# sabarim/STEm-Seg

Measured on AMD Instinct MI355X. Metric: clips/sec (T=8, 480p) embed+cluster, higher is better.
Workload: dtype f16x3: fp32 emulated from 2 fp16 terms per operand (22-bit operand significands; fp32 has 24), power-of-two operand scaling, 3 fp16 MFMA products per fp32 product, fp32 accumulate; |activation| >= 2.6e5 -> non-finite, flagged on the device, clip re-run in bf16x6

## Files before the change

### include/stemseg_hip.h

```cpp
#ifndef STEMSEG_HIP_H
#define STEMSEG_HIP_H

#include <stddef.h>
#include <stdint.h>

#ifdef __cplusplus
extern "C" {
#endif

#define STEMSEG_HIP_ABI_VERSION 11

#define STEMSEG_OK              0
#define STEMSEG_E_INVALID      -1
#define STEMSEG_E_HIP          -2
#define STEMSEG_E_WORKSPACE    -3
#define STEMSEG_E_UNSUPPORTED  -4

#define STEMSEG_MAX_HEAD_OUT   10
#define STEMSEG_MAX_WIDE_HEAD_OUT 64
#define STEMSEG_MAX_INSTANCES  64
#define STEMSEG_MAX_EMB_DIMS    8
#define STEMSEG_MAX_SEMSEG_CLASSES 128

int         stemseg_hip_version(void);
const char* stemseg_hip_last_error(void);
int         stemseg_hip_device_count(void);

int stemseg_hip_profile_enable(int32_t on);
int stemseg_hip_profile_read(double* out_host, int32_t n_tags);

typedef struct StemsegVolume {
    float*  ptr;
    int64_t c_stride, t_stride, y_stride;
    int32_t C, T, H, W;
    int64_t limit;
} StemsegVolume;

int stemseg_hip_padded_geometry(int32_t C, int32_t T, int32_t H, int32_t W, int64_t out[5]);


int stemseg_hip_pack_conv_weight(const float* w, float* packed, int32_t Cout, int32_t Cin, int32_t taps, void* stream);

#define STEMSEG_TILE_CFG_DEEP 8
typedef struct StemsegConvEpilogue {
    int32_t      relu;
    const float* residual;
    int64_t      res_c_stride, res_t_stride, res_y_stride;
    int32_t      decode_H, decode_W;
    int32_t      precision;
    int32_t      frames, plan_frames;
    int64_t      plan_scratch_floats;
} StemsegConvEpilogue;
#define STEMSEG_PRECISION_F32    0
#define STEMSEG_PRECISION_BF16X6 2
#define STEMSEG_PRECISION_F16X3  3
int64_t stemseg_hip_packed_weight_bytes_prec(int32_t Cout, int32_t Cin, int32_t taps, int32_t precision);
int stemseg_hip_pack_conv_weight_prec(const float* w, void* packed, int32_t Cout, int32_t Cin, int32_t taps, int32_t precision, void* stream);
int stemseg_hip_conv3d(const StemsegVolume* in, const float* packed_w, const float* bias, const StemsegVolume* out,
                       int32_t kt, int32_t kh, int32_t kw, int32_t tile_cfg, float* splitk_scratch,
                       int64_t splitk_scratch_floats, const StemsegConvEpilogue* epilogue, void* stream);
int stemseg_hip_conv3d_zero_t_halo(const StemsegVolume* in, const float* packed_w, const float* bias, const StemsegVolume* out,
                                   int32_t kt, int32_t kh, int32_t kw, int32_t tile_cfg, float* splitk_scratch,
                                   int64_t splitk_scratch_floats, const StemsegConvEpilogue* epilogue, int32_t groups, float eps,
                                   float* stats, double* gn_scratch, void* stream);
int stemseg_hip_conv3d_zero_t_halo_clips(const StemsegVolume* in, const float* packed_w, const float* bias, const StemsegVolume* out,
                                         int32_t kt, int32_t kh, int32_t kw, int32_t tile_cfg, float* splitk_scratch,
                                         int64_t splitk_scratch_floats, const StemsegConvEpilogue* epilogue, int32_t groups, float eps,
                                         float* stats, double* gn_scratch, int32_t plan_clips, void* stream);

int stemseg_hip_conv3d_zero_t_halo_batch(const StemsegVolume* in, const float* packed_w, const float* bias, const StemsegVolume* out,
                                         int32_t kt, int32_t kh, int32_t kw, int32_t tile_cfg, const StemsegConvEpilogue* epilogue,
                                         int32_t n_clips, int64_t in_clip_stride, int64_t out_clip_stride, void* stream);

typedef struct StemsegConvPlanRecord {
    int32_t kt, kh, kw;
    int32_t ck, mt;
    int32_t rows, tw, nt;
    int32_t flat, pmax;
    int32_t gl, blk;
    int32_t threads;
    int32_t precision;
    int32_t ksplit, chunks_per_split, nchunks;
    int32_t grid[3];
    int32_t row0, row1;
    int32_t vec4, vec_epi;
    int32_t reduce;
    int32_t gn;
    int32_t zero_t_halo;
    int32_t nb;
    int32_t deep;
} StemsegConvPlanRecord;
#define STEMSEG_PLAN_GN          1
#define STEMSEG_PLAN_ZERO_T_HALO 2
int stemseg_hip_conv3d_plan(const StemsegVolume* in, const float* bias, const StemsegVolume* out, int32_t kt, int32_t kh, int32_t kw,
                            int32_t tile_cfg, const float* splitk_scratch, int64_t splitk_scratch_floats,
                            const StemsegConvEpilogue* epilogue, int32_t form, int32_t gn_groups, StemsegConvPlanRecord* records,
                            int32_t capacity, int32_t* count);
int stemseg_hip_conv3d_plan_clips(const StemsegVolume* in, const float* bias, const StemsegVolume* out, int32_t kt, int32_t kh, int32_t kw,
                                  int32_t tile_cfg, const float* splitk_scratch, int64_t splitk_scratch_floats,
                                  const StemsegConvEpilogue* epilogue, int32_t form, int32_t gn_groups, int32_t plan_clips,
                                  StemsegConvPlanRecord* records, int32_t capacity, int32_t* count);

int64_t stemseg_hip_packed_grouped_weight_bytes(int32_t Cout, int32_t Cin_g, int32_t groups, int32_t precision);
int stemseg_hip_pack_grouped_conv_weight(const float* w, void* packed, int32_t Cout, int32_t Cin_g, int32_t groups, int32_t precision, void* stream);
int stemseg_hip_conv2d_grouped(const StemsegVolume* in, const void* packed_w, const float* bias, const StemsegVolume* out, int32_t groups,
                               int32_t stride, int32_t relu, int32_t precision, int32_t plan_frames, void* stream);

int64_t stemseg_hip_conv3d_gn_scratch_doubles(int32_t Cout, int32_t groups);
int stemseg_hip_conv3d_gn(const StemsegVolume* in, const float* packed_w, const float* bias, const StemsegVolume* out,
                          int32_t kt, int32_t kh, int32_t kw, int32_t tile_cfg, float* splitk_scratch,
                          int64_t splitk_scratch_floats, int32_t precision, int32_t groups, float eps,
                          float* stats, double* gn_scratch, void* stream);

int stemseg_hip_groupnorm_stats(const float* x, int32_t C, int64_t S, int32_t groups, float eps,
                                float* stats, double* scratch, void* stream);

int stemseg_hip_gn_relu_pool(const float* x, int32_t C, int32_t T, int32_t H, int32_t W, int32_t groups,
                             const float* stats, const float* gamma, const float* beta, int32_t pool,
                             const StemsegVolume* out, void* stream);

int stemseg_hip_upsample_trilinear(const float* in, int32_t C, int32_t T, int32_t H, int32_t W,
                                   int32_t st, int32_t sy, int32_t sx, const StemsegVolume* out, void* stream);

int stemseg_hip_copy_to_volume(const float* in, int32_t layout, const StemsegVolume* out, void* stream);

int stemseg_hip_heads(const float* x, int32_t Cin, int32_t T, int32_t H, int32_t W,
                      const float* w, const float* bias, int32_t n_out, const int32_t* act_host,
                      const int32_t* grid_axis_host, const float* grid_t, const float* grid_y, const float* grid_x,
                      float* out, void* stream);

int stemseg_hip_nonfinite_flags(const float* x, int64_t n, int32_t* flags, int32_t n_flags, void* stream);

typedef struct StemsegDecoderDesc {
    int32_t struct_bytes;
    int32_t in_channels;
    int32_t inter[4];
    int32_t T, H4, W4;
    int32_t gn_groups;
    float   gn_eps;
    int32_t pool[3];
    int32_t t_scale[3];
    int32_t n_out;
    int32_t act[STEMSEG_MAX_EMB_DIMS * 2];
    int32_t grid_axis[STEMSEG_MAX_EMB_DIMS * 2];
    int32_t input_layout;
    int32_t concurrency;
    int32_t detached;
    int32_t precision;
    int32_t n_clips;
    int64_t feat_clip_stride[4];
    int64_t out_clip_stride;
    int32_t plan_clips;
    int32_t reserved;
} StemsegDecoderDesc;

typedef struct StemsegDecoderWeights {
    const float* conv_w[7];
    const float* conv_b[7];
    const float* gn_w[7];
    const float* gn_b[7];
    const float* fuse_w[3];
    const float* head_w;
    const float* head_b;
    const float* grid_t;
    const float* grid_y;
    const float* grid_x;
} StemsegDecoderWeights;

size_t stemseg_hip_decoder_workspace_bytes(const StemsegDecoderDesc* desc);
int stemseg_hip_decoder_init_workspace(const StemsegDecoderDesc* desc, void* workspace, size_t ws_bytes, void* stream);
int stemseg_hip_decoder_check_workspace(const StemsegDecoderDesc* desc, const void* workspace, size_t ws_bytes, int32_t* n_bad_host,
                                        int64_t* first_bad_host, void* stream);
int stemseg_hip_decoder_forward(const StemsegDecoderDesc* desc, const StemsegDecoderWeights* weights,
                                const float* const feats[4], float* out,
                                void* workspace, size_t ws_bytes, void* stream);

int stemseg_hip_decoder_join(int32_t concurrency, void* stream);

#define STEMSEG_MAX_ENCODER_BLOCKS 40

typedef struct StemsegEncoderDesc {
    int32_t struct_bytes;
    int32_t blocks[4];
    int32_t T, H, W;
    int32_t out_channels;
    int32_t precision;
    int32_t n_clips;
    int32_t clip_frames;
    int32_t clip_stride;
    int32_t plan_frames;
    int32_t fuse_tail;
    int32_t conv2_groups;
    int32_t width_per_group;
    int32_t stride_in_3x3;
} StemsegEncoderDesc;

typedef struct StemsegEncoderWeights {
    const float* stem_w;
    const float* stem_b;
    const float* stem_w_s2d;
    const float* conv1_w[STEMSEG_MAX_ENCODER_BLOCKS];   const float* conv1_b[STEMSEG_MAX_ENCODER_BLOCKS];
    const float* conv2_w[STEMSEG_MAX_ENCODER_BLOCKS];   const float* conv2_b[STEMSEG_MAX_ENCODER_BLOCKS];
    const float* conv3_w[STEMSEG_MAX_ENCODER_BLOCKS];   const float* conv3_b[STEMSEG_MAX_ENCODER_BLOCKS];
    const float* down_w[STEMSEG_MAX_ENCODER_BLOCKS];    const float* down_b[STEMSEG_MAX_ENCODER_BLOCKS];
    const float* fpn_inner_w[4]; const float* fpn_inner_b[4];
    const float* fpn_layer_w[4]; const float* fpn_layer_b[4];
} StemsegEncoderWeights;

size_t stemseg_hip_encoder_workspace_bytes(const StemsegEncoderDesc* desc);
int stemseg_hip_encoder_plan_offsets(const StemsegEncoderDesc* desc, int64_t* out25);
int stemseg_hip_encoder_stage_end_mask(const StemsegEncoderDesc* desc, int32_t* mask_out);

int stemseg_hip_stem_conv(const float* frames, const float* w_tap_major, const float* bias, float* out, int32_t T, int32_t H, int32_t W,
                          void* stream);
#define STEMSEG_STREAM_FORM_AUTO   0
#define STEMSEG_STREAM_FORM_SCALAR 1
#define STEMSEG_STREAM_FORM_VEC4   2
#define STEMSEG_UP2_FORM_SCALAR    1
#define STEMSEG_UP2_FORM_VEC4X2    2
#define STEMSEG_UP2_FORM_DENSE     3
int stemseg_hip_maxpool3x3s2(const float* in, int64_t planes, int32_t H, int32_t W, float* out, int32_t form, int32_t* form_used, void* stream);
int stemseg_hip_encoder_subsample2(const float* in, int64_t planes, int32_t H, int32_t W, float* out, int32_t form, int32_t* form_used,
                                   void* stream);
int stemseg_hip_upsample2x_add(const StemsegVolume* fine, const float* fine_dense, const StemsegVolume* coarse, int32_t form, int32_t* form_used,
                               void* stream);
int stemseg_hip_stem_s2d(const float* frames, int32_t T, int32_t H, int32_t W, const StemsegVolume* s2d, void* stream);
int stemseg_hip_encoder_stream_forms(const StemsegEncoderDesc* desc, int32_t out[7]);
int stemseg_hip_encoder_init_workspace(const StemsegEncoderDesc* desc, void* workspace, size_t ws_bytes, void* stream);
int stemseg_hip_encoder_check_workspace(const StemsegEncoderDesc* desc, const void* workspace, size_t ws_bytes, int32_t* n_bad_host,
                                        int64_t* first_bad_host, void* stream);
int stemseg_hip_encoder_forward(const StemsegEncoderDesc* desc, const StemsegEncoderWeights* weights, const float* frames,
                                const StemsegVolume* out, void* workspace, size_t ws_bytes, void* stream);
int stemseg_hip_encoder_stem_forward(const StemsegEncoderDesc* desc, const StemsegEncoderWeights* weights, const float* frames, float* stem_out,
                                     float* pooled, void* workspace, size_t ws_bytes, void* stream);


int stemseg_hip_seediness_accumulate(float* acc, const float* plane, int64_t n, int32_t first, void* stream);
int stemseg_hip_fg_mask(const float* acc, float count, float thr, uint8_t* mask, int64_t n, void* stream);
int stemseg_hip_fg_mask_frames(const float* acc, const float* counts, float thr, uint8_t* mask, int32_t F, int64_t HW,
                               void* stream);

int stemseg_hip_fg_gather(const float* emb, const float* bw, const float* seed, const uint8_t* fg,
                          int32_t E, int32_t Ev, int32_t T, int64_t HW,
                          float* emb_out, float* bw_out, float* seed_out, int32_t* voxel_index,
                          int64_t* frame_offsets, void* scratch, void* stream);

typedef struct StemsegClusterParams {
    float   primary_prob_thresh;
    float   secondary_prob_thresh;
    float   min_seediness_prob;
    int32_t max_instances;
    int32_t n_free_dims;
    float   free_dim_bandwidths[STEMSEG_MAX_EMB_DIMS];
} StemsegClusterParams;
// ... 319 lines not shown
```

### stem-seg_amd/csrc/conv_igemm.h

```cpp
#pragma once
#include "common.h"
#include "split_operand.h"
#include <algorithm>
#include <type_traits>

namespace stemseg {

typedef float f32x16 __attribute__((ext_vector_type(16)));

constexpr int MIN_WG4 = 4;

struct ConvKParams {
    const float* in;
    int64_t in_cs, in_ts, in_ys, in_limit;
    int in_H;
    const float* wpk;
    const float* bias;
    float* out;
    int64_t out_cs, out_ts, out_ys;
    int Cin, Cout, T, H, W;
    int tiles_x, tiles_y;
    int vec4;
    int chunks_per_split;
    int64_t out_split_stride;
    int relu;
    const float* res;
    int64_t res_cs, res_ts, res_ys;
    int dec_H, dec_W;
    int vec_epi;
    int t_fastest;
    int flat_t;
    int T_all;
    int n_co;
    double* gn_part;
    int gn_cpg, gn_cap, gn_slot0;
    int* gn_used_host;
    int nb;
    int zero_t_halo;
    int64_t in_bs, out_bs, gn_bs;
    unsigned int* out_p16;
};

template <int KT_, int KH_, int KW_, int CK_, int MI_, int NI_, int WM_, int WN_, int COLS_, bool PIPE_ = false, int BF_ = 0, bool DB_ = false,
          int PMAX_ = 0, bool GL_ = false, int BLK_ = 0>
struct ConvCfg {
    static constexpr bool PIPE = PIPE_, X6 = BF_ >= 2, F16 = BF_ == 3, DB = DB_, FLAT = PMAX_ > 0, GL = GL_;
    static_assert(BF_ == 0 || BF_ == 2 || BF_ == 3, "precision: 0 fp32-input MFMA, 2 bf16x6, 3 f16x3");
    static constexpr int NPX = BF_ == 2 ? 3 : 2;
    static constexpr int NPROD = BF_ == 2 ? 6 : 3;
    static constexpr int PMAX = PMAX_;
    static constexpr int KT = KT_, KH = KH_, KW = KW_, CK = CK_, MI = MI_, NI = NI_, WM = WM_, WN = WN_, COLS = COLS_;
    static constexpr int TAPS = KT * KH * KW;
    static constexpr int NTHREADS = 64 * WM * WN;
    static constexpr int MT = WM * MI * 32;
    static constexpr int NSEG = WN * NI;
    static constexpr bool BLK = BLK_ != 0;
    static constexpr bool DEEP = BLK_ < 0;
    static constexpr int TD = DEEP ? WN_ : 1;
    static constexpr int TPL = DEEP ? TD + 2 : KT_;
    static constexpr int NLIVE = (BLK && !DEEP) ? BLK_ * COLS_ : NSEG;
    static constexpr int ROWS = DEEP ? 4 * NI_ : (BLK ? 4 * BLK_ : NSEG / COLS);
    static constexpr int TW = BLK ? 8 * COLS_ : COLS_ * 32;
    static constexpr int RH = ROWS + KH - 1;
    static constexpr int XL = (TW + KW - 1 + 3) / 4;
    static constexpr int XP = DEEP ? 24 : (BLK ? ((4 * XL + 23) / 32) * 32 + 8 : 4 * XL);
    static constexpr int NT = NSEG * 32;
    static constexpr int FL = NT + 2 * PMAX + 8;
    static constexpr int IN_CH_STRIDE = FLAT ? KT * FL : KT * RH * XP;
    static constexpr int IN_PAIR_STRIDE = PMAX_ > 0 ? KT * (WN_ * NI_ * 32 + 2 * PMAX_ + 8) : TPL * RH * XP;
    static constexpr int IN_PLANE_STRIDE = (CK / 2) * IN_PAIR_STRIDE;
    static constexpr int IN_FLOATS = X6 ? NPX * IN_PLANE_STRIDE : CK * IN_CH_STRIDE;
    static constexpr SplitLayout SL = SplitLayout(TAPS, BF_, CK_);
    static_assert(BF_ < 2 || CK_ == split_chunk_channels(TAPS, BF_), "split-staged tiles walk the channel chunks the weights were packed in");
    static constexpr int TPG = SL.TPG, CPH = SL.CPH, NTG = SL.NTG;
    static constexpr int NCG = X6 ? SL.NCG : 1;
    static constexpr int G = NTG * NCG;
    static constexpr int NPL = SL.NPL;
    static constexpr int W_FLOATS = X6 ? NPL * G * 2 * MT * 4 : CK * TAPS * MT;
    static constexpr int GA = (G + 1) / 2;
    static constexpr int WMODE = (BF_ >= 2 && G <= 2) ? (BF_ == 3 ? 1 : ((WM * WN >= 8 || MI * NI < 8) ? 2 : 0)) : 0;
    static constexpr bool SP = WMODE == 1, LA = WMODE == 2;
    static constexpr int BUF_FLOATS = IN_FLOATS + W_FLOATS;
    static constexpr int LDS_FLOATS = BUF_FLOATS * (DB ? 2 : 1);
    static_assert(!X6 || CK % (2 * CPH) == 0, "split-staged: a chunk holds whole k-groups");
    static_assert(BLK || NSEG % COLS == 0, "segments must fill whole rows");
    static_assert(!BLK || (BF_ >= 2 && PMAX_ == 0 && NI_ == 2 && NLIVE <= NSEG && NLIVE > NSEG - NI_ && XP % 32 == (DEEP ? 24 : 8) && XP >= 4 * XL), "block tiles: split-staged, the last wave may lack its second block");
    static_assert(!DEEP || (BF_ == 3 && KT_ == 3 && WM_ == 1 && COLS_ == 1 && BLK_ == -1), "deep tile: f16x3, 3x3x3, one wave per output plane");
    static_assert(CK % 4 == 0 || (DB && GL_ && CK == 2 && !X6), "channel chunk is a multiple of the packed sub-chunk (4), or one channel pair (GL)");
    static_assert(LDS_FLOATS * 4 <= (X6 ? 160 : 80) * 1024, "two workgroups per CU (x6 eight-wave tiles: one)");
    static_assert(!X6 || (!DB && !GL && G >= 2 && CK % 2 == 0), "x6: 2-D / 3-D tiles, two weight phases");
    static_assert(!FLAT || (KH == 3 && KW == 3 && PMAX % 4 == 0), "flat tiles: 3x3 taps");
    static_assert(DB == GL_, "two LDS buffers are the direct-to-LDS form");
    static_assert(!GL || (DB && !X6), "direct-to-LDS staging is the double-buffered fp32 form");
    static constexpr int NWAVES = WM * WN;
    static constexpr int MIN_WG = X6 ? (MI * NI > 8 ? 1 : NWAVES >= 8 ? 2 : (LDS_FLOATS * 4 * 2 <= 160 * 1024 ? NWAVES / 2 : NWAVES / 4))
                                     : ((GL && LDS_FLOATS * 4 * 4 <= 140 * 1024 && MI * NI <= 4) ? MIN_WG4 : ((GL && LDS_FLOATS * 4 * 3 <= 160 * 1024) ? 3 : 2));
};

template <class C>
__global__ __launch_bounds__(C::NTHREADS, C::MIN_WG) void conv_igemm_kernel(const ConvKParams p) {
    __shared__ __attribute__((aligned(16))) float smem[C::LDS_FLOATS];
    float* const in_lds = smem;
    float* const w_lds = smem + C::IN_FLOATS;

    const int tid = threadIdx.x;
    const int lane = tid & 63;
    const int wave = __builtin_amdgcn_readfirstlane(tid >> 6);
    const int wm = wave / C::WN, wn = wave % C::WN;
    const int half = lane >> 5, l31 = lane & 31;

    int bx;
    {
        const int nwg = gridDim.x, xcd = blockIdx.x & 7, q = nwg >> 3, r = nwg & 7;
        bx = (xcd < r ? xcd * (q + 1) : r * (q + 1) + (xcd - r) * q) + (blockIdx.x >> 3);
    }
    const int co_tile = bx % p.n_co;
    bx /= p.n_co;
    int tx, ty, t;
    if constexpr (C::DEEP) {
        tx = bx % p.tiles_x;
        ty = bx / p.tiles_x;
        t = 0;
    } else if (C::KT > 1 && p.t_fastest) {
        t = bx % p.T;
        bx /= p.T;
        tx = bx % p.tiles_x;
        ty = bx / p.tiles_x;
    } else {
        tx = bx % p.tiles_x;
        bx /= p.tiles_x;
        ty = bx % p.tiles_y;
        t = bx / p.tiles_y;
    }
    const int x0 = C::FLAT ? 0 : tx * C::TW, y0 = C::FLAT ? 0 : ty * C::ROWS;
    constexpr bool TV = C::KT == 3 && C::X6 && !C::FLAT && (C::F16 || C::MI * C::NI < 8);
    int tvar = 0;
    if constexpr (TV) {
        if constexpr (C::DEEP) tvar = wn == 0 ? 1 : (wn == C::WN - 1 ? 2 : 0);
        else if (p.zero_t_halo && p.T > 1) tvar = t == 0 ? 1 : (t == p.T - 1 ? 2 : 0);
    }
    const int svar = C::DEEP ? 0 : tvar;
    const int t_out = C::DEEP ? wn : t;
    auto seg_row = [](const int sN, const int l) __attribute__((always_inline)) { return C::DEEP ? (sN % C::NI) * 4 + (l >> 3) : (C::BLK ? (sN / C::COLS) * 4 + (l >> 3) : sN / C::COLS); };
    auto seg_col = [](const int sN, const int l) __attribute__((always_inline)) { return C::DEEP ? (l & 7) : (C::BLK ? (sN % C::COLS) * 8 + (l & 7) : (sN % C::COLS) * 32 + l); };
    const bool ni1_live = !C::BLK || (wn * C::NI + 1 < C::NLIVE);
    const int pitch = (int)p.in_ys;
    const int F0 = pitch + tx * C::NT;
    const int co0 = co_tile * C::MT;

    f32x16 acc[C::MI][C::NI];
#pragma unroll
    for (int mi = 0; mi < C::MI; ++mi)
#pragma unroll
        for (int ni = 0; ni < C::NI; ++ni)
#pragma unroll
            for (int r = 0; r < 16; ++r) acc[mi][ni][r] = 0.f;

    const float* a_ptr = w_lds + half * C::MT + wm * (C::MI * 32) + l31;
    const float* b_ptr[C::NI];
#pragma unroll
    for (int ni = 0; ni < C::NI; ++ni) {
        const int s = wn * C::NI + ni;
        b_ptr[ni] = C::FLAT ? in_lds + half * C::IN_CH_STRIDE + s * 32 + l31 + 3
                            : in_lds + half * C::IN_CH_STRIDE + seg_row(s, l31) * C::XP + seg_col(s, l31);
    }

    const unsigned int* b_ptr6[C::NI];
#pragma unroll
    for (int ni = 0; ni < C::NI; ++ni) {
        const int s = wn * C::NI + ni;
        b_ptr6[ni] = C::FLAT ? reinterpret_cast<const unsigned int*>(in_lds) + half * (C::CPH / 2) * C::IN_PAIR_STRIDE + s * 32 + l31 + 3
                             : reinterpret_cast<const unsigned int*>(in_lds) + half * (C::CPH / 2) * C::IN_PAIR_STRIDE + seg_row(min(s, C::NLIVE - 1), l31) * C::XP + seg_col(min(s, C::NLIVE - 1), l31);
        if constexpr (C::DEEP) b_ptr6[ni] += wn * (C::RH * C::XP);
    }
    const float* in_tile = p.in + (int64_t)blockIdx.y * p.in_bs + (int64_t)t * p.in_ts + x0;
    const int64_t tile_base = (int64_t)t * p.in_ts + x0;

    constexpr int XQ = C::XP / 4;
    constexpr int NQ = C::FLAT ? C::IN_FLOATS / 4 : C::CK * C::KT * C::RH * XQ;
    constexpr int MQ = C::MT / 4;
    constexpr int NWQ = C::X6 ? C::NPL * C::G * 2 * C::MT : C::CK * C::TAPS * MQ;
    constexpr int IN_PT = (NQ + C::NTHREADS - 1) / C::NTHREADS, W_PT = (NWQ + C::NTHREADS - 1) / C::NTHREADS;
    auto fetch_in = [&](int c0, int q) -> float4 {
        if constexpr (C::FLAT) {
            constexpr int FQ = C::FL / 4;
            const int j4 = q % FQ, rr = q / FQ, dt = rr % C::KT, c = rr / C::KT;
            const int f = F0 - pitch - 4 + 4 * j4;
            const int64_t rel = (int64_t)(c0 + c) * p.in_cs + (int64_t)dt * p.in_ts + f;
            float4 v = make_float4(0.f, 0.f, 0.f, 0.f);
            if (c0 + c < p.Cin && f >= 0 && 4 * j4 < C::NT + 2 * pitch + 8 && tile_base + rel + 4 <= p.in_limit)
                v = *reinterpret_cast<const float4*>(in_tile + rel);
            return v;
        }
        const int xq = q % XQ;
        int rr = q / XQ;
        const int r = rr % C::RH;
        rr /= C::RH;
        const int dt = rr % C::KT;
        const int c = rr / C::KT;
        const int yy = min(y0 + r, p.in_H - 1);
        const int64_t rel = (int64_t)(c0 + c) * p.in_cs + (int64_t)dt * p.in_ts + (int64_t)yy * p.in_ys + xq * 4;
        float4 v = make_float4(0.f, 0.f, 0.f, 0.f);
        if (c0 + c < p.Cin && tile_base + rel + 4 <= p.in_limit) v = *reinterpret_cast<const float4*>(in_tile + rel);
        return v;
    };
    auto fetch_w = [&](int c0, int q) -> float4 {
        const int mq = q % MQ;
        if constexpr (C::CK == 2) {
            const int row2 = q / MQ, tap = row2 >> 1, e = row2 & 1;
            const float* wsrc2 = p.wpk + ((int64_t)(c0 / 4) * (C::TAPS * 4) + tap * 4 + ((c0 >> 1) & 1) * 2 + e) * p.Cout + co0;
            float4 v2 = make_float4(0.f, 0.f, 0.f, 0.f);
            if (c0 + e < p.Cin && co0 + mq * 4 < p.Cout) v2 = *reinterpret_cast<const float4*>(wsrc2 + mq * 4);
            return v2;
        }
        const int row = q / MQ;
        const int ch = c0 + (row / (C::TAPS * 4)) * 4 + (row & 3);
        const float* wsrc = p.wpk + (int64_t)(c0 / 4) * (C::TAPS * 4) * p.Cout + co0;
        float4 v = make_float4(0.f, 0.f, 0.f, 0.f);
        if (ch < p.Cin && co0 + mq * 4 < p.Cout) v = *reinterpret_cast<const float4*>(wsrc + (int64_t)row * p.Cout + mq * 4);
        return v;
    };
    auto addr_in = [&](int c0, int q) -> const float* {
        int64_t rel;
        if constexpr (C::FLAT) {
            constexpr int FQ = C::FL / 4;
            const int j4 = q % FQ, rr = q / FQ, dt = rr % C::KT, c = rr / C::KT;
            const int f = max(F0 - pitch - 4 + 4 * j4, 0);
            rel = (int64_t)(c0 + c) * p.in_cs + (int64_t)dt * p.in_ts + f;
        } else {
            const int xq = q % XQ;
            int rr = q / XQ;
            const int r = rr % C::RH;
            rr /= C::RH;
            const int dt = rr % C::KT;
            const int c = rr / C::KT;
            const int yy = min(y0 + r, p.in_H - 1);
            rel = (int64_t)(c0 + c) * p.in_cs + (int64_t)dt * p.in_ts + (int64_t)yy * p.in_ys + xq * 4;
        }
        const int64_t last = p.in_limit - 4 - tile_base;
        return in_tile + (rel < last ? rel : last);
    };
    auto addr_w = [&](int c0, int q) -> const float* {
        const int mq = q % MQ;
        if constexpr (C::CK == 2) {
            const int row2 = q / MQ, tap = row2 >> 1, e = row2 & 1;
            return p.wpk + ((int64_t)(c0 / 4) * (C::TAPS * 4) + tap * 4 + ((c0 >> 1) & 1) * 2 + e) * p.Cout + co0 + mq * 4;
        } else {
            const int row = q / MQ;
            return p.wpk + (int64_t)(c0 / 4) * (C::TAPS * 4) * p.Cout + co0 + (int64_t)row * p.Cout + mq * 4;
        }
    };
    auto glds_chunk = [&](int c0, const int off) {
        typedef const __attribute__((address_space(1))) void* gptr_t;
        typedef __attribute__((address_space(3))) void* lptr_t;
#pragma unroll
        for (int k = 0; k < IN_PT; ++k) {
            const int q = tid + k * C::NTHREADS;
            if (q < NQ) __builtin_amdgcn_global_load_lds((gptr_t)addr_in(c0, q), (lptr_t)(in_lds + off + (q - lane) * 4), 16, 0, 0);
        }
#pragma unroll
        for (int k = 0; k < W_PT; ++k) {
            const int q = tid + k * C::NTHREADS;
            if (q < NWQ) __builtin_amdgcn_global_load_lds((gptr_t)addr_w(c0, q), (lptr_t)(w_lds + off + (q - lane) * 4), 16, 0, 0);
        }
    };
    auto stage_direct = [&](int c0) {
        if (p.vec4) {
            for (int q = tid; q < NQ; q += C::NTHREADS) *reinterpret_cast<float4*>(in_lds + q * 4) = fetch_in(c0, q);
        } else if constexpr (!C::FLAT) {
            constexpr int NE = C::CK * C::KT * C::RH * C::XP;
            for (int q = tid; q < NE; q += C::NTHREADS) {
                const int xx = q % C::XP;
                int rr = q / C::XP;
                const int r = rr % C::RH;
                rr /= C::RH;
                const int dt = rr % C::KT;
                const int c = rr / C::KT;
                const int yy = min(y0 + r, p.in_H - 1);
                const int64_t rel = (int64_t)(c0 + c) * p.in_cs + (int64_t)dt * p.in_ts + (int64_t)yy * p.in_ys + xx;
                float v = 0.f;
                if (c0 + c < p.Cin && tile_base + rel < p.in_limit) v = in_tile[rel];
                in_lds[q] = v;
            }
        }
        for (int q = tid; q < NWQ; q += C::NTHREADS) *reinterpret_cast<float4*>(w_lds + q * 4) = fetch_w(c0, q);
    };

    auto split3 = [](const float x, unsigned int& h, unsigned int& m, unsigned int& l) {
        unsigned short sh, sm, sl = 0;
        if constexpr (C::F16) split_act_f16(x, sh, sm);
        else split_bf16x3(x, sh, sm, sl);
        h = sh; m = sm; l = sl;
    };
    constexpr int FQ6 = C::FL / 4;
    constexpr int XL6 = C::XL;
    constexpr int NQ6 = C::FLAT ? (C::CK / 2) * C::KT * FQ6 : (C::CK / 2) * (C::DEEP ? C::TD : C::KT) * C::RH * XL6;
    auto in6_lds = [](const int q) __attribute__((always_inline)) {
        if constexpr (C::DEEP) return (q / XL6 + (q / (XL6 * C::RH * C::TD)) * 2 * C::RH + C::RH) * C::XP + (q % XL6) * 4;
        else return C::BLK ? (q / XL6) * C::XP + (q % XL6) * 4 : q * 4;
    };
    constexpr int IN_PT6 = C::X6 ? (NQ6 + C::NTHREADS - 1) / C::NTHREADS : 1;
    constexpr int NWQ_A = C::NPL * C::GA * 2 * C::MT, NWQ6 = C::NPL * C::G * 2 * C::MT;
    auto in6_rel = [&](int q, int& c) -> int64_t {
        if constexpr (C::FLAT) {
            const int j4 = q % FQ6, rr = q / FQ6, dt = rr % C::KT;
            c = 2 * (rr / C::KT);
            const int f = F0 - pitch - 4 + 4 * j4;
            if (f < 0 || 4 * j4 >= C::NT + 2 * pitch + 8) return -1;
            return (int64_t)c * p.in_cs + (int64_t)dt * p.in_ts + f;
        }
        const int xq = q % XL6;
        int rr = q / XL6;
        const int r = rr % C::RH;
        rr /= C::RH;
        constexpr int NPLQ = C::DEEP ? C::TD : C::KT;
        const int dt = rr % NPLQ + (C::DEEP ? 1 : 0);
        c = 2 * (rr / NPLQ);
        const int yy = min(y0 + r, p.in_H - 1);
        return (int64_t)c * p.in_cs + (int64_t)dt * p.in_ts + (int64_t)yy * p.in_ys + xq * 4;
    };
    auto fetch_in6 = [&](int c0, int q, float4& v0, float4& v1) {
        int c;
        const int64_t rel0 = in6_rel(q, c);
        const int64_t rel = rel0 + (int64_t)c0 * p.in_cs;
        v0 = v1 = make_float4(0.f, 0.f, 0.f, 0.f);
        if (rel0 < 0) return;
        if (c0 + c < p.Cin && tile_base + rel + 4 <= p.in_limit) v0 = *reinterpret_cast<const float4*>(in_tile + rel);
        if (c0 + c + 1 < p.Cin && tile_base + rel + p.in_cs + 4 <= p.in_limit) v1 = *reinterpret_cast<const float4*>(in_tile + rel + p.in_cs);
    };
    unsigned int in6_voff[IN_PT6];
    int in6_clim[IN_PT6];
    const int64_t in6_room = (p.in_limit - 4 - tile_base) * 4;
    constexpr int R6 = C::RH * XL6;
    constexpr int NQ6V = TV ? (C::CK / 2) * 2 * R6 : NQ6;
    constexpr int IN_PT6V = TV ? (NQ6V + C::NTHREADS - 1) / C::NTHREADS : IN_PT6;
    auto in6_live = [](const int qv, const int first) __attribute__((always_inline)) { return qv + (qv / (2 * R6)) * R6 + (first ? R6 : 0); };
    if constexpr (C::X6) {
#pragma unroll
        for (int k = 0; k < IN_PT6; ++k) {
            int q = tid + k * C::NTHREADS;
            bool inside = q < NQ6;
            if constexpr (TV && !C::DEEP) {
                if (tvar) { inside = q < NQ6V; q = inside ? in6_live(q, tvar == 1) : 0; }
            }
            int c = 0;
            const int64_t rel0 = inside ? in6_rel(q, c) : 0;
            const int64_t rel = rel0 < 0 ? 0 : rel0;
            in6_voff[k] = (unsigned int)(rel * 4);
            const int64_t slack = in6_room - rel * 4;
            const int64_t by_room = slack < 0 ? 0 : slack / (p.in_cs * 4) + 1;
            in6_clim[k] = (inside && rel0 >= 0) ? (int)min((int64_t)(p.Cin - c), by_room) : 0;
        }
    }
    typedef float f32x4 __attribute__((ext_vector_type(4)));
    auto fetch_in6_fast = [&](int c0, int k, f32x4& v0, f32x4& v1) __attribute__((always_inline)) {
        const char* base = reinterpret_cast<const char*>(in_tile) + (int64_t)c0 * p.in_cs * 4;
        const unsigned int cs4 = (unsigned int)(p.in_cs * 4);
        v0 = *reinterpret_cast<const f32x4*>(base + (c0 < in6_clim[k] ? in6_voff[k] : 0u));
        v1 = *reinterpret_cast<const f32x4*>(base + (c0 + 1 < in6_clim[k] ? in6_voff[k] + cs4 : 0u));
    };
    auto store_in6 = [&](int q, const float4& v0, const float4& v1) {
        unsigned int h0, m0, l0, h1, m1, l1;
        uint4 ph, pm, pl;
        if constexpr (C::F16) {
            split_pair_f16(v0.x, v1.x, ph.x, pm.x); split_pair_f16(v0.y, v1.y, ph.y, pm.y);
            split_pair_f16(v0.z, v1.z, ph.z, pm.z); split_pair_f16(v0.w, v1.w, ph.w, pm.w);
            unsigned int* d16 = reinterpret_cast<unsigned int*>(in_lds) + in6_lds(q);
            *reinterpret_cast<uint4*>(d16) = ph;
            *reinterpret_cast<uint4*>(d16 + C::IN_PLANE_STRIDE) = pm;
            return;
        }
        split3(v0.x, h0, m0, l0); split3(v1.x, h1, m1, l1); ph.x = h0 | (h1 << 16); pm.x = m0 | (m1 << 16); pl.x = l0 | (l1 << 16);
        split3(v0.y, h0, m0, l0); split3(v1.y, h1, m1, l1); ph.y = h0 | (h1 << 16); pm.y = m0 | (m1 << 16); pl.y = l0 | (l1 << 16);
        split3(v0.z, h0, m0, l0); split3(v1.z, h1, m1, l1); ph.z = h0 | (h1 << 16); pm.z = m0 | (m1 << 16); pl.z = l0 | (l1 << 16);
        split3(v0.w, h0, m0, l0); split3(v1.w, h1, m1, l1); ph.w = h0 | (h1 << 16); pm.w = m0 | (m1 << 16); pl.w = l0 | (l1 << 16);
        unsigned int* d = reinterpret_cast<unsigned int*>(in_lds) + in6_lds(q);
        *reinterpret_cast<uint4*>(d) = ph;
        *reinterpret_cast<uint4*>(d + C::IN_PLANE_STRIDE) = pm;
        if constexpr (C::NPX == 3) *reinterpret_cast<uint4*>(d + 2 * C::IN_PLANE_STRIDE) = pl;
    };
    auto store_in6_masked = [&](int c0, int k, int q, const f32x4& r0, const f32x4& r1) __attribute__((always_inline)) {
        const bool ok0 = c0 < in6_clim[k], ok1 = c0 + 1 < in6_clim[k];
        float4 v0, v1;
        v0.x = ok0 ? r0.x : 0.f; v0.y = ok0 ? r0.y : 0.f; v0.z = ok0 ? r0.z : 0.f; v0.w = ok0 ? r0.w : 0.f;
        v1.x = ok1 ? r1.x : 0.f; v1.y = ok1 ? r1.y : 0.f; v1.z = ok1 ? r1.z : 0.f; v1.w = ok1 ? r1.w : 0.f;
        store_in6(q, v0, v1);
    };
    auto stage_in6_direct = [&](int c0) {
        if (p.vec4) {
            for (int q = tid; q < NQ6; q += C::NTHREADS) {
                float4 v0, v1;
                fetch_in6(c0, q, v0, v1);
                store_in6(q, v0, v1);
            }
        } else if constexpr (!C::FLAT && !C::DEEP) {
            constexpr int NE6 = (C::CK / 2) * C::KT * C::RH * C::XP;
            for (int q = tid; q < NE6; q += C::NTHREADS) {
                const int xx = q % C::XP;
                int rr = q / C::XP;
                const int r = rr % C::RH;
                rr /= C::RH;
                const int dt = rr % C::KT;
                const int c = 2 * (rr / C::KT);
                const int yy = min(y0 + r, p.in_H - 1);
                const int64_t rel = (int64_t)(c0 + c) * p.in_cs + (int64_t)dt * p.in_ts + (int64_t)yy * p.in_ys + xx;
                float a0 = 0.f, a1 = 0.f;
                if (c0 + c < p.Cin && tile_base + rel < p.in_limit) a0 = in_tile[rel];
                if (c0 + c + 1 < p.Cin && tile_base + rel + p.in_cs < p.in_limit) a1 = in_tile[rel + p.in_cs];
                unsigned int h0, m0, l0, h1, m1, l1;
                split3(a0, h0, m0, l0);
                split3(a1, h1, m1, l1);
                unsigned int* d = reinterpret_cast<unsigned int*>(in_lds) + q;
                d[0] = h0 | (h1 << 16);
                d[C::IN_PLANE_STRIDE] = m0 | (m1 << 16);
                if constexpr (C::NPX == 3) d[2 * C::IN_PLANE_STRIDE] = l0 | (l1 << 16);
            }
        }
    };
    constexpr int W_PT6 = C::X6 ? ((C::SP ? NWQ6 : NWQ_A) + C::NTHREADS - 1) / C::NTHREADS : 1;
    static_assert(C::NTHREADS % C::MT == 0 && NWQ_A % C::MT == 0, "weight pieces: a thread keeps its column");
    const unsigned int w6_voff = C::X6 ? ((unsigned int)(tid / C::MT) * (unsigned int)p.Cout + (unsigned int)min(tid % C::MT, p.Cout - 1 - co0)) * 16u : 0u;
    auto w6_src = [&](int c0, int q_uniform) __attribute__((always_inline)) -> const char* {
        const char* base = reinterpret_cast<const char*>(p.wpk) +
                           (((int64_t)(c0 / C::CK) * (C::NPL * C::G * 2) + q_uniform / C::MT) * p.Cout + co0) * 16;
        return base + w6_voff;
    };
    auto compute6 = [&](auto g0c, auto g1c, auto&& side, auto live_c) __attribute__((always_inline)) {
        constexpr int g0 = decltype(g0c)::value, g1 = decltype(g1c)::value;
        constexpr bool LIVE1 = decltype(live_c)::value;
        constexpr int NPL = C::NPL, NPX = C::NPX, NA = 3;
        typedef typename std::conditional<C::F16, _Float16, __bf16>::type h16;
        typedef h16 h16x8 __attribute__((ext_vector_type(8)));
        const char* a_base = reinterpret_cast<const char*>(w_lds) + (half * C::MT + wm * (C::MI * 32) + l31) * 16;
        const unsigned int* bdy6[C::NI][3];
        if constexpr (C::FLAT) {
#pragma unroll
            for (int ni = 0; ni < C::NI; ++ni) { bdy6[ni][0] = b_ptr6[ni]; bdy6[ni][1] = b_ptr6[ni] + pitch; bdy6[ni][2] = b_ptr6[ni] + 2 * pitch; }
        }
        auto ld_b = [&](const int grp, h16x8 (&b)[NPX][C::NI]) __attribute__((always_inline)) {
            const int cg = grp / C::NTG, tg = grp % C::NTG;
#pragma unroll
            for (int ni = 0; ni < (LIVE1 ? C::NI : 1); ++ni)
#pragma unroll
                for (int pl = 0; pl < NPX; ++pl) {
                    uint4 w4;
                    unsigned int* wv = reinterpret_cast<unsigned int*>(&w4);
#pragma unroll
                    for (int wd = 0; wd < 4; ++wd) {
                        const int j0 = 2 * wd, tapi = j0 / C::CPH, chl = j0 % C::CPH;
                        int tap = tg * C::TPG + tapi;
                        tap = tap < C::TAPS ? tap : C::TAPS - 1;
                        const int dt = tap / (C::KH * C::KW), dy = (tap / C::KW) % C::KH, dx = tap % C::KW;
                        if constexpr (C::FLAT) {
                            const int off = pl * C::IN_PLANE_STRIDE + (cg * C::CPH + chl / 2) * C::IN_PAIR_STRIDE + dt * C::FL + dx;
                            wv[wd] = bdy6[ni][dy][off];
                        } else {
                            const int off = pl * C::IN_PLANE_STRIDE + (cg * C::CPH + chl / 2) * C::IN_PAIR_STRIDE + (dt * C::RH + dy) * C::XP + dx;
                            wv[wd] = b_ptr6[ni][off];
                        }
                    }
                    b[pl][ni] = __builtin_bit_cast(h16x8, w4);
                }
        };
        auto ld_a = [&](const int grp, const int mi, h16x8 (&a)[NA]) __attribute__((always_inline)) {
#pragma unroll
            for (int pl = 0; pl < NPL; ++pl)
                a[pl] = *reinterpret_cast<const h16x8*>(a_base + (((grp * NPL + pl) * 2) * C::MT + mi * 32) * 16);
        };
        auto mm = [&](const int mi, h16x8 (&a)[NA], const h16x8 (&b)[NPX][C::NI]) __attribute__((always_inline)) {
            if constexpr (C::F16) {
                a[2] = a[0] * (h16)(1.0f / F16X3_LO_SCALE);
#define SS_X6_TERM(PA, PB)                                                                                                     \
    _Pragma("unroll") for (int ni = 0; ni < (LIVE1 ? C::NI : 1); ++ni)                                                         \
        acc[mi][ni] = __builtin_amdgcn_mfma_f32_32x32x16_f16(a[PA], b[PB][ni], acc[mi][ni], 0, 0, 0);
                SS_X6_TERM(1, 0) SS_X6_TERM(2, 1) SS_X6_TERM(0, 0)
#undef SS_X6_TERM
            } else {
#define SS_X6_TERM(PA, PB)                                                                                                     \
    _Pragma("unroll") for (int ni = 0; ni < (LIVE1 ? C::NI : 1); ++ni)                                                         \
        acc[mi][ni] = __builtin_amdgcn_mfma_f32_32x32x16_bf16(a[PA], b[PB][ni], acc[mi][ni], 0, 0, 0);
                SS_X6_TERM(2, 0) SS_X6_TERM(0, 2) SS_X6_TERM(1, 1) SS_X6_TERM(1, 0) SS_X6_TERM(0, 1) SS_X6_TERM(0, 0)
#undef SS_X6_TERM
            }
        };
        constexpr int NSTEP = (g1 - g0) * C::MI;
        h16x8 bfr[NPX][C::NI], a0[NA], a1[NA];
        side(-1);
        ld_b(g0, bfr);
        ld_a(g0, 0, a0);
#pragma unroll
        for (int st = 0; st < NSTEP; st += 2) {
            const int mi = st % C::MI;
            if (st + 1 < NSTEP) ld_a(g0 + (st + 1) / C::MI, (st + 1) % C::MI, a1);
            side(st);
            __builtin_amdgcn_sched_barrier(0);
            mm(mi, a0, bfr);
            __builtin_amdgcn_sched_barrier(0);
            if (st + 1 < NSTEP) {
                if ((st + 1) % C::MI == 0) ld_b(g0 + (st + 1) / C::MI, bfr);
                if (st + 2 < NSTEP) ld_a(g0 + (st + 2) / C::MI, (st + 2) % C::MI, a0);
                side(st + 1);
                __builtin_amdgcn_sched_barrier(0);
                mm((st + 1) % C::MI, a1, bfr);
                __builtin_amdgcn_sched_barrier(0);
                if (st + 2 < NSTEP && (st + 2) % C::MI == 0) ld_b(g0 + (st + 2) / C::MI, bfr);
            }
        }
    };
    auto compute = [&](const int buf_off = 0) {
        constexpr int NSUB = C::CK >= 4 ? C::CK / 4 : 1, NCP = C::CK >= 4 ? 2 : 1, WROWS = C::CK >= 4 ? 4 : 2;
        const float* bdy[C::NI][3];
        if constexpr (C::FLAT) {
#pragma unroll
            for (int ni = 0; ni < C::NI; ++ni) {
                bdy[ni][0] = b_ptr[ni]; bdy[ni][1] = b_ptr[ni] + pitch; bdy[ni][2] = b_ptr[ni] + 2 * pitch;
            }
        }
        constexpr int NSTEPS = NSUB * C::TAPS * NCP;
        auto ld = [&](const int i, float (&a)[C::MI], float (&b)[C::NI]) {
            const int cp = i % NCP, tap = (i / NCP) % C::TAPS, sub = i / (NCP * C::TAPS);
            const int dt = tap / (C::KH * C::KW), dy = (tap / C::KW) % C::KH, dx = tap % C::KW;
            const int wrow = (sub * C::TAPS + tap) * WROWS + cp * 2;
            const int boff = C::FLAT ? (sub * 4 + cp * 2) * C::IN_CH_STRIDE + dt * C::FL + dx
                                     : (sub * 4 + cp * 2) * C::IN_CH_STRIDE + (dt * C::RH + dy) * C::XP + dx;
#pragma unroll
            for (int mi = 0; mi < C::MI; ++mi) a[mi] = a_ptr[buf_off + wrow * C::MT + mi * 32];
#pragma unroll
            for (int ni = 0; ni < C::NI; ++ni) {
                if constexpr (C::FLAT) b[ni] = bdy[ni][dy][buf_off + boff];
                else b[ni] = b_ptr[ni][buf_off + boff];
            }
        };
        auto mm = [&](const float (&a)[C::MI], const float (&b)[C::NI]) {
#pragma unroll
            for (int mi = 0; mi < C::MI; ++mi)
#pragma unroll
                for (int ni = 0; ni < C::NI; ++ni)
                    acc[mi][ni] = __builtin_amdgcn_mfma_f32_32x32x2f32(a[mi], b[ni], acc[mi][ni], 0, 0, 0);
        };
        float a0[C::MI], b0[C::NI], a1[C::MI], b1[C::NI];
        ld(0, a0, b0);
#pragma unroll
        for (int i = 0; i < NSTEPS; i += 2) {
            if (i + 1 < NSTEPS) ld(i + 1, a1, b1);
            __builtin_amdgcn_sched_barrier(0);
            mm(a0, b0);
            __builtin_amdgcn_sched_barrier(0);
            if (i + 1 < NSTEPS) {
                if (i + 2 < NSTEPS) ld(i + 2, a0, b0);
                __builtin_amdgcn_sched_barrier(0);
                mm(a1, b1);
                __builtin_amdgcn_sched_barrier(0);
            }
        }
    };

    const int c_begin = blockIdx.z * p.chunks_per_split * C::CK;
    const int c_end = min(p.Cin, c_begin + p.chunks_per_split * C::CK);
    if constexpr (C::X6) {
        typedef std::integral_constant<int, 0> Q0;
        typedef std::integral_constant<int, NWQ_A> QA;
        typedef std::integral_constant<int, NWQ6> QE;
        f32x4 rin[2 * IN_PT6];
        f32x4 rw6[W_PT6];
        f32x4 rw6b[W_PT6];
        auto fetch_w6_k = [&](int c0, auto q0c, auto q1c, f32x4 (&r)[W_PT6], const int k) __attribute__((always_inline)) {
            constexpr int q0 = decltype(q0c)::value, q1 = decltype(q1c)::value;
            if ((k + 1) * C::NTHREADS <= q1 - q0 || q0 + tid + k * C::NTHREADS < q1) r[k] = *reinterpret_cast<const f32x4*>(w6_src(c0, q0 + k * C::NTHREADS));
        };
        auto store_w6 = [&](auto q0c, auto q1c, const f32x4 (&r)[W_PT6]) __attribute__((always_inline)) {
            constexpr int q0 = decltype(q0c)::value, q1 = decltype(q1c)::value;
    #pragma unroll
            for (int k = 0; k < W_PT6; ++k) { const int q = q0 + tid + k * C::NTHREADS; if ((k + 1) * C::NTHREADS <= q1 - q0 || (k * C::NTHREADS < q1 - q0 && q < q1)) *reinterpret_cast<f32x4*>(w_lds + q * 4) = r[k]; }
        };
        auto store_in6_all = [&](int c0, auto var_c) __attribute__((always_inline)) {
            constexpr int V = decltype(var_c)::value;
            constexpr int NQV = V ? NQ6V : NQ6, PTV = V ? IN_PT6V : IN_PT6;
            if (p.vec4) {
#pragma unroll
                for (int k = 0; k < PTV; ++k) {
                    const int q = tid + k * C::NTHREADS;
                    if ((k + 1) * C::NTHREADS <= NQV || q < NQV) store_in6_masked(c0, k, V ? in6_live(q, V == 1) : q, rin[2 * k], rin[2 * k + 1]);
                }
            } else stage_in6_direct(c0);
        };
        auto side_items = [&](const int st, auto nspread_c, auto n_in_c, auto n_w_c, auto&& f_in, auto&& f_w) __attribute__((always_inline)) {
            constexpr int nspread = decltype(nspread_c)::value, n_in = decltype(n_in_c)::value, n_w = decltype(n_w_c)::value, n = n_in + n_w;
            if (st >= nspread || st < 0) return;
#pragma unroll
            for (int i = 0; i < n; ++i)
                if (i >= st * n / nspread && i < (st + 1) * n / nspread) { if (i < n_in) f_in(i); else f_w(i - n_in); }
        };
        constexpr int NSA = C::GA * C::MI, NSB = (C::G - C::GA) * C::MI, NSALL = C::G * C::MI;
        constexpr int NPA = (NWQ_A + C::NTHREADS - 1) / C::NTHREADS, NPB = (NWQ6 - NWQ_A + C::NTHREADS - 1) / C::NTHREADS;
        constexpr int NPALL = (NWQ6 + C::NTHREADS - 1) / C::NTHREADS;
        constexpr bool SPRD = C::F16;
        typedef std::integral_constant<int, C::GA> GAc;
        typedef std::integral_constant<int, C::G> Gc;
        typedef std::integral_constant<int, 0> I0;
        typedef std::integral_constant<int, IN_PT6> INc;
        constexpr int TG_FIRST = TV ? (C::KH * C::KW) / C::TPG : 0, TG_LAST = TV ? (2 * C::KH * C::KW + C::TPG - 1) / C::TPG : C::G;
        static_assert(!TV || (C::NCG == 1 && !C::SP && !C::LA && TG_FIRST < C::GA && TG_LAST > C::GA), "temporal-halo variants: one channel group, both phases keep a k-group");
        if (c_begin < c_end) {
            if constexpr (TV) {
                const int q_lo = svar == 1 ? C::NPL * TG_FIRST * 2 * C::MT : 0, q_hi = svar == 2 ? C::NPL * TG_LAST * 2 * C::MT : NWQ6;
                for (int q = q_lo + tid; q < q_hi; q += C::NTHREADS) *reinterpret_cast<float4*>(w_lds + q * 4) = *reinterpret_cast<const float4*>(w6_src(c_begin, q - tid));
            } else {
                for (int q = tid; q < NWQ6; q += C::NTHREADS) *reinterpret_cast<float4*>(w_lds + q * 4) = *reinterpret_cast<const float4*>(w6_src(c_begin, q - tid));
            }
            if constexpr (C::DEEP) {
                constexpr int ZQ = C::RH * C::XP / 4;
                for (int q = tid; q < C::NPX * (C::CK / 2) * 2 * ZQ; q += C::NTHREADS) {
                    const int k = q / ZQ;
                    unsigned int* d = reinterpret_cast<unsigned int*>(in_lds) + (k >> 1) * C::IN_PAIR_STRIDE + (k & 1) * (C::TD + 1) * (C::RH * C::XP) + (q % ZQ) * 4;
                    *reinterpret_cast<uint4*>(d) = make_uint4(0u, 0u, 0u, 0u);
                }
            }
            stage_in6_direct(c_begin);
        }
        __syncthreads();
        typedef std::true_type Yes;
        typedef std::false_type No;
        auto f_in_at = [&](const int cn) { return [&, cn](const int k) __attribute__((always_inline)) { if (p.vec4) fetch_in6_fast(cn, k, rin[2 * k], rin[2 * k + 1]); }; };
        if constexpr (C::SP) {
            auto chunk = [&](const int c0, auto more_c) __attribute__((always_inline)) {
                constexpr bool more = decltype(more_c)::value;
                const int cn = c0 + C::CK;
                compute6(Q0{}, Gc{}, [&](const int st) __attribute__((always_inline)) {
                    if constexpr (more) {
                        side_items(SPRD ? st : -1 - st, std::integral_constant<int, SPRD ? NSALL : 1>{}, INc{}, std::integral_constant<int, NPALL>{}, f_in_at(cn),
                                   [&](const int k) __attribute__((always_inline)) { fetch_w6_k(cn, Q0{}, QE{}, rw6, k); });
                    }
                }, Yes{});
                __syncthreads();
                if constexpr (more) {
                    store_w6(Q0{}, QE{}, rw6);
                    store_in6_all(cn, I0{});
                    __syncthreads();
                }
            };
            int c0 = c_begin;
            for (; c0 + C::CK < c_end; c0 += C::CK) chunk(c0, Yes{});
            if (c0 < c_end) chunk(c0, No{});
        } else if constexpr (C::LA) {
            if (c_begin + C::CK < c_end) {
#pragma unroll
                for (int k = 0; k < NPA; ++k) fetch_w6_k(c_begin + C::CK, Q0{}, QA{}, rw6, k);
            }
            auto chunk = [&](const int c0, auto more_c, auto more2_c) __attribute__((always_inline)) {
                constexpr bool more = decltype(more_c)::value, more2 = decltype(more2_c)::value;
                const int cn = c0 + C::CK, cnn = c0 + 2 * C::CK;
                compute6(Q0{}, GAc{}, [&](const int st) __attribute__((always_inline)) {
                    if constexpr (more) side_items(SPRD ? st : -1 - st, std::integral_constant<int, SPRD ? NSA : 1>{}, INc{}, std::integral_constant<int, NPB>{}, f_in_at(cn),
                                         [&](const int k) __attribute__((always_inline)) { fetch_w6_k(cn, QA{}, QE{}, rw6b, k); });
                }, Yes{});
                __syncthreads();
                if constexpr (more) store_w6(Q0{}, QA{}, rw6);
                compute6(GAc{}, Gc{}, [&](const int st) __attribute__((always_inline)) {
                    if constexpr (more2) side_items(SPRD ? st : -1 - st, std::integral_constant<int, SPRD ? NSB : 1>{}, I0{}, std::integral_constant<int, NPA>{}, [](const int) {},
                                          [&](const int k) __attribute__((always_inline)) { fetch_w6_k(cnn, Q0{}, QA{}, rw6, k); });
                }, Yes{});
                __syncthreads();
                if constexpr (more) {
                    store_w6(QA{}, QE{}, rw6b);
                    store_in6_all(cn, I0{});
                    __syncthreads();
                }
            };
            int c0 = c_begin;
            for (; c0 + 2 * C::CK < c_end; c0 += C::CK) chunk(c0, Yes{}, Yes{});
            if (c0 + C::CK < c_end) { chunk(c0, Yes{}, No{}); c0 += C::CK; }
            if (c0 < c_end) chunk(c0, No{}, No{});
        } else {
            auto chunk = [&](const int c0, auto more_c, auto live_c, auto var_c) __attribute__((always_inline)) {
                constexpr bool more = decltype(more_c)::value;
                constexpr int V = decltype(var_c)::value;
                constexpr int VS = C::DEEP ? 0 : V;
                constexpr int G0 = V == 1 ? TG_FIRST : 0, G1 = V == 2 ? TG_LAST : C::G;
                typedef std::integral_constant<int, G0> G0c;
                typedef std::integral_constant<int, G1> G1c;
                typedef std::integral_constant<int, C::NPL * (VS == 1 ? TG_FIRST : 0) * 2 * C::MT> QS;
                typedef std::integral_constant<int, C::NPL * (VS == 2 ? TG_LAST : C::G) * 2 * C::MT> QL;
                constexpr int nsa = (C::GA - G0) * C::MI, nsb = (G1 - C::GA) * C::MI;
                constexpr int npa = (NWQ_A - QS::value + C::NTHREADS - 1) / C::NTHREADS, npb = (QL::value - NWQ_A + C::NTHREADS - 1) / C::NTHREADS;
                typedef std::integral_constant<int, VS ? IN_PT6V : IN_PT6> INv;
                const int cn = c0 + C::CK;
                compute6(G0c{}, GAc{}, [&](const int st) __attribute__((always_inline)) {
                    if constexpr (more) side_items(SPRD ? st : -1 - st, std::integral_constant<int, SPRD ? nsa : 1>{}, INv{}, std::integral_constant<int, npa>{}, f_in_at(cn),
                                         [&](const int k) __attribute__((always_inline)) { fetch_w6_k(cn, QS{}, QA{}, rw6, k); });
                }, live_c);
                __syncthreads();
                if constexpr (more) store_w6(QS{}, QA{}, rw6);
                compute6(GAc{}, G1c{}, [&](const int st) __attribute__((always_inline)) {
                    if constexpr (more) {
                        side_items(SPRD ? st : -1 - st, std::integral_constant<int, SPRD ? nsb : 1>{}, I0{}, std::integral_constant<int, npb>{}, [](const int) {},
                                   [&](const int k) __attribute__((always_inline)) { fetch_w6_k(cn, QA{}, QL{}, rw6, k); });
                    }
                }, live_c);
                __syncthreads();
                if constexpr (more) {
                    store_w6(QA{}, QL{}, rw6);
                    store_in6_all(cn, std::integral_constant<int, VS>{});
                    __syncthreads();
                }
            };
            auto run_v = [&](auto live_c, auto var_c) __attribute__((always_inline)) {
                int c0 = c_begin;
                for (; c0 + C::CK < c_end; c0 += C::CK) chunk(c0, Yes{}, live_c, var_c);
                if (c0 < c_end) chunk(c0, No{}, live_c, var_c);
            };
            auto run = [&](auto live_c) __attribute__((always_inline)) {
                if constexpr (TV) {
                    if (tvar == 1) run_v(live_c, std::integral_constant<int, 1>{});
                    else if (tvar == 2) run_v(live_c, std::integral_constant<int, 2>{});
                    else run_v(live_c, I0{});
                } else run_v(live_c, I0{});
            };
            if constexpr (C::BLK && C::NLIVE < C::NSEG) {
                if (ni1_live) run(Yes{});
                else run(No{});
            } else run(Yes{});
        }
        if constexpr (C::F16) {
            constexpr SplitLayout sl(C::TAPS, STEMSEG_PRECISION_F16X3, C::CK);
            const float* invp = reinterpret_cast<const float*>(reinterpret_cast<const char*>(p.wpk) + sl.inv_offset(p.Cout, p.Cin));
            const int co_w = co0 + wm * (C::MI * 32) + 4 * half;
#pragma unroll
            for (int mi = 0; mi < C::MI; ++mi)
#pragma unroll
                for (int j = 0; j < 4; ++j) {
                    const int co4 = co_w + mi * 32 + 8 * j;
                    const float4 sc = co4 < p.Cout ? *reinterpret_cast<const float4*>(invp + co4) : make_float4(1.f, 1.f, 1.f, 1.f);
#pragma unroll
                    for (int ni = 0; ni < C::NI; ++ni) {
                        acc[mi][ni][4 * j + 0] *= sc.x; acc[mi][ni][4 * j + 1] *= sc.y;
                        acc[mi][ni][4 * j + 2] *= sc.z; acc[mi][ni][4 * j + 3] *= sc.w;
// ... 31 lines not shown
        }
        __syncthreads();
        for (int c0 = c_begin; c0 < c_end; c0 += C::CK) {
            const bool more = c0 + C::CK < c_end;
            if (more) fetch_regs(c0 + C::CK);
            __builtin_amdgcn_sched_barrier(0);
            compute();
            __syncthreads();
            if (more) {
                regs_to_lds();
                __syncthreads();
            }
        }
    } else {
        for (int c0 = c_begin; c0 < c_end; c0 += C::CK) {
            __syncthreads();
            stage_direct(c0);
            __syncthreads();
            compute();
        }
    }

    const int co_base = co0 + wm * (C::MI * 32);
    if (p.gn_part) {
        __syncthreads();
        constexpr int GPW8 = C::MI * 4;
        double* red = reinterpret_cast<double*>(smem + C::NWAVES * 32 * 36);
        static_assert(C::NWAVES * 32 * 36 + 2 * C::WM * C::WN * GPW8 * 2 * 2 <= C::LDS_FLOATS, "GN partial sums must fit the staging LDS");
        const bool g4 = p.gn_cpg == 4;
        bool ok[C::NI];
#pragma unroll
        for (int ni = 0; ni < C::NI; ++ni) {
            const int sN = wn * C::NI + ni;
            int y = y0 + seg_row(sN, l31), x = x0 + seg_col(sN, l31);
            if constexpr (C::FLAT) {
                const int f = F0 + sN * 32 + l31, y1 = f / pitch, x1 = f - y1 * pitch;
                y = y1 - 1;
                x = (x1 >= 1) ? x1 - 1 : p.W;
            }
            ok[ni] = y < p.H && x < p.W && sN < C::NLIVE;
        }
#pragma unroll
        for (int mi = 0; mi < C::MI; ++mi) {
#pragma unroll
            for (int j = 0; j < 4; ++j) {
                float fs = 0.f, fss = 0.f;
#pragma unroll
                for (int rr = 0; rr < 4; ++rr) {
                    const int co = co_base + mi * 32 + rr + 8 * j + 4 * half;
                    const float bv = (p.bias && co < p.Cout) ? p.bias[co] : 0.f;
#pragma unroll
                    for (int ni = 0; ni < C::NI; ++ni)
                        if (ok[ni]) {
                            const float v = acc[mi][ni][4 * j + rr] + bv;
                            fs += v;
                            fss += v * v;
                        }
                }
                double ds = (double)fs, dss = (double)fss;
#pragma unroll
                for (int o = 16; o > 0; o >>= 1) { ds += __shfl_xor(ds, o, 64); dss += __shfl_xor(dss, o, 64); }
                if (!g4) { ds += __shfl_xor(ds, 32, 64); dss += __shfl_xor(dss, 32, 64); }
                if (l31 == 0 && (g4 || half == 0)) {
                    const int gl = g4 ? (mi * 4 + j) * 2 + half : mi * 4 + j;
                    const int gpw = g4 ? 2 * GPW8 : GPW8;
                    double* d = red + ((size_t)(wm * gpw + gl) * C::WN + wn) * 2;
                    d[0] = ds; d[1] = dss;
                }
            }
        }
        __syncthreads();
        {
            const int gpw = g4 ? 2 * GPW8 : GPW8, ngw = C::WM * gpw;
            if (tid < ngw) {
                double a = 0.0, b = 0.0;
#pragma unroll
                for (int k = 0; k < C::WN; ++k) { a += red[((size_t)tid * C::WN + k) * 2]; b += red[((size_t)tid * C::WN + k) * 2 + 1]; }
                const int gg = co0 / p.gn_cpg + tid;
                if (gg * p.gn_cpg < p.Cout) {
                    const int slot = p.gn_slot0 + (t * p.tiles_y + ty) * p.tiles_x + tx;
                    double* o = p.gn_part + (int64_t)blockIdx.y * p.gn_bs + ((size_t)gg * p.gn_cap + slot) * 2;
                    o[0] = a; o[1] = b;
                }
            }
        }
        __syncthreads();
    }
    if (p.vec_epi && !C::FLAT) {
        __syncthreads();
        constexpr int TP = 36;
        float* tl = smem + wave * (32 * TP);
        static_assert(C::NWAVES * 32 * 36 <= C::LDS_FLOATS, "epilogue transpose buffer must fit the staging LDS");
#pragma unroll
        for (int ni = 0; ni < C::NI; ++ni) {
            const int s = wn * C::NI + ni;
            if (C::BLK && s >= C::NLIVE) continue;
            const int y = y0 + seg_row(s, (lane & 7) * 4);
            const int xs = x0 + seg_col(s, (lane & 7) * 4) - (lane & 7) * 4;
            constexpr int MG = (C::MI >= 2 && C::MIN_WG < 3) ? 2 : 1;
#pragma unroll
            for (int m0 = 0; m0 < C::MI; m0 += MG) {
                float4 rres[MG][4];
                float rbias[MG][4];
#pragma unroll
                for (int mg = 0; mg < MG; ++mg)
#pragma unroll
                    for (int j = 0; j < 4; ++j) {
                        const int row = (lane >> 3) + 8 * j, c4 = (lane & 7) * 4;
                        const int co = co_base + (m0 + mg) * 32 + row;
                        const int x = xs + c4;
                        rres[mg][j] = make_float4(0.f, 0.f, 0.f, 0.f);
                        rbias[mg][j] = 0.f;
                        if (y < p.H && x < p.W && co < p.Cout) {
                            if (p.res) rres[mg][j] = *reinterpret_cast<const float4*>(p.res + (int64_t)co * p.res_cs + (int64_t)t_out * p.res_ts + (int64_t)y * p.res_ys + x);
                            if (p.bias) rbias[mg][j] = p.bias[co];
                        }
                    }
#pragma unroll
                for (int mg = 0; mg < MG; ++mg) {
                    const int mi = m0 + mg;
#pragma unroll
                    for (int r = 0; r < 16; ++r) tl[((r & 3) + 8 * (r >> 2) + 4 * half) * TP + l31] = acc[mi][ni][r];
                    __builtin_amdgcn_s_waitcnt(0xc07f);
#pragma unroll
                    for (int j = 0; j < 4; ++j) {
                        const int row = (lane >> 3) + 8 * j, c4 = (lane & 7) * 4;
                        const int co = co_base + mi * 32 + row;
                        const int x = xs + c4;
                        if (y < p.H && x < p.W && co < p.Cout) {
                            float4 v = *reinterpret_cast<const float4*>(tl + row * TP + c4);
                            const float bv = rbias[mg][j];
                            v.x += bv; v.y += bv; v.z += bv; v.w += bv;
                            const int64_t off = (int64_t)t_out * p.out_ts + (int64_t)y * p.out_ys + x;
                            const float4 rv = rres[mg][j];
                            v.x += rv.x; v.y += rv.y; v.z += rv.z; v.w += rv.w;
                            if (p.relu) { v.x = relu_keep_nan(v.x); v.y = relu_keep_nan(v.y); v.z = relu_keep_nan(v.z); v.w = relu_keep_nan(v.w); }
                            *reinterpret_cast<float4*>(p.out + (int64_t)blockIdx.y * p.out_bs + (int64_t)blockIdx.z * p.out_split_stride + (int64_t)co * p.out_cs + off) = v;
                        }
                    }
                    __builtin_amdgcn_s_waitcnt(0xc07f);
                }
            }
        }
        return;
    }
#pragma unroll
    for (int ni = 0; ni < C::NI; ++ni) {
        const int s = wn * C::NI + ni;
        if (C::BLK && s >= C::NLIVE) continue;
        int y = y0 + seg_row(s, l31);
        int x = x0 + seg_col(s, l31);
        int te = t_out;
        if constexpr (C::FLAT) {
            int f = F0 + s * 32 + l31;
            if (p.flat_t) {
                te = f / (int)p.in_ts;
                f -= te * (int)p.in_ts;
            }
            const int y1 = f / pitch, x1 = f - y1 * pitch;
            y = (y1 >= 1 && te < p.T_all) ? y1 - 1 : p.H;
            x = (x1 >= 1) ? x1 - 1 : p.W;
        }
        if (y < p.H && x < p.W) {
            int64_t off, roff = 0;
            if (p.dec_W > 0) {
                const int hw = p.dec_H * p.dec_W;
                const int t2 = x / hw, r2 = x - t2 * hw, y2 = r2 / p.dec_W, x2 = r2 - y2 * p.dec_W;
                off = (int64_t)t2 * p.out_ts + (int64_t)y2 * p.out_ys + x2;
                roff = (int64_t)t2 * p.res_ts + (int64_t)y2 * p.res_ys + x2;
            } else {
                off = (int64_t)te * p.out_ts + (int64_t)y * p.out_ys + x;
                roff = (int64_t)te * p.res_ts + (int64_t)y * p.res_ys + x;
            }
            if constexpr (C::F16) {
                if (p.out_p16) {
                    const int64_t plane_words = (int64_t)(p.Cout / 8) * p.out_cs * 4;
#pragma unroll
                    for (int mi = 0; mi < C::MI; ++mi)
#pragma unroll
                        for (int q = 0; q < 4; ++q) {
                            const int co4 = co_base + mi * 32 + 8 * q + 4 * half;
                            if (co4 < p.Cout) {
                                float v[4];
#pragma unroll
                                for (int k = 0; k < 4; ++k) {
                                    v[k] = acc[mi][ni][4 * q + k] + (p.bias ? p.bias[co4 + k] : 0.f);
                                    if (p.relu) v[k] = relu_keep_nan(v[k]);
                                }
                                uint2 hw, lw;
                                split_pair_f16(v[0], v[1], hw.x, lw.x);
                                split_pair_f16(v[2], v[3], hw.y, lw.y);
                                unsigned int* d = p.out_p16 + ((int64_t)(co4 / 8) * p.out_cs + off) * 4 + 2 * half;
                                *reinterpret_cast<uint2*>(d) = hw;
                                *reinterpret_cast<uint2*>(d + plane_words) = lw;
                            }
                        }
                    continue;
                }
            }
            float* o = p.out + (int64_t)blockIdx.y * p.out_bs + (int64_t)blockIdx.z * p.out_split_stride + off;
#pragma unroll
            for (int mi = 0; mi < C::MI; ++mi) {
#pragma unroll
                for (int r = 0; r < 16; ++r) {
                    const int co = co_base + mi * 32 + (r & 3) + 8 * (r >> 2) + 4 * half;
                    if (co < p.Cout) {
                        float v = acc[mi][ni][r] + (p.bias ? p.bias[co] : 0.f);
                        if (p.res) v += p.res[(int64_t)co * p.res_cs + roff];
                        if (p.relu) v = relu_keep_nan(v);
                        o[(int64_t)co * p.out_cs] = v;
                    }
                }
            }
        }
    }
}

struct SplitReduceParams {
    const float* partial;
    const float* bias;
    const float* res;
    float* out;
    int64_t out_cs, out_ts, out_ys, res_cs, res_ts, res_ys, slab;
    int C, H, W, ksplit, relu;
    int64_t V;
    unsigned per_c;
    double* gn_part;
    int gn_cpg, gn_cap, gn_slot0;
    int64_t part_bs, out_bs, gn_bs;
};
void launch_splitk_reduce(const SplitReduceParams& rp, bool vec, unsigned blocks_per_channel, unsigned clips, hipStream_t s);
constexpr int SPLITK_REDUCE_TAG = 63;

constexpr double CU_FLOPS_F32 = 0.46e12;

struct PlanCtx {
    ConvKParams shape;
    int64_t scratch_floats;
};

struct LaunchCtx {
    hipStream_t s;
    float* scratch;
    int64_t scratch_floats;
    const PlanCtx* plan;
    bool p16_keep_plan = false;
    PlanSink* sink = nullptr;
    int plan_clips = 1;
    bool deep_tile = false;
    LaunchCtx without_scratch() const { return LaunchCtx{s, nullptr, 0, plan, p16_keep_plan, sink, plan_clips, deep_tile}; }
    LaunchCtx without_plan() const { return LaunchCtx{s, scratch, scratch_floats, nullptr, p16_keep_plan, sink, plan_clips, deep_tile}; }
};

template <class C>
static int64_t tile_workgroups(const ConvKParams& d, int flat_t = 0) {
    int64_t tx = C::FLAT ? ceil_div((int64_t)d.H * d.in_ys, C::NT) : ceil_div(d.W, C::TW);
    const int64_t ty = C::FLAT ? 1 : ceil_div(d.H, C::ROWS);
    int64_t T = ceil_div(d.T, C::TD);
    if (C::FLAT && flat_t) { tx = ceil_div((int64_t)d.T * d.in_ts, C::NT); T = 1; }
    return tx * ty * T * ceil_div(d.Cout, C::MT);
}

template <class C>
static int plan_ksplit(const ConvKParams& p, const LaunchCtx& L, int flat_t, int nchunks) {
    int ksplit = 1;
    const PlanCtx* plan = L.plan;
    float* const scratch = L.scratch;
    const ConvKParams& d = plan ? plan->shape : p;
    const int64_t d_T = plan ? d.T : p.T_all;
    ConvKParams dd = d;
    dd.T = (int)d_T;
    const int64_t wgs = tile_workgroups<C>(dd, flat_t);
    const int64_t slab_plan = (int64_t)d.Cout * d_T * d.H * d.W;
    const int64_t plan_scratch = plan ? plan->scratch_floats : L.scratch_floats / p.nb;
    const int64_t wg_target = (C::X6 && C::NWAVES >= 8) ? 320 : 640;
    const int64_t wgs_planned = wgs * std::max(L.plan_clips, 1);
    while (scratch && ksplit * 2 <= 16 && ksplit * 2 <= nchunks && wgs_planned * ksplit * 2 <= wg_target && slab_plan * ksplit * 2 <= plan_scratch) ksplit *= 2;
    if (p.out_p16 && C::F16 && wgs >= 128 && !L.p16_keep_plan) ksplit = 1;
    return ksplit;
}

template <class C>
static int launch_cfg(ConvKParams p, const LaunchCtx& L, int force_ksplit = 0) {
    hipStream_t s = L.s;
    float* const scratch = L.scratch;
    const int64_t scratch_floats = L.scratch_floats;
    p.tiles_x = C::FLAT ? (int)ceil_div((int64_t)p.H * p.in_ys, C::NT) : (int)ceil_div(p.W, C::TW);
    p.tiles_y = C::FLAT ? 1 : (int)ceil_div(p.H, C::ROWS);
    p.T_all = p.T;
    const int flat_t = (C::FLAT && p.flat_t) ? 1 : 0;
    if (flat_t) {
        p.tiles_x = (int)ceil_div((int64_t)p.T * p.in_ts, C::NT);
        p.T = 1;
    }
    p.flat_t = flat_t;
    const int out_vec = p.vec_epi;
    if (C::FLAT) p.vec_epi = 0;
    const int nchunks = (int)ceil_div(p.Cin, C::CK);
    const int64_t slab = (int64_t)p.Cout * p.T_all * p.H * p.W;
    int ksplit = plan_ksplit<C>(p, L, flat_t, nchunks);
    if (force_ksplit > 0) ksplit = (scratch && (int64_t)p.nb * force_ksplit * slab <= scratch_floats) ? std::min(force_ksplit, nchunks) : 1;
    p.chunks_per_split = (int)ceil_div(nchunks, ksplit);
    ksplit = (int)ceil_div(nchunks, p.chunks_per_split);
    SS_CHECK_ARG(ksplit == 1 || (int64_t)p.nb * ksplit * slab <= scratch_floats, "conv3d: split-K scratch too small (%lld floats needed, %lld given)",
                 (long long)((int64_t)p.nb * ksplit * slab), (long long)scratch_floats);
    if (p.out_p16) {
        if (ksplit > 1 || !C::F16) p.out_p16 = nullptr;
        else { p.vec_epi = 0; if (p.gn_used_host) *p.gn_used_host = 1; }
    }
    SplitReduceParams rp;
    const bool rp_vec = out_vec && p.dec_W == 0 && (reinterpret_cast<uintptr_t>(scratch) % 16 == 0) && (slab % 4 == 0);
    if (ksplit > 1) {
        rp.partial = scratch; rp.bias = p.bias; rp.res = p.res; rp.out = p.out;
        rp.out_cs = p.out_cs; rp.out_ts = p.out_ts; rp.out_ys = p.out_ys; rp.res_cs = p.res_cs; rp.res_ts = p.res_ts; rp.res_ys = p.res_ys;
        rp.slab = slab; rp.C = p.Cout; rp.V = (int64_t)p.T_all * p.H * p.W; rp.ksplit = ksplit; rp.relu = p.relu;
        rp.H = p.dec_W > 0 ? p.dec_H : p.H; rp.W = p.dec_W > 0 ? p.dec_W : p.W;
        rp.gn_part = nullptr; rp.gn_cpg = rp.gn_cap = rp.gn_slot0 = 0;
        rp.part_bs = (int64_t)ksplit * slab; rp.out_bs = p.out_bs; rp.gn_bs = p.gn_bs;
        p.out_bs = (int64_t)ksplit * slab;
        p.out = scratch; p.bias = nullptr; p.res = nullptr; p.relu = 0; p.dec_H = p.dec_W = 0;
        p.out_cs = (int64_t)p.T_all * p.H * p.W; p.out_ts = (int64_t)p.H * p.W; p.out_ys = p.W;
        p.out_split_stride = slab;
        p.vec_epi = !C::FLAT && (p.W % 4 == 0) && (reinterpret_cast<uintptr_t>(scratch) % 16 == 0);
    } else p.out_split_stride = 0;
    p.n_co = (int)ceil_div(p.Cout, C::MT);
    const int grid_T = C::DEEP ? 1 : p.T;
    const int64_t red_items = slab / p.Cout / (rp_vec ? 4 : 1);
    const unsigned red_bx = (unsigned)ceil_div(red_items, 256);
    if (p.gn_part) {
        const int slot0 = *p.gn_used_host;
        const int64_t slots = ksplit > 1 ? (int64_t)p.gn_cpg * red_bx : (int64_t)p.tiles_x * p.tiles_y * grid_T;
        SS_CHECK_ARG(slot0 + slots <= p.gn_cap, "conv3d: GroupNorm partial table too small (%lld slots needed, %d available)",
                     (long long)(slot0 + slots), p.gn_cap);
        if (ksplit > 1) { rp.gn_part = p.gn_part; rp.gn_cpg = p.gn_cpg; rp.gn_cap = p.gn_cap; rp.gn_slot0 = slot0; p.gn_part = nullptr; }
        else p.gn_slot0 = slot0;
        *p.gn_used_host = slot0 + (int)slots;
    }
    dim3 grid((unsigned)((int64_t)p.tiles_x * p.tiles_y * grid_T * p.n_co), (unsigned)p.nb, (unsigned)ksplit);
    const double flops = 2.0 * p.Cin * C::TAPS * (double)p.Cout * p.T_all * p.H * p.W * p.nb;
    constexpr int tile_rows = (C::FLAT || C::BLK) ? C::NSEG : C::ROWS;
    const int tag = C::TAPS == 16 ? -1 : C::TAPS == 1 ? 10 + C::NSEG : (C::KT == 1 ? 20 + tile_rows : (tile_rows == 16 ? 9 : tile_rows));
    if (L.sink) {
        PlanSink& k = *L.sink;
        if (k.n < k.cap) {
            StemsegConvPlanRecord& r = k.rec[k.n];
            r.kt = C::KT; r.kh = C::KH; r.kw = C::KW; r.ck = C::CK; r.mt = C::MT; r.rows = C::ROWS; r.tw = C::TW; r.nt = C::NT;
            r.flat = C::FLAT ? 1 : 0; r.pmax = C::PMAX; r.gl = C::GL ? 1 : 0; r.blk = C::BLK ? C::ROWS / 4 : 0; r.threads = C::NTHREADS;
            r.precision = C::F16 ? STEMSEG_PRECISION_F16X3 : (C::X6 ? STEMSEG_PRECISION_BF16X6 : STEMSEG_PRECISION_F32);
            r.ksplit = ksplit; r.chunks_per_split = p.chunks_per_split; r.nchunks = nchunks;
            r.grid[0] = (int32_t)grid.x; r.grid[1] = (int32_t)grid.y; r.grid[2] = (int32_t)grid.z;
            r.row0 = k.row0; r.row1 = k.row0 + p.H;
            r.vec4 = p.vec4; r.vec_epi = p.vec_epi;
            r.reduce = ksplit > 1 ? (rp_vec ? 1 : 2) : 0;
            r.gn = ksplit > 1 ? (rp.gn_part ? 2 : 0) : (p.gn_part ? 1 : 0);
            r.zero_t_halo = p.zero_t_halo; r.nb = p.nb;
            r.deep = C::DEEP ? C::TD : 0;
        }
        ++k.n;
        return STEMSEG_OK;
    }
    void* ev = profile_begin(tag, flops, s);
    hipLaunchKernelGGL(conv_igemm_kernel<C>, grid, dim3(C::NTHREADS), 0, s, p);
    if (ksplit > 1) {
        SS_CHECK_ARG(red_items < (1ll << 32) - 256 && p.Cout <= 65535, "conv3d: split-K output too large (%lld elements)", (long long)slab);
        rp.per_c = (unsigned)red_items;
        void* ev_red = profile_begin(SPLITK_REDUCE_TAG, 4.0 * (ksplit + 1.0) * (double)slab * p.nb, s);
        launch_splitk_reduce(rp, rp_vec, red_bx, (unsigned)p.nb, s);
        profile_end(ev_red, s);
    }
    profile_end(ev, s);
    SS_LAUNCH_CHECK();
    return STEMSEG_OK;
}

struct RowPlan { double cost; int nA, k; };

template <class C>
static RowPlan plan_rows(const ConvKParams& d, bool have_scratch, int64_t scratch_floats, double cu_flops, int occ, double eff) {
    const int64_t slots = 256 * occ;
    const int tiles_x = (int)ceil_div(d.W, C::TW);
    const int n = (int)ceil_div(d.H, C::ROWS);
    const int64_t c = (int64_t)tiles_x * d.T * ceil_div(d.Cout, C::MT);
    const int nchunks = (int)ceil_div(d.Cin, C::CK);
    const double t_round = occ * 2.0 * C::MT * ((double)C::ROWS * C::TW) * d.Cin * C::TAPS / (cu_flops * eff);
    RowPlan best{(double)ceil_div(n * c, slots) * t_round, n, 1};
    const double t_plain = best.cost;
    static const int ks[] = {2, 3, 4, 6, 8};
    for (int nA = 0; nA < n && have_scratch; ++nA) {
        const int64_t slabB = (int64_t)d.Cout * d.T * (d.H - (int64_t)nA * C::ROWS) * d.W;
        for (int k : ks) {
            if (k > nchunks || k * slabB > scratch_floats) continue;
            const double rounds = (double)ceil_div(nA * c, slots) + (double)ceil_div((n - nA) * c * k, slots) / k;
            const double t = rounds * t_round + 2.0 * k * slabB * 4.0 / 3.0e12 + 8e-6;
            if (t < best.cost) best = RowPlan{t, nA, k};
        }
    }
    if (best.cost > 0.97 * t_plain) best = RowPlan{t_plain, n, 1};
    return best;
}

template <class C>
static int launch_rows(const ConvKParams& p0, const LaunchCtx& L, const RowPlan& plan) {
    if (plan.k <= 1) return launch_cfg<C>(p0, L);
    auto rows = [&](int r0, int r1) {
        ConvKParams q = p0;
        q.in += (int64_t)r0 * p0.in_ys; q.in_limit -= (int64_t)r0 * p0.in_ys; q.in_H = (r1 - r0) + C::KH - 1;
        q.out += (int64_t)r0 * p0.out_ys;
        if (q.res) q.res += (int64_t)r0 * p0.res_ys;
        q.H = r1 - r0;
        return q;
    };
    const int rA = plan.nA * C::ROWS;
    if (rA > 0) {
        const int rc = launch_cfg<C>(rows(0, rA), L.without_scratch().without_plan());
        if (rc) return rc;
    }
    const ConvKParams qB = rows(rA, p0.H);
    SS_CHECK_ARG((int64_t)p0.nb * plan.k * qB.Cout * qB.T * qB.H * qB.W <= L.scratch_floats, "conv3d: split-K scratch too small for the planned row cut");
    if (L.sink) L.sink->row0 = rA;
    return launch_cfg<C>(qB, L.without_plan(), plan.k);
}

template <class Big, class Med>
static int launch_planned(const ConvKParams& p, const ConvKParams& d, const LaunchCtx& L, int occ_big, int occ_med) {
    const int64_t plan_scratch = L.plan ? L.plan->scratch_floats : L.scratch_floats / p.nb;
    const RowPlan a = plan_rows<Big>(d, L.scratch != nullptr, plan_scratch, CU_FLOPS_F32, occ_big, 1.0);
    const RowPlan b = plan_rows<Med>(d, L.scratch != nullptr, plan_scratch, CU_FLOPS_F32, occ_med, 0.92);
    if (b.cost < 0.97 * a.cost) return launch_rows<Med>(p, L, b);
    return launch_rows<Big>(p, L, a);
}

template <class C>
static double tile_efficiency(int H, int W) {
    return (double)H * W / ((double)C::ROWS * ceil_div(H, C::ROWS) * (double)C::TW * ceil_div(W, C::TW));
}
template <class C>
static double flat_tile_efficiency(const ConvKParams& p) {
    return (double)p.H * p.W / ((double)C::NT * ceil_div((int64_t)p.H * p.in_ys, C::NT));
}

template <int BFV>
int launch_split_family(ConvKParams& p, const ConvKParams& d, const LaunchCtx& L, int tile_cfg, bool k3, bool k2);
int launch_stem_f16x3(const ConvKParams& p, const LaunchCtx& L);

}
```

### stem-seg_amd/csrc/conv_igemm.hip

```cpp
#include "conv_igemm.h"

namespace stemseg {

template <bool VEC>
__global__ __launch_bounds__(256) void splitk_reduce_kernel(const SplitReduceParams p) {
    constexpr int VW = VEC ? 4 : 1;
    const unsigned wq = (unsigned)p.W / VW;
    const unsigned c = blockIdx.y;
    const unsigned j = blockIdx.x * 256u + threadIdx.x;
    const bool active = j < p.per_c;
    const float* const partial = p.partial + (int64_t)blockIdx.z * p.part_bs;
    float* const outp = p.out + (int64_t)blockIdx.z * p.out_bs;
    float s1 = 0.f, s2 = 0.f;
    if (active) {
        const unsigned r2 = j / wq, x = (j - r2 * wq) * VW;
        const unsigned t = r2 / (unsigned)p.H, y = r2 - t * (unsigned)p.H;
        const int64_t i = (int64_t)c * p.V + (int64_t)r2 * p.W + x;
        const int64_t o = (int64_t)c * p.out_cs + (int64_t)t * p.out_ts + (int64_t)y * p.out_ys + x;
        if constexpr (VEC) {
            float4 acc = *reinterpret_cast<const float4*>(partial + i);
            for (int z = 1; z < p.ksplit; ++z) {
                const float4 v = *reinterpret_cast<const float4*>(partial + (int64_t)z * p.slab + i);
                acc.x += v.x; acc.y += v.y; acc.z += v.z; acc.w += v.w;
            }
            if (p.bias) { const float b = p.bias[c]; acc.x += b; acc.y += b; acc.z += b; acc.w += b; }
            if (p.res) {
                const float4 r = *reinterpret_cast<const float4*>(p.res + (int64_t)c * p.res_cs + (int64_t)t * p.res_ts + (int64_t)y * p.res_ys + x);
                acc.x += r.x; acc.y += r.y; acc.z += r.z; acc.w += r.w;
            }
            if (p.relu) { acc.x = relu_keep_nan(acc.x); acc.y = relu_keep_nan(acc.y); acc.z = relu_keep_nan(acc.z); acc.w = relu_keep_nan(acc.w); }
            *reinterpret_cast<float4*>(outp + o) = acc;
            s1 = (acc.x + acc.y) + (acc.z + acc.w);
            s2 = (acc.x * acc.x + acc.y * acc.y) + (acc.z * acc.z + acc.w * acc.w);
        } else {
            float acc = partial[i];
            for (int z = 1; z < p.ksplit; ++z) acc += partial[(int64_t)z * p.slab + i];
            if (p.bias) acc += p.bias[c];
            if (p.res) acc += p.res[(int64_t)c * p.res_cs + (int64_t)t * p.res_ts + (int64_t)y * p.res_ys + x];
            if (p.relu) acc = relu_keep_nan(acc);
            outp[o] = acc;
            s1 = acc;
            s2 = acc * acc;
        }
    }
    if (p.gn_part) {
        __shared__ double red[2][4];
        double d1 = (double)s1, d2 = (double)s2;
#pragma unroll
        for (int o = 32; o > 0; o >>= 1) { d1 += __shfl_xor(d1, o, 64); d2 += __shfl_xor(d2, o, 64); }
        if ((threadIdx.x & 63) == 0) { red[0][threadIdx.x >> 6] = d1; red[1][threadIdx.x >> 6] = d2; }
        __syncthreads();
        if (threadIdx.x == 0) {
            const int g = (int)c / p.gn_cpg, slot = p.gn_slot0 + ((int)c % p.gn_cpg) * (int)gridDim.x + (int)blockIdx.x;
            double* o = p.gn_part + (int64_t)blockIdx.z * p.gn_bs + ((size_t)g * p.gn_cap + slot) * 2;
            o[0] = (red[0][0] + red[0][1]) + (red[0][2] + red[0][3]);
            o[1] = (red[1][0] + red[1][1]) + (red[1][2] + red[1][3]);
        }
    }
}

void launch_splitk_reduce(const SplitReduceParams& rp, bool vec, unsigned blocks_per_channel, unsigned clips, hipStream_t s) {
    if (vec) hipLaunchKernelGGL(splitk_reduce_kernel<true>, dim3(blocks_per_channel, (unsigned)rp.C, clips), dim3(256), 0, s, rp);
    else hipLaunchKernelGGL(splitk_reduce_kernel<false>, dim3(blocks_per_channel, (unsigned)rp.C, clips), dim3(256), 0, s, rp);
}

using K3Big = ConvCfg<3, 3, 3, 4, 4, 2, 1, 4, 1>;
using K3BigGL = ConvCfg<3, 3, 3, 2, 4, 2, 1, 4, 1, false, 0, true, 0, true>;
using K3Med = ConvCfg<3, 3, 3, 4, 2, 2, 2, 2, 1, true>;
using K3Small = ConvCfg<3, 3, 3, 4, 2, 1, 2, 2, 1, true>;
using K1Big = ConvCfg<1, 1, 1, 32, 4, 2, 1, 4, 8, true>;
using K1Small = ConvCfg<1, 1, 1, 32, 2, 2, 2, 2, 4, true>;
using K1M64 = ConvCfg<1, 1, 1, 32, 2, 2, 1, 4, 8, true>;
using K1BigGL = ConvCfg<1, 1, 1, 16, 4, 2, 1, 4, 8, false, 0, true, 0, true>;
using K1SmallGL = ConvCfg<1, 1, 1, 16, 2, 2, 2, 2, 4, false, 0, true, 0, true>;
using K1M64GL = ConvCfg<1, 1, 1, 16, 2, 2, 1, 4, 8, false, 0, true, 0, true>;
using K2Big = ConvCfg<1, 3, 3, 8, 4, 2, 1, 4, 1, true>;
using K2Med = ConvCfg<1, 3, 3, 8, 2, 2, 2, 2, 1, true>;
using K2Small = ConvCfg<1, 3, 3, 8, 2, 1, 2, 2, 1, true>;
using K2M64 = ConvCfg<1, 3, 3, 8, 2, 2, 1, 4, 1, true>;
using K2FlatBig = ConvCfg<1, 3, 3, 8, 4, 2, 1, 4, 8, true, 0, false, 112>;
using K2FlatMed = ConvCfg<1, 3, 3, 8, 2, 2, 2, 2, 4, true, 0, false, 112>;
using K3FlatMed = ConvCfg<3, 3, 3, 4, 2, 2, 2, 2, 4, true, 0, false, 112>;
using K3FlatSmall = ConvCfg<3, 3, 3, 4, 2, 1, 2, 2, 2, true, 0, false, 112>;
using K2FlatBig56 = ConvCfg<1, 3, 3, 8, 4, 2, 1, 4, 8, true, 0, false, 56>;
using K2FlatMed56 = ConvCfg<1, 3, 3, 8, 2, 2, 2, 2, 4, true, 0, false, 56>;
using K3FlatMed56 = ConvCfg<3, 3, 3, 4, 2, 2, 2, 2, 4, true, 0, false, 56>;
using K3FlatSmall56 = ConvCfg<3, 3, 3, 4, 2, 1, 2, 2, 2, true, 0, false, 56>;

template <class Flat, class Tile2D>
static bool prefer_flat(const ConvKParams& p, int tile_cfg) {
    if (!p.vec4 || tile_cfg > 0 || p.dec_W > 0 || p.in_ys > Flat::PMAX || p.in_ys % 4 != 0 || p.W + 2 > p.in_ys) return false;
    return flat_tile_efficiency<Flat>(p) > 1.08 * tile_efficiency<Tile2D>(p.H, p.W);
}

template <class GLCfg, class Cfg>
static int launch_gl(const ConvKParams& p, const LaunchCtx& L) {
    if (p.vec4 && p.Cin % GLCfg::CK == 0 && p.Cout % GLCfg::MT == 0) return launch_cfg<GLCfg>(p, L);
    return launch_cfg<Cfg>(p, L);
}

int launch_conv3d(const StemsegVolume& in, const float* packed_w, const float* bias, const StemsegVolume& out,
                  int kt, int kh, int kw, int tile_cfg, hipStream_t s, float* scratch, int64_t scratch_floats, const ConvEpilogue* epi) {
    SS_CHECK_ARG(in.ptr && out.ptr && packed_w, "conv3d: null pointer");
    const bool deep_tile = tile_cfg == STEMSEG_TILE_CFG_DEEP;
    if (deep_tile) tile_cfg = 0;
    const int prec = epi ? epi->precision : STEMSEG_PRECISION_F32;
    SS_CHECK_ARG(prec == STEMSEG_PRECISION_F32 || prec == STEMSEG_PRECISION_BF16X6 || prec == STEMSEG_PRECISION_F16X3,
                 "conv3d: precision %d (0 f32, 2 bf16x6, 3 f16x3)", prec);
    const bool k3 = (kt == 3 && kh == 3 && kw == 3), k1 = (kt == 1 && kh == 1 && kw == 1), k2 = (kt == 1 && kh == 3 && kw == 3);
    const bool k4 = (kt == 1 && kh == 4 && kw == 4);
    SS_CHECK_ARG(k3 || k1 || k2 || (k4 && prec == STEMSEG_PRECISION_F16X3), "conv3d: kernel %dx%dx%d unsupported (3x3x3, 1x3x3, 1x1x1; 1x4x4 in f16x3 mode)", kt, kh, kw);
    const bool flat = epi && epi->dec_W > 0;
    if (flat) {
        SS_CHECK_ARG(k1 && in.T == 1 && in.H == 1 && epi->dec_H > 0 && (int64_t)out.T * out.H * out.W == in.W &&
                     out.H == epi->dec_H && out.W == epi->dec_W, "conv3d: flat-decode epilogue needs a 1x1x1 conv on a [C][V] input with V == T*H*W of `out`");
    } else {
        SS_CHECK_ARG(in.T == out.T + kt - 1 && in.H == out.H + kh - 1 && in.W == out.W + kw - 1,
                     "conv3d: input extents (%d,%d,%d) must be output (%d,%d,%d) + kernel - 1", in.T, in.H, in.W, out.T, out.H, out.W);
    }
    SS_CHECK_ARG(in.C % 4 == 0 && out.C % 32 == 0, "conv3d: Cin %% 4 == 0 and Cout %% 32 == 0 required (got %d, %d)", in.C, out.C);
    ConvKParams p;
    p.in = in.ptr; p.in_cs = in.c_stride; p.in_ts = in.t_stride; p.in_ys = in.y_stride; p.in_limit = in.limit; p.in_H = in.H;
    p.wpk = packed_w; p.bias = bias;
    p.out = out.ptr; p.out_cs = out.c_stride; p.out_ts = out.t_stride; p.out_ys = out.y_stride;
    p.Cin = in.C; p.Cout = out.C; p.T = out.T; p.H = out.H; p.W = out.W;
    if (flat) { p.T = 1; p.H = 1; p.W = in.W; }
    p.relu = epi ? epi->relu : 0;
    p.res = epi ? epi->res : nullptr;
    p.res_cs = epi ? epi->res_cs : 0; p.res_ts = epi ? epi->res_ts : 0; p.res_ys = epi ? epi->res_ys : 0;
    p.dec_H = flat ? epi->dec_H : 0; p.dec_W = flat ? epi->dec_W : 0;
    p.gn_part = epi ? epi->gn_part : nullptr;
    p.gn_cpg = epi ? epi->gn_cpg : 0; p.gn_cap = epi ? epi->gn_cap : 0; p.gn_slot0 = 0;
    p.gn_used_host = epi ? epi->gn_used : nullptr;
    p.zero_t_halo = (epi && epi->zero_t_halo && k3) ? 1 : 0;
    p.out_p16 = nullptr;
    if (epi && epi->p16_out) {
        const bool dense = out.t_stride == (int64_t)out.H * out.W && out.y_stride == out.W && out.c_stride == (int64_t)out.T * out.H * out.W;
        SS_CHECK_ARG(epi->p16_done && dense && !flat && !epi->res && !epi->gn_part && out.C % 8 == 0 && prec == STEMSEG_PRECISION_F16X3 && (!epi || epi->nb <= 1),
                     "conv3d: the pair-plane output needs f16x3, a dense output volume, no residual / statistics / clip batch");
        *epi->p16_done = 0;
        p.out_p16 = epi->p16_out;
        p.gn_used_host = epi->p16_done;
    }
    p.nb = (epi && epi->nb > 1) ? epi->nb : 1;
    p.in_bs = p.nb > 1 ? epi->in_bs : 0; p.out_bs = p.nb > 1 ? epi->out_bs : 0; p.gn_bs = p.nb > 1 ? epi->gn_bs : 0;
    SS_CHECK_ARG(p.nb == 1 || (!p.res && p.nb <= 65535 && p.in_bs % 4 == 0 && p.out_bs % 4 == 0), "conv3d: a clip batch takes no residual and 16-byte aligned clip strides");
    SS_CHECK_ARG(!p.gn_part || ((p.gn_cpg == 4 || p.gn_cpg == 8) && p.gn_used_host && p.Cout % p.gn_cpg == 0 && !(epi->relu || epi->res)),
                 "conv3d: fused GroupNorm statistics need groups of 4 or 8 channels and a plain (bias-only) epilogue");
    auto al16 = [](const void* ptr, int64_t cs, int64_t ts, int64_t ys, int T, int H) {
        return (reinterpret_cast<uintptr_t>(ptr) % 16 == 0) && (cs % 4 == 0) && (T == 1 || ts % 4 == 0) && (H == 1 || ys % 4 == 0);
    };
    p.vec_epi = (!flat && p.W % 4 == 0 && al16(p.out, p.out_cs, p.out_ts, p.out_ys, p.T, p.H) &&
                 (!p.res || al16(p.res, p.res_cs, p.res_ts, p.res_ys, p.T, p.H))) ? 1 : 0;
    p.tiles_x = p.tiles_y = 0;
    p.t_fastest = 1;
    p.flat_t = 0; p.T_all = p.T;
    const bool aligned = (reinterpret_cast<uintptr_t>(in.ptr) % 16 == 0) && (in.c_stride % 4 == 0) &&
                         (in.T == 1 || in.t_stride % 4 == 0) && (in.H == 1 || in.y_stride % 4 == 0);
    p.vec4 = aligned ? 1 : 0;
    SS_CHECK_ARG(reinterpret_cast<uintptr_t>(packed_w) % 16 == 0, "conv3d: packed weights must be 16-byte aligned");
    PlanCtx pc_store;
    const PlanCtx* pc = nullptr;
    if (epi && epi->plan_frames > 0) {
        SS_CHECK_ARG(epi->frames > 0 && epi->plan_scratch_floats >= 0, "conv3d: plan_frames needs the launch's own frame count");
        pc_store.shape = p;
        pc_store.scratch_floats = epi->plan_scratch_floats;
        if (p.T == 1 && p.H == 1) {
            SS_CHECK_ARG(p.W % epi->frames == 0, "conv3d: flat volume of %d voxels is not %d whole frames", p.W, epi->frames);
            const int64_t Wp = (int64_t)(p.W / epi->frames) * epi->plan_frames;
            SS_CHECK_ARG(Wp < (1ll << 31), "conv3d: planning volume too large");
            pc_store.shape.W = (int)Wp;
        } else {
            SS_CHECK_ARG(p.T == epi->frames, "conv3d: launch of %d t-planes announced as %d frames", p.T, epi->frames);
            pc_store.shape.T = epi->plan_frames;
        }
        pc_store.shape.T_all = pc_store.shape.T;
        pc = &pc_store;
    }
    const ConvKParams& d = pc ? pc->shape : p;
    SS_CHECK_ARG(!epi || (epi->plan_clips >= 0 && epi->plan_clips <= 4096), "conv3d: plan_clips %d", epi ? epi->plan_clips : 0);
    const LaunchCtx L{s, scratch, scratch_floats, pc, epi && epi->p16_keep_plan, epi ? epi->plan_sink : nullptr, epi && epi->plan_clips > 1 ? epi->plan_clips : 1, deep_tile};
    if (k4) return launch_stem_f16x3(p, L);
    if (prec == STEMSEG_PRECISION_BF16X6) return launch_split_family<2>(p, d, L, tile_cfg, k3, k2);
    if (prec == STEMSEG_PRECISION_F16X3) return launch_split_family<3>(p, d, L, tile_cfg, k3, k2);
    const bool auto_cfg = tile_cfg <= 0 || tile_cfg > 3;
    if (k3) {
        int cfg = tile_cfg;
        if (auto_cfg) {
            if (tile_workgroups<K3Big>(d) >= 512) cfg = 1;
            else if (tile_workgroups<K3Med>(d) >= 384) cfg = 2;
            else cfg = 3;
        }
        if (cfg == 2 && prefer_flat<K3FlatMed56, K3Med>(p, tile_cfg)) return launch_cfg<K3FlatMed56>(p, L);
        if (cfg == 3 && prefer_flat<K3FlatSmall56, K3Small>(p, tile_cfg)) return launch_cfg<K3FlatSmall56>(p, L);
        if (cfg == 2 && prefer_flat<K3FlatMed, K3Med>(p, tile_cfg)) return launch_cfg<K3FlatMed>(p, L);
        if (cfg == 3 && prefer_flat<K3FlatSmall, K3Small>(p, tile_cfg)) return launch_cfg<K3FlatSmall>(p, L);
        if (cfg == 1 && p.vec4 && p.Cout % 128 == 0) {
            if (auto_cfg) return launch_planned<K3BigGL, K3Med>(p, d, L, 2, 2);
            return launch_cfg<K3BigGL>(p, L);
        }
        if (cfg == 1 && auto_cfg) return launch_planned<K3Big, K3Med>(p, d, L, 2, 2);
        if (cfg == 1) return launch_cfg<K3Big>(p, L);
        if (cfg == 2) return launch_cfg<K3Med>(p, L);
        return launch_cfg<K3Small>(p, L);
    }
    if (k2) {
        if (p.Cout <= 64) return launch_cfg<K2M64>(p, L);
        int cfg = tile_cfg;
        if (auto_cfg) {
            const int64_t need = scratch ? 96 : 384;
            if (tile_workgroups<K2Big>(d) >= need) cfg = 1;
            else if (tile_workgroups<K2Med>(d) >= need) cfg = 2;
            else cfg = 3;
        }
        if (cfg == 1 && prefer_flat<K2FlatBig56, K2Big>(p, tile_cfg)) return launch_cfg<K2FlatBig56>(p, L);
        if (cfg >= 2 && prefer_flat<K2FlatMed56, K2Med>(p, tile_cfg)) return launch_cfg<K2FlatMed56>(p, L);
        if (cfg == 1 && prefer_flat<K2FlatBig, K2Big>(p, tile_cfg)) return launch_cfg<K2FlatBig>(p, L);
        if (cfg >= 2 && prefer_flat<K2FlatMed, K2Med>(p, tile_cfg)) return launch_cfg<K2FlatMed>(p, L);
        if (cfg == 1 && auto_cfg && tile_workgroups<K2Big>(d) >= 512) return launch_planned<K2Big, K2Med>(p, d, L, 3, 3);
        if (cfg == 1) return launch_cfg<K2Big>(p, L);
        if (cfg == 2) return launch_cfg<K2Med>(p, L);
        return launch_cfg<K2Small>(p, L);
    }
    if (p.Cout <= 64) return launch_gl<K1M64GL, K1M64>(p, L);
    int cfg = tile_cfg;
    if (cfg <= 0 || cfg > 2) {
        cfg = (tile_workgroups<K1Big>(d) >= (scratch ? 96 : 512)) ? 1 : 2;
        if (p.Cin <= 256 && p.Cout >= 4 * p.Cin && tile_workgroups<K1Big>(d) < 2048) cfg = 2;
    }
    if (cfg == 1) return launch_gl<K1BigGL, K1Big>(p, L);
    return launch_gl<K1SmallGL, K1Small>(p, L);
}

int launch_conv3d_gn(const StemsegVolume& in, const float* packed_w, const float* bias, const StemsegVolume& out, int kt, int kh, int kw,
                     int tile_cfg, hipStream_t s, float* splitk_scratch, int64_t splitk_scratch_floats, const ConvEpilogue* epi, int groups,
                     float eps, float* stats, double* gn_scratch, int64_t stats_bs) {
    SS_CHECK_ARG(stats && gn_scratch && groups > 0 && out.C % groups == 0, "conv3d_gn: bad GroupNorm arguments");
    const int cpg = out.C / groups;
    const int64_t S = (int64_t)out.T * out.H * out.W;
    const bool dense = out.t_stride == (int64_t)out.H * out.W && out.y_stride == out.W && out.c_stride == S;
    const int64_t slot_bound = ceil_div(out.W, 32) * ceil_div(out.H, 2) * out.T + (int64_t)cpg * ceil_div(S, 256);
    if ((cpg != 4 && cpg != 8) || slot_bound > GN_SLOT_CAP || (epi && (epi->relu || epi->res || epi->dec_W > 0))) {
        SS_CHECK_ARG(dense, "conv3d_gn: the separate statistics pass needs a dense output");
        PlanSink* const sink = epi ? epi->plan_sink : nullptr;
        const int rec0 = sink ? sink->n : 0;
        int rc = launch_conv3d(in, packed_w, bias, out, kt, kh, kw, tile_cfg, s, splitk_scratch, splitk_scratch_floats, epi);
        if (sink) {
            for (int i = rec0; i < sink->n && i < sink->cap; ++i) sink->rec[i].gn = 3;
            return rc;
        }
        const int nb = (epi && epi->nb > 1) ? epi->nb : 1;
        for (int b = 0; b < nb && !rc; ++b)
            rc = launch_gn_stats(out.ptr + (nb > 1 ? b * epi->out_bs : 0), out.C, S, groups, eps, stats + (int64_t)b * stats_bs, gn_scratch + (nb > 1 ? b * epi->gn_bs : 0), s);
        return rc;
    }
    ConvEpilogue e = epi ? *epi : ConvEpilogue();
    int used = 0;
    e.gn_part = gn_scratch; e.gn_cpg = cpg; e.gn_cap = GN_SLOT_CAP; e.gn_used = &used;
    const int rc = launch_conv3d(in, packed_w, bias, out, kt, kh, kw, tile_cfg, s, splitk_scratch, splitk_scratch_floats, &e);
    if (rc || e.plan_sink) return rc;
    return launch_gn_finalize_slots(gn_scratch, groups, GN_SLOT_CAP, used, (double)cpg * (double)S, eps, stats, s, e.nb, e.gn_bs, stats_bs);
}

static ConvEpilogue epilogue_from_abi(const StemsegConvEpilogue* epilogue) {
    ConvEpilogue e;
    if (epilogue) {
        e.relu = epilogue->relu; e.res = epilogue->residual; e.res_cs = epilogue->res_c_stride; e.res_ts = epilogue->res_t_stride;
        e.res_ys = epilogue->res_y_stride; e.dec_H = epilogue->decode_H; e.dec_W = epilogue->decode_W;
        e.precision = epilogue->precision;
        e.frames = epilogue->frames; e.plan_frames = epilogue->plan_frames; e.plan_scratch_floats = epilogue->plan_scratch_floats;
    }
    return e;
}

}

extern "C" int64_t stemseg_hip_conv3d_gn_scratch_doubles(int32_t Cout, int32_t groups) {
    return (Cout > 0 && groups > 0) ? stemseg::gn_scratch_doubles(Cout, groups) : 0;
}

extern "C" int stemseg_hip_conv3d_gn(const StemsegVolume* in, const float* packed_w, const float* bias, const StemsegVolume* out,
                                     int32_t kt, int32_t kh, int32_t kw, int32_t tile_cfg, float* splitk_scratch, int64_t splitk_scratch_floats,
                                     int32_t precision, int32_t groups, float eps, float* stats, double* gn_scratch, void* stream) {
    using namespace stemseg;
    SS_CHECK_ARG(in && out, "conv3d_gn: null volume");
    ConvEpilogue e;
    e.precision = precision;
    return launch_conv3d_gn(*in, packed_w, bias, *out, kt, kh, kw, tile_cfg, as_stream(stream), splitk_scratch, splitk_scratch_floats, &e, groups,
                            eps, stats, gn_scratch);
}

extern "C" int stemseg_hip_conv3d(const StemsegVolume* in, const float* packed_w, const float* bias, const StemsegVolume* out,
                                  int32_t kt, int32_t kh, int32_t kw, int32_t tile_cfg, float* splitk_scratch,
                                  int64_t splitk_scratch_floats, const StemsegConvEpilogue* epilogue, void* stream) {
    using namespace stemseg;
    SS_CHECK_ARG(in && out, "conv3d: null volume");
    ConvEpilogue e = epilogue_from_abi(epilogue);
    return launch_conv3d(*in, packed_w, bias, *out, kt, kh, kw, tile_cfg, as_stream(stream), splitk_scratch, splitk_scratch_floats,
                         epilogue ? &e : nullptr);
}

static int conv3d_zero_t_halo(const StemsegVolume* in, const float* packed_w, const float* bias, const StemsegVolume* out, int32_t kt, int32_t kh,
                              int32_t kw, int32_t tile_cfg, float* splitk_scratch, int64_t splitk_scratch_floats, const StemsegConvEpilogue* epilogue,
                              int32_t groups, float eps, float* stats, double* gn_scratch, int32_t plan_clips, void* stream) {
    using namespace stemseg;
    SS_CHECK_ARG(in && out, "conv3d_zero_t_halo: null volume");
    SS_CHECK_ARG(kt == 3, "conv3d_zero_t_halo: the promise is about the temporal halo planes of a kernel with kt == 3 (got %d)", kt);
    ConvEpilogue e = epilogue_from_abi(epilogue);
    e.zero_t_halo = 1;
    e.plan_clips = plan_clips;
    if (stats)
        return launch_conv3d_gn(*in, packed_w, bias, *out, kt, kh, kw, tile_cfg, as_stream(stream), splitk_scratch, splitk_scratch_floats, &e, groups,
                                eps, stats, gn_scratch);
    return launch_conv3d(*in, packed_w, bias, *out, kt, kh, kw, tile_cfg, as_stream(stream), splitk_scratch, splitk_scratch_floats, &e);
}

extern "C" int stemseg_hip_conv3d_zero_t_halo(const StemsegVolume* in, const float* packed_w, const float* bias, const StemsegVolume* out,
                                              int32_t kt, int32_t kh, int32_t kw, int32_t tile_cfg, float* splitk_scratch,
                                              int64_t splitk_scratch_floats, const StemsegConvEpilogue* epilogue, int32_t groups, float eps,
                                              float* stats, double* gn_scratch, void* stream) {
    return conv3d_zero_t_halo(in, packed_w, bias, out, kt, kh, kw, tile_cfg, splitk_scratch, splitk_scratch_floats, epilogue, groups, eps, stats, gn_scratch, 0, stream);
}

extern "C" int stemseg_hip_conv3d_zero_t_halo_clips(const StemsegVolume* in, const float* packed_w, const float* bias, const StemsegVolume* out,
                                                    int32_t kt, int32_t kh, int32_t kw, int32_t tile_cfg, float* splitk_scratch,
                                                    int64_t splitk_scratch_floats, const StemsegConvEpilogue* epilogue, int32_t groups, float eps,
                                                    float* stats, double* gn_scratch, int32_t plan_clips, void* stream) {
    return conv3d_zero_t_halo(in, packed_w, bias, out, kt, kh, kw, tile_cfg, splitk_scratch, splitk_scratch_floats, epilogue, groups, eps, stats, gn_scratch, plan_clips,
                              stream);
}

extern "C" int stemseg_hip_conv3d_zero_t_halo_batch(const StemsegVolume* in, const float* packed_w, const float* bias, const StemsegVolume* out,
                                                    int32_t kt, int32_t kh, int32_t kw, int32_t tile_cfg, const StemsegConvEpilogue* epilogue,
                                                    int32_t n_clips, int64_t in_clip_stride, int64_t out_clip_stride, void* stream) {
    using namespace stemseg;
    SS_CHECK_ARG(in && out, "conv3d_zero_t_halo_batch: null volume");
    SS_CHECK_ARG(kt == 3, "conv3d_zero_t_halo: the promise is about the temporal halo planes of a kernel with kt == 3 (got %d)", kt);
    SS_CHECK_ARG(n_clips >= 1 && n_clips <= 4096 && in_clip_stride >= 0 && out_clip_stride >= 0, "conv3d_zero_t_halo_batch: n_clips=%d", n_clips);
    ConvEpilogue e = epilogue_from_abi(epilogue);
    e.zero_t_halo = 1;
    e.nb = n_clips; e.in_bs = in_clip_stride; e.out_bs = out_clip_stride;
    return launch_conv3d(*in, packed_w, bias, *out, kt, kh, kw, tile_cfg, as_stream(stream), nullptr, 0, &e);
}

static int conv3d_plan(const StemsegVolume* in, const float* bias, const StemsegVolume* out, int32_t kt, int32_t kh, int32_t kw, int32_t tile_cfg,
                       const float* splitk_scratch, int64_t splitk_scratch_floats, const StemsegConvEpilogue* epilogue, int32_t form,
                       int32_t gn_groups, int32_t plan_clips, StemsegConvPlanRecord* records, int32_t capacity, int32_t* count) {
    using namespace stemseg;
    SS_CHECK_ARG(in && out && count && capacity >= 0 && (records || capacity == 0), "conv3d_plan: null volume / record array");
    SS_CHECK_ARG((form & ~(STEMSEG_PLAN_GN | STEMSEG_PLAN_ZERO_T_HALO)) == 0, "conv3d_plan: form %d", form);
    alignas(16) static float no_weights[4];
    alignas(16) static double no_table[2];
    PlanSink sink{records, capacity, 0};
    ConvEpilogue e;
    const bool gn = (form & STEMSEG_PLAN_GN) != 0, zth = (form & STEMSEG_PLAN_ZERO_T_HALO) != 0;
    if (gn && !zth) e.precision = epilogue ? epilogue->precision : STEMSEG_PRECISION_F32;
    else e = epilogue_from_abi(epilogue);
    if (zth) {
        SS_CHECK_ARG(kt == 3, "conv3d_zero_t_halo: the promise is about the temporal halo planes of a kernel with kt == 3 (got %d)", kt);
        e.zero_t_halo = 1;
    }
    e.plan_sink = &sink;
    e.plan_clips = plan_clips;
    float* const scratch = const_cast<float*>(splitk_scratch);
    const int rc = gn ? launch_conv3d_gn(*in, no_weights, bias, *out, kt, kh, kw, tile_cfg, nullptr, scratch, splitk_scratch_floats, &e, gn_groups, 1e-5f,
                                         no_weights, no_table)
                      : launch_conv3d(*in, no_weights, bias, *out, kt, kh, kw, tile_cfg, nullptr, scratch, splitk_scratch_floats, &e);
    *count = sink.n;
    return rc;
}

extern "C" int stemseg_hip_conv3d_plan(const StemsegVolume* in, const float* bias, const StemsegVolume* out, int32_t kt, int32_t kh, int32_t kw,
                                       int32_t tile_cfg, const float* splitk_scratch, int64_t splitk_scratch_floats,
                                       const StemsegConvEpilogue* epilogue, int32_t form, int32_t gn_groups, StemsegConvPlanRecord* records,
                                       int32_t capacity, int32_t* count) {
    return conv3d_plan(in, bias, out, kt, kh, kw, tile_cfg, splitk_scratch, splitk_scratch_floats, epilogue, form, gn_groups, 0, records, capacity, count);
}

extern "C" int stemseg_hip_conv3d_plan_clips(const StemsegVolume* in, const float* bias, const StemsegVolume* out, int32_t kt, int32_t kh, int32_t kw,
                                             int32_t tile_cfg, const float* splitk_scratch, int64_t splitk_scratch_floats,
                                             const StemsegConvEpilogue* epilogue, int32_t form, int32_t gn_groups, int32_t plan_clips,
                                             StemsegConvPlanRecord* records, int32_t capacity, int32_t* count) {
    return conv3d_plan(in, bias, out, kt, kh, kw, tile_cfg, splitk_scratch, splitk_scratch_floats, epilogue, form, gn_groups, plan_clips, records, capacity, count);
}
```

### stem-seg_amd/csrc/conv_split_f16x3.hip

```cpp
#include "conv_split_family.h"

namespace stemseg {

template int launch_split_family<3>(ConvKParams& p, const ConvKParams& d, const LaunchCtx& L, int tile_cfg, bool k3, bool k2);

int launch_stem_f16x3(const ConvKParams& p, const LaunchCtx& L) { return launch_cfg<SplitTiles<3>::Y4Stem>(p, L.without_scratch()); }

}
```

### stem-seg_amd/csrc/conv_split_family.h

```cpp
#pragma once
#include "conv_igemm.h"

namespace stemseg {

template <int BFV>
struct SplitTiles {
    static constexpr int CK2 = split_chunk_channels(9, BFV);
    using Y3Big = ConvCfg<3, 3, 3, 4, 4, 2, 1, 8, 1, false, BFV>;
    using Y3Med = ConvCfg<3, 3, 3, 4, 2, 2, 2, 4, 1, false, BFV>;
    using Y3Small = ConvCfg<3, 3, 3, 4, 2, 1, 2, 4, 1, false, BFV>;
    using Y2Big = ConvCfg<1, 3, 3, CK2, 4, 2, 1, 8, 1, false, BFV>;
    using Y2Med = ConvCfg<1, 3, 3, CK2, 2, 2, 2, 2, 1, false, BFV>;
    using Y2Small = ConvCfg<1, 3, 3, CK2, 2, 1, 2, 2, 1, false, BFV>;
    using Y2M64 = ConvCfg<1, 3, 3, CK2, 2, 2, 1, 4, 1, false, BFV>;
    using Y1Big = ConvCfg<1, 1, 1, 32, 4, 2, 1, 4, 8, false, BFV>;
    using Y1Small = ConvCfg<1, 1, 1, 32, 2, 2, 2, 2, 4, false, BFV>;
    using Y1M64 = ConvCfg<1, 1, 1, 32, 2, 2, 1, 4, 8, false, BFV>;
    using Y1Wide = ConvCfg<1, 1, 1, 32, 4, 2, 2, 4, 8, false, BFV>;
    template <int PMAX> using Y2Flat = ConvCfg<1, 3, 3, CK2, 4, 2, 1, 8, 16, false, BFV, false, PMAX>;
    using Y4Stem = ConvCfg<1, 4, 4, 16, 2, 2, 1, 8, 1, false, BFV>;
    using Y3Blk = ConvCfg<3, 3, 3, 4, 4, 2, 1, 8, 3, false, BFV, false, 0, false, 5>;
    using Y2Blk = ConvCfg<1, 3, 3, CK2, 4, 2, 1, 8, 3, false, BFV, false, 0, false, 5>;
    using Y3Blk7 = ConvCfg<3, 3, 3, 4, 2, 2, 2, 4, 7, false, BFV, false, 0, false, 1>;
};

struct DeepTiles {
    using Y3Deep = ConvCfg<3, 3, 3, 4, 4, 2, 1, 8, 1, false, 3, false, 0, false, -1>;
};
template <class Deep>
static bool deep_tile_eligible(const ConvKParams& p, const ConvKParams& d, const LaunchCtx& L, bool k3) {
    if (!L.deep_tile || !k3 || !p.zero_t_halo || p.T != Deep::TD || d.T != Deep::TD || p.H % Deep::ROWS != 0 || p.W % Deep::TW != 0 || !p.vec4 || p.out_p16 || p.dec_W > 0) return false;
    ConvKParams q = p;
    q.T_all = q.T;
    return plan_ksplit<Deep>(q, L, 0, (int)ceil_div(p.Cin, Deep::CK)) == 1;
}

template <int BFV>
int launch_split_family(ConvKParams& p, const ConvKParams& d, const LaunchCtx& L, int tile_cfg, bool k3, bool k2) {
    float* const scratch = L.scratch;
    typedef SplitTiles<BFV> F;
    using Y3Big = typename F::Y3Big; using Y3Med = typename F::Y3Med; using Y3Small = typename F::Y3Small;
    using Y2Big = typename F::Y2Big; using Y2Med = typename F::Y2Med; using Y2Small = typename F::Y2Small; using Y2M64 = typename F::Y2M64;
    using Y1Small = typename F::Y1Small; using Y1Big = typename F::Y1Big; using Y1M64 = typename F::Y1M64; using Y1Wide = typename F::Y1Wide;
    const bool auto_cfg = tile_cfg <= 0 || tile_cfg > 3;
    int cfg = (auto_cfg || tile_cfg == 6) ? 0 : tile_cfg;
    if constexpr (BFV == 3) {
        const bool flat_ok = p.vec4 && p.dec_W == 0 && p.in_ys % 4 == 0 && p.W + 2 <= p.in_ys && p.in_ys <= 224 && p.Cout % 128 == 0;
        if (flat_ok && k2 && !p.gn_part && p.in_ts == (int64_t)p.in_H * p.in_ys && p.in_H == p.H + 2 &&
            (tile_cfg == 5 || (auto_cfg && tile_workgroups<Y2Big>(d) >= (scratch ? 96 : 384)))) {
            const double e2d = tile_efficiency<Y2Big>(p.H, p.W);
            const double efl = (double)d.T * p.H * p.W / (512.0 * ceil_div((int64_t)d.T * p.in_ts, 512));
            if (tile_cfg == 5 || (efl > 1.04 * e2d && p.in_ys <= 56)) {
                p.flat_t = 1;
                if (p.in_ys <= 56) return launch_cfg<typename F::template Y2Flat<56>>(p, L);
                if (p.in_ys <= 112) return launch_cfg<typename F::template Y2Flat<112>>(p, L);
                return launch_cfg<typename F::template Y2Flat<224>>(p, L);
            }
        }
    }
    if constexpr (BFV == 3) {
        if (deep_tile_eligible<DeepTiles::Y3Deep>(p, d, L, k3)) return launch_cfg<DeepTiles::Y3Deep>(p, L);
    }
    static_assert(F::Y2Blk::ROWS == F::Y3Blk::ROWS && F::Y2Blk::TW == F::Y3Blk::TW && Y2Big::ROWS == Y3Big::ROWS && Y2Big::TW == Y3Big::TW, "blk_gain: the 2-D and 3-D tiles cover the same positions");
    auto blk_gain = [&]() { return tile_efficiency<typename F::Y3Blk>(p.H, p.W) > 1.06 * tile_efficiency<Y3Big>(p.H, p.W); };
    if constexpr (BFV == 3) {
        if (k3 && p.vec4 && (tile_cfg == 6 || (auto_cfg && tile_workgroups<Y3Big>(d) >= 384 && tile_workgroups<typename F::Y3Blk>(d) >= 384 && blk_gain())))
            return launch_cfg<typename F::Y3Blk>(p, L);
        if (k2 && p.vec4 && p.Cout > 64 && (tile_cfg == 6 || (auto_cfg && tile_workgroups<Y2Big>(d) >= (scratch ? 96 : 384) && tile_workgroups<typename F::Y2Blk>(d) >= 384 && blk_gain())))
            return launch_cfg<typename F::Y2Blk>(p, L);
    }
    if (k3) {
        if (cfg == 0) cfg = tile_workgroups<Y3Big>(d) >= 384 ? 1 : (tile_workgroups<Y3Med>(d) >= (scratch ? 32 : 256) ? 2 : 3);
        if constexpr (BFV == 3) {
            const double e_b7 = tile_efficiency<typename F::Y3Blk7>(p.H, p.W), e_med = tile_efficiency<Y3Med>(p.H, p.W);
            if (p.vec4 && (tile_cfg == 7 || (auto_cfg && cfg == 2 && e_b7 > 1.06 * e_med)))
                return launch_cfg<typename F::Y3Blk7>(p, L);
        }
        if (cfg == 1) return launch_cfg<Y3Big>(p, L);
        if (cfg == 2) return launch_cfg<Y3Med>(p, L);
        return launch_cfg<Y3Small>(p, L);
    }
    if (k2) {
        if (p.Cout <= 64) return launch_cfg<Y2M64>(p, L);
        if (cfg == 0) {
            const int64_t need = scratch ? 96 : 384;
            cfg = tile_workgroups<Y2Big>(d) >= need ? 1 : (tile_workgroups<Y2Med>(d) >= need ? 2 : 3);
        }
        if (cfg == 1) return launch_cfg<Y2Big>(p, L);
        if (cfg == 2) return launch_cfg<Y2Med>(p, L);
        return launch_cfg<Y2Small>(p, L);
    }
    if (p.Cout <= 64) return launch_cfg<Y1M64>(p, L);
    if (tile_cfg == 3 && p.Cout % 256 == 0) return launch_cfg<Y1Wide>(p, L);
    if (auto_cfg && p.Cout % 256 == 0 && p.Cin >= p.Cout && !p.res && tile_workgroups<Y1Wide>(d) >= 128)
        return launch_cfg<Y1Wide>(p, L.without_scratch());
    if (cfg == 0 || cfg > 2) {
        if (BFV == 3) {
            cfg = 2;
        } else {
            cfg = (tile_workgroups<Y1Big>(d) >= (scratch ? 96 : 512)) ? 1 : 2;
            if (p.Cin <= 256 && p.Cout >= 4 * p.Cin && tile_workgroups<Y1Big>(d) < 2048) cfg = 2;
        }
    }
    if (cfg == 1) return launch_cfg<Y1Big>(p, L);
    return launch_cfg<Y1Small>(p, L);
}

}
```

### stem-seg_amd/stemseg_amd/hip.py

```python
import ctypes as C
import os

import torch

_HERE = os.path.dirname(os.path.abspath(__file__))
LIB_PATH = os.environ.get("STEMSEG_HIP_LIB") or os.path.join(_HERE, "lib", "libstemseg_hip.so")

MAX_INSTANCES = 64
MAX_EMB_DIMS = 8
ABI_VERSION = 11


class Volume(C.Structure):
    _fields_ = [("ptr", C.c_void_p), ("c_stride", C.c_int64), ("t_stride", C.c_int64), ("y_stride", C.c_int64),
                ("C", C.c_int32), ("T", C.c_int32), ("H", C.c_int32), ("W", C.c_int32), ("limit", C.c_int64)]


class DecoderDesc(C.Structure):
    _fields_ = [("struct_bytes", C.c_int32), ("in_channels", C.c_int32), ("inter", C.c_int32 * 4),
                ("T", C.c_int32), ("H4", C.c_int32), ("W4", C.c_int32), ("gn_groups", C.c_int32), ("gn_eps", C.c_float),
                ("pool", C.c_int32 * 3), ("t_scale", C.c_int32 * 3), ("n_out", C.c_int32),
                ("act", C.c_int32 * (2 * MAX_EMB_DIMS)), ("grid_axis", C.c_int32 * (2 * MAX_EMB_DIMS)),
                ("input_layout", C.c_int32), ("concurrency", C.c_int32), ("detached", C.c_int32), ("precision", C.c_int32),
                ("n_clips", C.c_int32), ("feat_clip_stride", C.c_int64 * 4), ("out_clip_stride", C.c_int64),
                ("plan_clips", C.c_int32),
                ("reserved", C.c_int32)]


class DecoderWeights(C.Structure):
    _fields_ = [("conv_w", C.c_void_p * 7), ("conv_b", C.c_void_p * 7), ("gn_w", C.c_void_p * 7), ("gn_b", C.c_void_p * 7),
                ("fuse_w", C.c_void_p * 3), ("head_w", C.c_void_p), ("head_b", C.c_void_p),
                ("grid_t", C.c_void_p), ("grid_y", C.c_void_p), ("grid_x", C.c_void_p)]


MAX_ENCODER_BLOCKS = 40


class ConvEpilogue(C.Structure):
    _fields_ = [("relu", C.c_int32), ("residual", C.c_void_p), ("res_c_stride", C.c_int64), ("res_t_stride", C.c_int64),
                ("res_y_stride", C.c_int64), ("decode_H", C.c_int32), ("decode_W", C.c_int32), ("precision", C.c_int32),
                ("frames", C.c_int32), ("plan_frames", C.c_int32), ("plan_scratch_floats", C.c_int64)]


class ConvPlanRecord(C.Structure):
    _fields_ = [(n, C.c_int32) for n in ("kt", "kh", "kw", "ck", "mt", "rows", "tw", "nt", "flat", "pmax", "gl", "blk", "threads", "precision",
                                         "ksplit", "chunks_per_split", "nchunks")] + [("grid", C.c_int32 * 3)] + \
               [(n, C.c_int32) for n in ("row0", "row1", "vec4", "vec_epi", "reduce", "gn", "zero_t_halo", "nb", "deep")]


class EncoderDesc(C.Structure):
    _fields_ = [("struct_bytes", C.c_int32), ("blocks", C.c_int32 * 4), ("T", C.c_int32), ("H", C.c_int32), ("W", C.c_int32),
                ("out_channels", C.c_int32), ("precision", C.c_int32), ("n_clips", C.c_int32), ("clip_frames", C.c_int32),
                ("clip_stride", C.c_int32), ("plan_frames", C.c_int32), ("fuse_tail", C.c_int32),
                ("conv2_groups", C.c_int32), ("width_per_group", C.c_int32), ("stride_in_3x3", C.c_int32)]


_BLK = C.c_void_p * MAX_ENCODER_BLOCKS


class EncoderWeights(C.Structure):
    _fields_ = [("stem_w", C.c_void_p), ("stem_b", C.c_void_p), ("stem_w_s2d", C.c_void_p),
                ("conv1_w", _BLK), ("conv1_b", _BLK), ("conv2_w", _BLK), ("conv2_b", _BLK), ("conv3_w", _BLK), ("conv3_b", _BLK),
                ("down_w", _BLK), ("down_b", _BLK),
                ("fpn_inner_w", C.c_void_p * 4), ("fpn_inner_b", C.c_void_p * 4), ("fpn_layer_w", C.c_void_p * 4), ("fpn_layer_b", C.c_void_p * 4)]


class ClusterParams(C.Structure):
    _fields_ = [("primary_prob_thresh", C.c_float), ("secondary_prob_thresh", C.c_float), ("min_seediness_prob", C.c_float),
                ("max_instances", C.c_int32), ("n_free_dims", C.c_int32), ("free_dim_bandwidths", C.c_float * MAX_EMB_DIMS)]


class ClusterMeta(C.Structure):
    _fields_ = [("K", C.c_int32), ("exhausted", C.c_int32), ("n_points", C.c_int64), ("n_unassigned_last", C.c_int64),
                ("centers", (C.c_float * MAX_EMB_DIMS) * MAX_INSTANCES), ("bandwidths", (C.c_float * MAX_EMB_DIMS) * MAX_INSTANCES),
                ("seed_prob", C.c_float * MAX_INSTANCES)]


class ClusterItem(C.Structure):
    _fields_ = [("emb", C.c_void_p), ("bw", C.c_void_p), ("seed", C.c_void_p), ("n_max", C.c_int64), ("n_points_dev", C.c_void_p),
                ("label_start", C.c_int64), ("labels", C.c_void_p), ("meta_dev", C.c_void_p), ("opt_masks", C.c_void_p), ("opt_probs", C.c_void_p),
                ("workspace", C.c_void_p), ("ws_bytes", C.c_size_t)]


class EmbeddingLossDesc(C.Structure):
    _fields_ = [("struct_bytes", C.c_int32), ("embedding_size", C.c_int32), ("n_free_dims", C.c_int32), ("n_instances", C.c_int32),
                ("T", C.c_int32), ("H", C.c_int32), ("W", C.c_int32), ("reserved", C.c_int32), ("free_dim_bandwidths", C.c_float * MAX_EMB_DIMS)]


class TargetPrepDesc(C.Structure):
    _fields_ = [("struct_bytes", C.c_int32), ("n_instances", C.c_int32), ("T", C.c_int32), ("H", C.c_int32), ("W", C.c_int32),
                ("reserved", C.c_int32)]


class SemsegLossDesc(C.Structure):
    _fields_ = [("struct_bytes", C.c_int32), ("n_classes", C.c_int32), ("has_foreground_channel", C.c_int32), ("T", C.c_int32),
                ("H", C.c_int32), ("W", C.c_int32), ("reserved", C.c_int32), ("reserved2", C.c_int32), ("stride_c", C.c_int64),
                ("stride_t", C.c_int64), ("stride_h", C.c_int64), ("stride_w", C.c_int64)]


class OptTensor(C.Structure):
    _fields_ = [("p", C.c_void_p), ("g", C.c_void_p), ("state1", C.c_void_p), ("state2", C.c_void_p), ("n", C.c_int64), ("flags", C.c_int32),
                ("reserved", C.c_int32)]


class OptChunk(C.Structure):
    _fields_ = [("tensor", C.c_int32), ("chunk", C.c_int32)]


class OptHyper(C.Structure):
    _fields_ = [("struct_bytes", C.c_int32), ("flags", C.c_int32), ("lr", C.c_float), ("momentum", C.c_float), ("one_minus_dampening", C.c_float),
                ("weight_decay", C.c_float), ("one_minus_beta1", C.c_float), ("beta2", C.c_float), ("one_minus_beta2", C.c_float), ("eps", C.c_float)]


_P, _I32, _I64, _F = C.c_void_p, C.c_int32, C.c_int64, C.c_float
SIGNATURES = {
    "stemseg_hip_version": (C.c_int, []),
    "stemseg_hip_last_error": (C.c_char_p, []),
    "stemseg_hip_device_count": (C.c_int, []),
    "stemseg_hip_profile_enable": (C.c_int, [_I32]),
    "stemseg_hip_profile_read": (C.c_int, [C.POINTER(C.c_double), _I32]),
    "stemseg_hip_padded_geometry": (C.c_int, [_I32, _I32, _I32, _I32, C.POINTER(_I64)]),
    "stemseg_hip_pack_conv_weight": (C.c_int, [_P, _P, _I32, _I32, _I32, _P]),
    "stemseg_hip_encoder_plan_offsets": (C.c_int, [_P, _P]),
    "stemseg_hip_encoder_stage_end_mask": (C.c_int, [_P, C.POINTER(_I32)]),
    "stemseg_hip_packed_weight_bytes_prec": (C.c_int64, [_I32, _I32, _I32, _I32]),
    "stemseg_hip_pack_conv_weight_prec": (C.c_int, [_P, _P, _I32, _I32, _I32, _I32, _P]),
    "stemseg_hip_conv3d": (C.c_int, [C.POINTER(Volume), _P, _P, C.POINTER(Volume), _I32, _I32, _I32, _I32, _P, _I64, C.POINTER(ConvEpilogue), _P]),
    "stemseg_hip_packed_grouped_weight_bytes": (C.c_int64, [_I32, _I32, _I32, _I32]),
    "stemseg_hip_pack_grouped_conv_weight": (C.c_int, [_P, _P, _I32, _I32, _I32, _I32, _P]),
    "stemseg_hip_conv2d_grouped": (C.c_int, [C.POINTER(Volume), _P, _P, C.POINTER(Volume), _I32, _I32, _I32, _I32, _I32, _P]),
    "stemseg_hip_conv3d_gn_scratch_doubles": (C.c_int64, [_I32, _I32]),
    "stemseg_hip_conv3d_plan": (C.c_int, [C.POINTER(Volume), _P, C.POINTER(Volume), _I32, _I32, _I32, _I32, _P, _I64, C.POINTER(ConvEpilogue), _I32, _I32,
                                          C.POINTER(ConvPlanRecord), _I32, C.POINTER(_I32)]),
    "stemseg_hip_conv3d_plan_clips": (C.c_int, [C.POINTER(Volume), _P, C.POINTER(Volume), _I32, _I32, _I32, _I32, _P, _I64, C.POINTER(ConvEpilogue), _I32, _I32,
                                                _I32, C.POINTER(ConvPlanRecord), _I32, C.POINTER(_I32)]),
    "stemseg_hip_conv3d_zero_t_halo": (C.c_int, [C.POINTER(Volume), _P, _P, C.POINTER(Volume), _I32, _I32, _I32, _I32, _P, _I64, C.POINTER(ConvEpilogue),
                                                _I32, _F, _P, _P, _P]),
    "stemseg_hip_conv3d_zero_t_halo_clips": (C.c_int, [C.POINTER(Volume), _P, _P, C.POINTER(Volume), _I32, _I32, _I32, _I32, _P, _I64, C.POINTER(ConvEpilogue),
                                                      _I32, _F, _P, _P, _I32, _P]),
    "stemseg_hip_conv3d_zero_t_halo_batch": (C.c_int, [C.POINTER(Volume), _P, _P, C.POINTER(Volume), _I32, _I32, _I32, _I32, C.POINTER(ConvEpilogue),
                                                      _I32, _I64, _I64, _P]),
    "stemseg_hip_conv3d_gn": (C.c_int, [C.POINTER(Volume), _P, _P, C.POINTER(Volume), _I32, _I32, _I32, _I32, _P, _I64, _I32, _I32, _F, _P, _P, _P]),
    "stemseg_hip_stem_conv": (C.c_int, [_P, _P, _P, _P, _I32, _I32, _I32, _P]),
    "stemseg_hip_maxpool3x3s2": (C.c_int, [_P, _I64, _I32, _I32, _P, _I32, C.POINTER(_I32), _P]),
    "stemseg_hip_encoder_subsample2": (C.c_int, [_P, _I64, _I32, _I32, _P, _I32, C.POINTER(_I32), _P]),
    "stemseg_hip_upsample2x_add": (C.c_int, [C.POINTER(Volume), _P, C.POINTER(Volume), _I32, C.POINTER(_I32), _P]),
    "stemseg_hip_stem_s2d": (C.c_int, [_P, _I32, _I32, _I32, C.POINTER(Volume), _P]),
    "stemseg_hip_encoder_stream_forms": (C.c_int, [C.POINTER(EncoderDesc), C.POINTER(_I32)]),
    "stemseg_hip_encoder_workspace_bytes": (C.c_size_t, [C.POINTER(EncoderDesc)]),
    "stemseg_hip_encoder_init_workspace": (C.c_int, [C.POINTER(EncoderDesc), _P, C.c_size_t, _P]),
    "stemseg_hip_encoder_check_workspace": (C.c_int, [C.POINTER(EncoderDesc), _P, C.c_size_t, C.POINTER(_I32), C.POINTER(_I64), _P]),
    "stemseg_hip_encoder_forward": (C.c_int, [C.POINTER(EncoderDesc), C.POINTER(EncoderWeights), _P, C.POINTER(Volume), _P, C.c_size_t, _P]),
    "stemseg_hip_encoder_stem_forward": (C.c_int, [C.POINTER(EncoderDesc), C.POINTER(EncoderWeights), _P, _P, _P, _P, C.c_size_t, _P]),
    "stemseg_hip_groupnorm_stats": (C.c_int, [_P, _I32, _I64, _I32, _F, _P, _P, _P]),
    "stemseg_hip_gn_relu_pool": (C.c_int, [_P, _I32, _I32, _I32, _I32, _I32, _P, _P, _P, _I32, C.POINTER(Volume), _P]),
    "stemseg_hip_upsample_trilinear": (C.c_int, [_P, _I32, _I32, _I32, _I32, _I32, _I32, _I32, C.POINTER(Volume), _P]),
    "stemseg_hip_copy_to_volume": (C.c_int, [_P, _I32, C.POINTER(Volume), _P]),
    "stemseg_hip_heads": (C.c_int, [_P, _I32, _I32, _I32, _I32, _P, _P, _I32, C.POINTER(_I32), C.POINTER(_I32), _P, _P, _P, _P, _P]),
    "stemseg_hip_nonfinite_flags": (C.c_int, [_P, _I64, _P, _I32, _P]),
    "stemseg_hip_decoder_workspace_bytes": (C.c_size_t, [C.POINTER(DecoderDesc)]),
    "stemseg_hip_decoder_init_workspace": (C.c_int, [C.POINTER(DecoderDesc), _P, C.c_size_t, _P]),
    "stemseg_hip_decoder_check_workspace": (C.c_int, [C.POINTER(DecoderDesc), _P, C.c_size_t, C.POINTER(_I32), C.POINTER(_I64), _P]),
    "stemseg_hip_decoder_forward": (C.c_int, [C.POINTER(DecoderDesc), C.POINTER(DecoderWeights), C.POINTER(_P), _P, _P, C.c_size_t, _P]),
    "stemseg_hip_decoder_join": (C.c_int, [_I32, _P]),
    "stemseg_hip_seediness_accumulate": (C.c_int, [_P, _P, _I64, _I32, _P]),
    "stemseg_hip_fg_mask": (C.c_int, [_P, _F, _F, _P, _I64, _P]),
    "stemseg_hip_fg_mask_frames": (C.c_int, [_P, _P, _F, _P, _I32, _I64, _P]),
    "stemseg_hip_fg_gather": (C.c_int, [_P, _P, _P, _P, _I32, _I32, _I32, _I64, _P, _P, _P, _P, _P, _P, _P]),
    "stemseg_hip_cluster_workspace_bytes": (C.c_size_t, [_I64]),
    "stemseg_hip_cluster": (C.c_int, [_P, _P, _P, _I64, _P, _I32, _I32, C.POINTER(ClusterParams), _I64, _P, _P, _P, _P, _P, C.c_size_t, _P]),
    "stemseg_hip_cluster_batch": (C.c_int, [C.POINTER(ClusterItem), _I32, _I32, _I32, C.POINTER(ClusterParams), _P]),
    "stemseg_hip_overlap_counts": (C.c_int, [_P, _P, _I64, _P, _I32, _P, _I32, _I32, _I32, _P, _P, _P, _P]),
    "stemseg_hip_label_presence": (C.c_int, [_P, _I64, _P, _I32, _P, _I32, _P]),
    "stemseg_hip_relabel": (C.c_int, [_P, _I64, _P, _I32, _P]),
    "stemseg_hip_fg_compact": (C.c_int, [_P, _I32, _I64, _P, _P, _P, _P]),
    "stemseg_hip_labels_to_codes": (C.c_int, [_P, _P, _P, _I64, _I64, _P, _I64, _P]),
    "stemseg_hip_pair_tables": (C.c_int, [_P, _P, _P, _I32, _I64, _I32, _P, _P]),
    "stemseg_hip_codes_to_labels": (C.c_int, [_P, _P, _P, _I32, _I64, _P, _I64, _I32, _P, _P]),
    "stemseg_hip_semseg_accumulate": (C.c_int, [_P, _P, _I32, _I32, _I64, C.POINTER(C.c_int32), _I32, _P]),
    "stemseg_hip_semseg_masks": (C.c_int, [_P, _P, _I32, _I32, _I64, _I32, _P, _P, _P]),
    "stemseg_hip_semseg_fg_clip": (C.c_int, [_P, _I32, _I32, _I64, _F, _P, _P, _P]),
    "stemseg_hip_preprocess_frames": (C.c_int, [_P, _I32, _I32, _I32, _I32, _I32, _I32, _I32, C.POINTER(C.c_float), C.POINTER(C.c_float), _I32, _I32, _P, _P]),
    "stemseg_hip_scatter_instance_index": (C.c_int, [_P, _P, _P, _I64, _P, _I32, _P, _I32, _I32, _P]),
    "stemseg_hip_resample_instance_masks": (C.c_int, [_P, _I32, _I32, C.c_float, _I32, _I32, _I32, _I32, _P, _P]),
    "stemseg_hip_scatter_instance_index_ex": (C.c_int, [_P, _P, _P, _I64, _P, _I32, _P, _I32, _I32, _I32, _P]),
    "stemseg_hip_resample_instance_masks_ex": (C.c_int, [_P, _I32, _I32, _I32, C.c_float, _I32, _I32, _I32, _I32, _P, _P]),
    "stemseg_hip_rle_workspace_bytes": (C.c_size_t, [_I32, _I32, _I32, _I32, _I64]),
    "stemseg_hip_rle_plan": (C.c_int, [_P, _I32, _I32, _I32, _I32, _I32, _I64, _P, C.c_size_t, _P, _P, _P, _P]),
    "stemseg_hip_rle_encode": (C.c_int, [_P, _I32, _I32, _I32, _I32, _I32, _I64, _P, C.c_size_t, _P, _P, _P, _P, _P, _P, _P]),
    "stemseg_hip_instance_class_stats": (C.c_int, [_P, _P, _P, _P, _I32, _I64, _P, _I32, _I32, _I32, _I32, _P, _I32, _P, _P, _P, _I32, _P, _P, _P]),
    "stemseg_hip_vis_composite": (C.c_int, [_P, _P, _I32, _I32, _I32, _I32, _P, _I32, _P, _P]),
    "stemseg_hip_jpeg_workspace_bytes": (C.c_size_t, [_I32, _I32, _I32]),
    "stemseg_hip_jpeg_plan": (C.c_int, [_P, _I32, _I32, _I32, _I32, _P, C.c_size_t, _P, _P, _P]),
    "stemseg_hip_jpeg_encode": (C.c_int, [_I32, _I32, _I32, _I32, _P, C.c_size_t, _P, _I64, _P, _P]),
    "stemseg_hip_jpeg_decode_workspace_bytes": (C.c_size_t, [_I32, _I32, _I32, _I32, _I64, _I64, _I32]),
    "stemseg_hip_jpeg_decode": (C.c_int, [_P, _P, _P, _I32, _I32, _I32, _I32, _I64, _I64, _I32, _I32, _P, C.c_size_t, _P, _P, _P]),
    "stemseg_hip_png_decode_workspace_bytes": (C.c_size_t, [_I32, _I32, _I32, _I32, _I64, _I32, _I32]),
    "stemseg_hip_png_decode": (C.c_int, [_P, _P, _P, _I32, _I32, _I32, _I32, _I64, _I32, _I32, _P, C.c_size_t, _P, _P, _P]),
    "stemseg_hip_embedding_loss_workspace_bytes": (C.c_size_t, [C.POINTER(EmbeddingLossDesc)]),
    "stemseg_hip_embedding_loss_forward": (C.c_int, [C.POINTER(EmbeddingLossDesc), _P, _P, _P, _P, C.c_size_t, _P, C.POINTER(_I32), _P]),
    "stemseg_hip_embedding_loss_backward": (C.c_int, [C.POINTER(EmbeddingLossDesc), _P, _P, _P, _P, C.c_size_t, _P, _I32, _I32, _P, _P]),
    "stemseg_hip_prepare_targets": (C.c_int, [C.POINTER(TargetPrepDesc), _P, _P, _P, _P, _P, _P, _P, _P]),
    "stemseg_hip_semseg_loss_workspace_bytes": (C.c_size_t, [C.POINTER(SemsegLossDesc)]),
    "stemseg_hip_semseg_loss_forward": (C.c_int, [C.POINTER(SemsegLossDesc), _P, _P, _P, _P, C.c_size_t, _P, _P, _P]),
    "stemseg_hip_semseg_loss_backward": (C.c_int, [C.POINTER(SemsegLossDesc), _P, _P, _P, _P, C.c_size_t, _P, _I32, _P, _P]),
    "stemseg_hip_level_head": (C.c_int, [_P, _I32, _I64, _P, _I32, _P, _P, _P]),
    "stemseg_hip_heads_backward_workspace_bytes": (C.c_size_t, [_I32, _I32, _I64]),
    "stemseg_hip_heads_backward": (C.c_int, [_P, _I32, _I32, _I32, _I32, _P, _P, _I32, C.POINTER(_I32), C.POINTER(_I32), _P, _P, _P, _P, _P, _P,
                                             _P, _P, _P, C.c_size_t, _P]),
    "stemseg_hip_wide_level_head": (C.c_int, [_P, _I32, _I64, _P, _I32, _P, _P, _P]),
    "stemseg_hip_wide_heads_backward_workspace_bytes": (C.c_size_t, [_I32, _I32, _I64]),
    "stemseg_hip_wide_heads_backward_chunks": (C.c_int, [_I32, _I32, _I64]),
    "stemseg_hip_wide_heads_backward": (C.c_int, [_P, _I32, _I64, _P, _I32, _P, _P, _P, _P, _P, C.c_size_t, _P]),
    "stemseg_hip_upsample_trilinear_backward": (C.c_int, [_P, _I32, _I32, _I32, _I32, _I32, _I32, _I32, _P, _P]),
    "stemseg_hip_gn_relu_pool_backward_workspace_bytes": (C.c_size_t, [_I32, _I32, _I32, _I32, _I32]),
    "stemseg_hip_gn_relu_pool_backward": (C.c_int, [_P, _I32, _I32, _I32, _I32, _I32, _P, _P, _P, _I32, _P, _P, _P, _P, _P, C.c_size_t, _P]),
    "stemseg_hip_conv3d_wgrad_workspace_bytes": (C.c_size_t, [_I32, _I32, _I32, _I32, _I32]),
    "stemseg_hip_conv3d_wgrad_chunks": (C.c_int, [_I32, _I32, _I32, _I32, _I32]),
    "stemseg_hip_conv3d_wgrad": (C.c_int, [C.POINTER(Volume), _P, _I32, _P, _P, _P, C.c_size_t, _P]),
    "stemseg_hip_conv3d_col2vol": (C.c_int, [_P, _I32, _I32, _I32, _I32, _P, _P]),
    "stemseg_hip_conv2d_wgrad_workspace_bytes": (C.c_size_t, [_I32, _I32, _I32, _I32, _I32, _I32]),
    "stemseg_hip_conv2d_wgrad_chunks": (C.c_int, [_I32, _I32, _I32, _I32, _I32, _I32]),
    "stemseg_hip_conv2d_wgrad": (C.c_int, [C.POINTER(Volume), _P, _I32, _I32, _P, _P, _P, C.c_size_t, _P]),
    "stemseg_hip_conv2d_col2img": (C.c_int, [_P, _I32, _I32, _I32, _I32, _P, _P, _P]),
    "stemseg_hip_conv2d_grouped_wgrad_workspace_bytes": (C.c_size_t, [_I32, _I32, _I32, _I32, _I32, _I32]),
    "stemseg_hip_conv2d_grouped_wgrad_chunks": (C.c_int, [_I32, _I32, _I32, _I32, _I32, _I32]),
    "stemseg_hip_conv2d_grouped_wgrad": (C.c_int, [C.POINTER(Volume), _P, _I32, _I32, _I32, _P, _P, C.c_size_t, _P]),
    "stemseg_hip_relu_backward": (C.c_int, [C.POINTER(Volume), _P, _P, _P, _P]),
    "stemseg_hip_conv2d_col2img_relu": (C.c_int, [_P, _I32, _I32, _I32, _I32, _P, C.POINTER(Volume), _P, _P]),
    "stemseg_hip_subsample2": (C.c_int, [_P, _I32, _I32, _I32, _I32, _P, _P]),
    "stemseg_hip_scatter2": (C.c_int, [_P, _I32, _I32, _I32, _I32, _P, _P, _P]),
    "stemseg_hip_scale_rows": (C.c_int, [_P, _P, _I32, _I64, _P]),
    "stemseg_hip_sum_partials": (C.c_int, [_P, _I32, _I64, _P, _P, _P]),
    "stemseg_hip_maxpool3x3s2_backward": (C.c_int, [_P, _P, _I64, _I32, _I32, _I32, _P, _I32, C.POINTER(_I32), _P]),
    "stemseg_hip_stem_wgrad_workspace_bytes": (C.c_size_t, [_I32, _I32, _I32]),
    "stemseg_hip_stem_wgrad_chunks": (C.c_int, [_I32, _I32, _I32]),
    "stemseg_hip_stem_wgrad": (C.c_int, [_P, _P, _I32, _I32, _I32, _P, _P, C.c_size_t, _P]),
    "stemseg_hip_opt_plan": (C.c_int, [C.POINTER(OptTensor), _I32, _I32, C.POINTER(OptChunk), _I64, C.POINTER(_I64)]),
    "stemseg_hip_opt_sgd_step": (C.c_int, [_P, _I32, _P, _I64, C.POINTER(OptHyper), _P, _P]),
    "stemseg_hip_opt_adam_step": (C.c_int, [_P, _I32, _P, _I64, C.POINTER(OptHyper), _P, _P, _P]),
    "stemseg_hip_opt_grad_norm": (C.c_int, [_P, _I32, _P, _I64, _P, _P, C.c_double, _P, _P, _P, _P]),
    "stemseg_hip_opt_bucket_plan": (C.c_int, [C.POINTER(OptTensor), _I32, C.POINTER(_I64), C.POINTER(_I64)]),
    "stemseg_hip_opt_pack_grads": (C.c_int, [_P, _I32, _P, _I64, _P, _P, _I64, C.c_float, _P]),
    "stemseg_hip_opt_unpack_grads": (C.c_int, [_P, _I32, _P, _I64, _P, _P, _I64, _P]),
    "stemseg_hip_opt_reduce_ranks": (C.c_int, [_P, _I32, _I64, _P, _P]),
    "stemseg_hip_rle_decode_workspace_bytes": (C.c_size_t, [_I64, _I32, _I32]),
    "stemseg_hip_rle_decode": (C.c_int, [_P, _I64, _P, _P, _P, _P, _I32, _I32, _I32, _I32, _P, C.c_size_t, _P, _P, _P]),
    "stemseg_hip_rle_decode_union_workspace_bytes": (C.c_size_t, [_I64, _I32, _I32]),
    "stemseg_hip_rle_decode_union": (C.c_int, [_P, _I64, _P, _P, _P, _P, _I32, _I32, _I32, _I32, _P, C.c_size_t, _P, _P, _P]),
    "stemseg_hip_rle_decode_labels_workspace_bytes": (C.c_size_t, [_I64, _I32, _I32]),
    "stemseg_hip_rle_decode_labels": (C.c_int, [_P, _I64, _P, _P, _P, _P, _P, _P, _I32, _I32, _I32, _I32, _P, C.c_size_t, _P, _P, _P, _P]),
    "stemseg_hip_rle_pair_inter_workspace_bytes": (C.c_size_t, [_I64, _I32, _I32]),
    "stemseg_hip_rle_pair_inter": (C.c_int, [_P, _I64, _P, _P, _P, _P, _I32, _I32, _I32, _I32, _P, C.c_size_t, _P, _P, _P, _P]),
    "stemseg_hip_resize_masks": (C.c_int, [_P, _I32, _I32, _I32, _I32, _I32, _I32, _I32, _P, _I32, _I32, _P, _P]),
    "stemseg_hip_warp_clip": (C.c_int, [_P, _P, _I32, _I32, _I32, _P, _P, _I32, _P, _P, _P, _P]),
    "stemseg_hip_motion_blur": (C.c_int, [_P, _I32, _I32, _I32, _P, _P, _P, _P]),
    "stemseg_hip_duplicate_instance": (C.c_int, [_P, _P, _I32, _I32, _I32, _P, _P, _P, _P]),
    "stemseg_hip_preprocess_frames_masked": (C.c_int, [_P, _P, _I32, _I32, _I32, _I32, _I32, _I32, _I32, C.POINTER(C.c_float), C.POINTER(C.c_float), _I32,
                                                       _I32, _P, _P]),
    "stemseg_hip_davis_eval_counts_size": (_I64, [_I32, _I32, _I32]),
    "stemseg_hip_davis_eval_counts": (C.c_int, [_P, _I32, _P, _I32, _I32, _I32, _I32, _I32, _I32, _P, _I64, _P]),
    "stemseg_hip_label_pair_counts_size": (_I64, [_I32, _I32, _I32]),
    "stemseg_hip_label_pair_counts": (C.c_int, [_P, _P, _I32, _I32, _I32, _I32, _I32, _P, _I64, _P]),
}

SEMSEG_OUTPUT_TYPES = {None: 0, "none": 0, "logits": 1, "probs": 2, "argmax": 3}

_lib = None


def lib():
    global _lib
    if _lib is None:
        if not os.path.exists(LIB_PATH):
            raise RuntimeError("libstemseg_hip.so not found at %s -- build it with `python stem-seg_amd/build.py` "
                               "(hipcc --offload-arch=gfx950); the hot path has no CPU fallback" % LIB_PATH)
        l = C.CDLL(LIB_PATH)
        for name, (res, args) in SIGNATURES.items():
            fn = getattr(l, name)
            fn.restype, fn.argtypes = res, args
        v = l.stemseg_hip_version()
        if v != ABI_VERSION:
            raise RuntimeError("libstemseg_hip.so ABI version %d != binding %d" % (v, ABI_VERSION))
        _lib = l
    return _lib


def require_gpu():
    l = lib()
# ... 50 lines not shown

def dense_volume(t):
    Cn, T, H, W = t.shape
    return Volume(t.data_ptr(), T * H * W, H * W, W, Cn, T, H, W, t.numel())


def flat_volume(t):
    Cn, V = t.shape[0], t[0].numel()
    return Volume(t.data_ptr(), V, 0, 0, Cn, 1, 1, V, t.numel())


def alloc_padded(Cn, T, H, W, device="cuda"):
    g = padded_geometry(Cn, T, H, W)
    return torch.zeros(g["total"], dtype=torch.float32, device=device), g


def alloc_padded_batch(n, Cn, T, H, W, device="cuda"):
    g = padded_geometry(Cn, T, H, W)
    stride = (g["total"] + 63) // 64 * 64
    whole = torch.zeros(n * stride, dtype=torch.float32, device=device)
    return [whole[c * stride:c * stride + g["total"]] for c in range(n)], g, stride


def padded_halo_view(buf, g, Cn, T, H, W):
    return Volume(buf.data_ptr(), g["cs"], g["ts"], g["pitch"], Cn, T + 2, H + 2, W + 2, g["total"])


def padded_interior_view(buf, g, Cn, T, H, W):
    return Volume(buf.data_ptr() + 4 * g["interior"], g["cs"], g["ts"], g["pitch"], Cn, T, H, W, g["total"] - g["interior"])


def padded_to_dense(buf, g, Cn, T, H, W):
    v = buf[:Cn * g["cs"]].view(Cn, T + 2, H + 2, g["pitch"])
    return v[:, 1:T + 1, 1:H + 1, 1:W + 1].contiguous()


def pack_conv_weight(w):
    w = w.contiguous()
    Cout, Cin = w.shape[0], w.shape[1]
    taps = w[0, 0].numel()
    out = torch.empty(Cout * Cin * taps, dtype=torch.float32, device=w.device)
    check(lib().stemseg_hip_pack_conv_weight(ptr(w, torch.float32), ptr(out), Cout, Cin, taps, stream()))
    return out


PRECISIONS = {"f32": 0, "bf16x6": 2, "f16x3": 3}
PRECISION_INFO = {
    "f32": dict(operand_significand_bits=24, products_per_fp32_product=1, mfma="v_mfma_f32_32x32x2_f32", exponent_range="fp32"),
    "bf16x6": dict(operand_significand_bits=24, products_per_fp32_product=6, mfma="v_mfma_f32_32x32x16_bf16", exponent_range="fp32"),
    "f16x3": dict(operand_significand_bits=22, products_per_fp32_product=3, mfma="v_mfma_f32_32x32x16_f16",
                  exponent_range="2.5e-4 <= |activation| < 2.6e5 at full width; beyond: non-finite output, flagged, re-run in bf16x6"),
}
DEFAULT_PRECISION = os.environ.get("STEMSEG_PRECISION", "f16x3")
assert DEFAULT_PRECISION in PRECISIONS, DEFAULT_PRECISION


def pack_conv_weight_any(w, precision="f32"):
    if precision == "f32":
        return pack_conv_weight(w)
    assert precision in ("bf16x6", "f16x3"), precision
    code = PRECISIONS[precision]
    w = w.contiguous()
    Cout, Cin = w.shape[0], w.shape[1]
    taps = w[0, 0].numel()
    nbytes = lib().stemseg_hip_packed_weight_bytes_prec(Cout, Cin, taps, code)
    if nbytes <= 0:
        raise ValueError("pack_conv_weight_any: unsupported shape / precision (%s, Cout %d, Cin %d, taps %d)" % (precision, Cout, Cin, taps))
    out = torch.empty(nbytes // 4, dtype=torch.float32, device=w.device)
    check(lib().stemseg_hip_pack_conv_weight_prec(ptr(w, torch.float32), ptr(out), Cout, Cin, taps, code, stream()))
    return out


def pack_grouped_conv_weight(w, groups, precision="f32"):
    w = w.contiguous()
    Cout, Cin_g = w.shape[0], w.shape[1]
    code = PRECISIONS[precision]
    nbytes = lib().stemseg_hip_packed_grouped_weight_bytes(Cout, Cin_g, groups, code)
    if nbytes <= 0 or tuple(w.shape[2:]) != (3, 3):
        raise ValueError("pack_grouped_conv_weight: unsupported shape / precision (%s, %s, %d groups)" % (precision, tuple(w.shape), groups))
    out = torch.empty(nbytes // 4, dtype=torch.float32, device=w.device)
    check(lib().stemseg_hip_pack_grouped_conv_weight(ptr(w, torch.float32), ptr(out), Cout, Cin_g, groups, code, stream()))
    return out


def conv2d_grouped(vin, packed_w, bias, vout, groups, stride=1, relu=False, precision="f32", plan_frames=0):
    check(lib().stemseg_hip_conv2d_grouped(C.byref(vin), ptr(packed_w), ptr(bias), C.byref(vout), int(groups), int(stride), int(bool(relu)),
                                           PRECISIONS[precision], int(plan_frames), stream()))


def stem_conv(frames, w, bias):
    require_gpu()
    T, _, H, W = frames.shape
    out = torch.empty(64, T, H // 2, W // 2, dtype=torch.float32, device=frames.device)
    wt = w.reshape(64, 147).t().contiguous()
    check(lib().stemseg_hip_stem_conv(ptr(frames.contiguous(), torch.float32), ptr(wt, torch.float32), ptr(bias.contiguous(), torch.float32), ptr(out), T, H, W, stream()))
    return out


STREAM_FORM_SCALAR, STREAM_FORM_VEC4 = 1, 2
UP2_FORM_SCALAR, UP2_FORM_VEC4X2, UP2_FORM_DENSE = 1, 2, 3


def _stride2_pass(fn, x, out, form):
    if x.dim() != 3:
        raise ValueError("x %s must be [planes, H, W]" % (tuple(x.shape),))
    planes, H, W = x.shape
    if out is None:
        out = torch.empty(planes, H // 2, W // 2, dtype=torch.float32, device=x.device)
    used = _I32(0)
    check(fn(ptr(x, torch.float32), planes, H, W, ptr(out, torch.float32), int(form), C.byref(used), stream()))
    return out, used.value


def maxpool3x3s2(x, out=None, form=0):
    return _stride2_pass(lib().stemseg_hip_maxpool3x3s2, x, out, form)


def encoder_subsample2(x, out=None, form=0):
    return _stride2_pass(lib().stemseg_hip_encoder_subsample2, x, out, form)


def upsample2x_add(fine, coarse, fine_dense=None, form=0):
    used = _I32(0)
    check(lib().stemseg_hip_upsample2x_add(C.byref(fine), ptr(fine_dense, torch.float32), C.byref(coarse), int(form), C.byref(used), stream()))
    return used.value


def stem_s2d(frames, s2d):
    T, _, H, W = frames.shape
    check(lib().stemseg_hip_stem_s2d(ptr(frames, torch.float32), T, H, W, C.byref(s2d), stream()))


def encoder_stream_forms(desc):
    out = (_I32 * 7)()
    check(lib().stemseg_hip_encoder_stream_forms(C.byref(desc), out))
    return list(out)


def _conv_epilogue(epilogue):
    if epilogue is None:
        return None
    e = ConvEpilogue()
    e.relu = int(epilogue.get("relu", 0))
    r = epilogue.get("residual")
    if r is not None:
        e.residual = r if isinstance(r, int) else r.data_ptr()
        e.res_c_stride, e.res_t_stride, e.res_y_stride = epilogue["res_strides"]
    e.decode_H, e.decode_W = epilogue.get("decode", (0, 0))
    e.precision = PRECISIONS[epilogue.get("precision", "f32")]
    e.frames, e.plan_frames, e.plan_scratch_floats = epilogue.get("plan", (0, 0, 0))
    return e


PLAN_GN, PLAN_ZERO_T_HALO = 1, 2
TILE_CFG_DEEP = 8
PLAN_REDUCE_FORMS = {0: None, 1: "vec16", 2: "scalar"}
PLAN_GN_FORMS = {0: None, 1: "tile epilogue", 2: "split-K reduce", 3: "separate pass"}


def conv3d_plan(vin, vout, k, tile_cfg=0, scratch=None, epilogue=None, bias=1 << 20, gn_groups=0, zero_t_halo=False, plan_clips=0):
    kt, kh, kw = (k, k, k) if isinstance(k, int) else k
    e = _conv_epilogue(epilogue)
    form = (PLAN_GN if gn_groups > 0 else 0) | (PLAN_ZERO_T_HALO if zero_t_halo else 0)
    addr, floats = scratch if scratch is not None else (None, 0)
    cap = 4
    rec, count = (ConvPlanRecord * cap)(), _I32(0)
    check(lib().stemseg_hip_conv3d_plan_clips(C.byref(vin), C.c_void_p(bias) if bias else None, C.byref(vout), kt, kh, kw, tile_cfg,
                                              C.c_void_p(addr) if addr else None, floats, C.byref(e) if e is not None else None, form, int(gn_groups),
                                              int(plan_clips), rec, cap, C.byref(count)))
    assert count.value <= cap, count.value
    out = []
    for r in rec[:count.value]:
        d = {n: getattr(r, n) for n, _ in ConvPlanRecord._fields_ if n != "grid"}
        d["grid"] = tuple(r.grid)
        d["precision"] = {v: n for n, v in PRECISIONS.items()}[r.precision]
        d["reduce"], d["gn"] = PLAN_REDUCE_FORMS[r.reduce], PLAN_GN_FORMS[r.gn]
        out.append(d)
    return out


def conv3d(vin, packed_w, bias, vout, k, tile_cfg=0, splitk_scratch=None, epilogue=None):
    n = 0 if splitk_scratch is None else splitk_scratch.numel()
    kt, kh, kw = (k, k, k) if isinstance(k, int) else k
    e = _conv_epilogue(epilogue)
    check(lib().stemseg_hip_conv3d(C.byref(vin), ptr(packed_w), ptr(bias), C.byref(vout), kt, kh, kw, tile_cfg,
                                   ptr(splitk_scratch), n, C.byref(e) if e is not None else None, stream()))


def conv3d_zero_t_halo(vin, packed_w, bias, vout, k=3, tile_cfg=0, splitk_scratch=None, precision="f32", gn_groups=0, eps=1e-5, plan_clips=0):
    n = 0 if splitk_scratch is None else splitk_scratch.numel()
    kt, kh, kw = (k, k, k) if isinstance(k, int) else k
    e = ConvEpilogue()
    e.precision = PRECISIONS[precision]
    stats = scratch = None
    if gn_groups > 0:
        stats = torch.empty(2 * gn_groups, dtype=torch.float32, device=packed_w.device)
        scratch = torch.empty(lib().stemseg_hip_conv3d_gn_scratch_doubles(vout.C, gn_groups), dtype=torch.float64, device=packed_w.device)
    check(lib().stemseg_hip_conv3d_zero_t_halo_clips(C.byref(vin), ptr(packed_w), ptr(bias), C.byref(vout), kt, kh, kw, tile_cfg, ptr(splitk_scratch), n,
                                                     C.byref(e), int(gn_groups), eps, ptr(stats), ptr(scratch), int(plan_clips), stream()))
    return stats


def conv3d_zero_t_halo_batch(vin, packed_w, bias, vout, n_clips, in_clip_stride, out_clip_stride, tile_cfg=0, precision="f32"):
    e = ConvEpilogue()
    e.precision = PRECISIONS[precision]
    check(lib().stemseg_hip_conv3d_zero_t_halo_batch(C.byref(vin), ptr(packed_w), ptr(bias), C.byref(vout), 3, 3, 3, tile_cfg, C.byref(e), int(n_clips),
                                                     int(in_clip_stride), int(out_clip_stride), stream()))


def conv3d_gn(vin, packed_w, bias, vout, k, groups, eps=1e-5, tile_cfg=0, splitk_scratch=None, precision="f32"):
    n = 0 if splitk_scratch is None else splitk_scratch.numel()
    kt, kh, kw = (k, k, k) if isinstance(k, int) else k
    dev = packed_w.device
    stats = torch.empty(2 * groups, dtype=torch.float32, device=dev)
    scratch = torch.empty(lib().stemseg_hip_conv3d_gn_scratch_doubles(vout.C, groups), dtype=torch.float64, device=dev)
    check(lib().stemseg_hip_conv3d_gn(C.byref(vin), ptr(packed_w), ptr(bias), C.byref(vout), kt, kh, kw, tile_cfg, ptr(splitk_scratch), n,
                                      PRECISIONS[precision], groups, eps, ptr(stats), ptr(scratch), stream()))
    return stats


def groupnorm_stats(x, groups, eps=1e-5):
    Cn = x.shape[0]
    S = x[0].numel()
    stats = torch.empty(2 * groups, dtype=torch.float32, device=x.device)
    scratch = torch.empty(groups * 128, dtype=torch.float64, device=x.device)
    check(lib().stemseg_hip_groupnorm_stats(ptr(x, torch.float32), Cn, S, groups, eps, ptr(stats), ptr(scratch), stream()))
    return stats


def gn_relu_pool(x, groups, stats, gamma, beta, pool, vout):
    Cn, T, H, W = x.shape
    check(lib().stemseg_hip_gn_relu_pool(ptr(x, torch.float32), Cn, T, H, W, groups, ptr(stats), ptr(gamma), ptr(beta),
                                         int(pool), C.byref(vout), stream()))


def upsample_trilinear(x, st, sy, sx, vout=None):
    Cn, T, H, W = x.shape
    out = None
    if vout is None:
        out = torch.empty(Cn, T * st, H * sy, W * sx, dtype=torch.float32, device=x.device)
        vout = dense_volume(out)
    check(lib().stemseg_hip_upsample_trilinear(ptr(x, torch.float32), Cn, T, H, W, st, sy, sx, C.byref(vout), stream()))
    return out


def copy_to_volume(x, layout, vout):
    check(lib().stemseg_hip_copy_to_volume(ptr(x, torch.float32), layout, C.byref(vout), stream()))


def heads(x, w, bias, act, grid_axis, gt, gy, gx):
    Cin, T, H, W = x.shape
    n_out = w.shape[0]
    out = torch.empty(n_out, T, H, W, dtype=torch.float32, device=x.device)
    a = (C.c_int32 * n_out)(*act)
    g = (C.c_int32 * n_out)(*grid_axis)
    check(lib().stemseg_hip_heads(ptr(x, torch.float32), Cin, T, H, W, ptr(w.contiguous()), ptr(bias), n_out, a, g,
                                  ptr(gt), ptr(gy), ptr(gx), ptr(out), stream()))
    return out


def level_head(x, w, add=None):
    Cin, V = x.shape[0], x[0].numel()
    n_out = w.shape[0]
    out = torch.empty((n_out,) + tuple(x.shape[1:]), dtype=torch.float32, device=x.device)
    check(lib().stemseg_hip_level_head(ptr(x, torch.float32), Cin, V, ptr(w, torch.float32), n_out, ptr(add), ptr(out), stream()))
    return out


def _workspace(nbytes, what, device):
    if nbytes == 0:
        raise RuntimeError("%s: %s" % (what, lib().stemseg_hip_last_error().decode()))
    return torch.empty(nbytes, dtype=torch.uint8, device=device)


def heads_backward(x, w, d_out, out=None, act=None, grid_axis=None, gt=None, gy=None, gx=None, want_dx=True, want_db=True):
    Cin, T, H, W = x.shape
    n_out = w.shape[0]
    dev = x.device
    ws = _workspace(lib().stemseg_hip_heads_backward_workspace_bytes(Cin, n_out, T * H * W), "heads_backward", dev)
    dx = torch.empty_like(x) if want_dx else None
    dw = torch.empty(n_out, Cin, dtype=torch.float32, device=dev)
    db = torch.empty(n_out, dtype=torch.float32, device=dev) if want_db else None
    a = g = None
    if act is not None:
        a, g = (C.c_int32 * n_out)(*act), (C.c_int32 * n_out)(*grid_axis)
    check(lib().stemseg_hip_heads_backward(ptr(x, torch.float32), Cin, T, H, W, ptr(w, torch.float32), None, n_out, a, g, ptr(gt), ptr(gy), ptr(gx),
                                           ptr(out), ptr(d_out, torch.float32), ptr(dx), ptr(dw), ptr(db), ptr(ws), ws.numel(), stream()))
    return dx, dw, db


def wide_level_head(x, w, add=None):
    Cin, V = x.shape[0], x[0].numel()
    n_out = w.shape[0]
    out = torch.empty((n_out,) + tuple(x.shape[1:]), dtype=torch.float32, device=x.device)
    check(lib().stemseg_hip_wide_level_head(ptr(x, torch.float32), Cin, V, ptr(w, torch.float32), n_out, ptr(add), ptr(out), stream()))
    return out


def wide_heads_backward_chunks(Cin, n_out, V):
    n = lib().stemseg_hip_wide_heads_backward_chunks(Cin, n_out, V)
    if n == 0:
        raise RuntimeError("wide_heads_backward: %s" % lib().stemseg_hip_last_error().decode())
    return n


def wide_heads_backward(x, w, dz, want_dx=True, want_db=False):
    Cin, V = x.shape[0], x[0].numel()
    n_out = w.shape[0]
    dev = x.device
    ws = _workspace(lib().stemseg_hip_wide_heads_backward_workspace_bytes(Cin, n_out, V), "wide_heads_backward", dev)
    dx = torch.empty_like(x) if want_dx else None
    dw = torch.empty(n_out, Cin, dtype=torch.float32, device=dev)
    db = torch.empty(n_out, dtype=torch.float32, device=dev) if want_db else None
    check(lib().stemseg_hip_wide_heads_backward(ptr(x, torch.float32), Cin, V, ptr(w, torch.float32), n_out, ptr(dz, torch.float32), ptr(dx), ptr(dw),
                                                ptr(db), ptr(ws), ws.numel(), stream()))
    return dx, dw, db


def upsample_trilinear_backward(d_out, st, sy, sx):
    Cn, To, Ho, Wo = d_out.shape
    if To % st or Ho % sy or Wo % sx:
        raise ValueError("upsample_trilinear_backward: %s is no multiple of the scale (%d, %d, %d)" % (tuple(d_out.shape), st, sy, sx))
    d_in = torch.empty(Cn, To // st, Ho // sy, Wo // sx, dtype=torch.float32, device=d_out.device)
    check(lib().stemseg_hip_upsample_trilinear_backward(ptr(d_out, torch.float32), Cn, To // st, Ho // sy, Wo // sx, st, sy, sx, ptr(d_in), stream()))
    return d_in


def gn_relu_pool_backward(x, groups, stats, gamma, beta, pool, d_out):
    Cn, T, H, W = x.shape
    dev = x.device
    dx = torch.empty_like(x)
# ... 1462 lines not shown
```

Before: 127.7.

## Map flat f16x3 conv tiles over dense output pixels instead of padded pitch

For flat-tile f16x3 convs with temporal kernel 1, output columns are now indexed over dense H*W pixels rather than the padded pitch layout. Each tile stages a variable input run covering its pixels' neighbourhoods, with a fixed LDS capacity and a host-side check that the worst run fits. This removes the MMA work and staging spent on padding columns and rows, and makes the flat path look more efficient in tile selection. The cost is extra index division per lane, variable-length staging loops with a spill-over direct-stage pass, and a larger LDS footprint. It also adds pair-plane and plan API plumbing.

```diff
diff --git a/include/stemseg_hip.h b/include/stemseg_hip.h
--- a/include/stemseg_hip.h
+++ b/include/stemseg_hip.h
@@ -89,9 +89,11 @@
     int32_t zero_t_halo;
     int32_t nb;
     int32_t deep;
+    int32_t flat_dense;
 } StemsegConvPlanRecord;
 #define STEMSEG_PLAN_GN          1
 #define STEMSEG_PLAN_ZERO_T_HALO 2
+#define STEMSEG_PLAN_PAIR_PLANES 4
 int stemseg_hip_conv3d_plan(const StemsegVolume* in, const float* bias, const StemsegVolume* out, int32_t kt, int32_t kh, int32_t kw,
                             int32_t tile_cfg, const float* splitk_scratch, int64_t splitk_scratch_floats,
                             const StemsegConvEpilogue* epilogue, int32_t form, int32_t gn_groups, StemsegConvPlanRecord* records,
@@ -100,6 +102,11 @@
                                   int32_t tile_cfg, const float* splitk_scratch, int64_t splitk_scratch_floats,
                                   const StemsegConvEpilogue* epilogue, int32_t form, int32_t gn_groups, int32_t plan_clips,
                                   StemsegConvPlanRecord* records, int32_t capacity, int32_t* count);
+int stemseg_hip_conv3d_pair_planes(const StemsegVolume* in, const float* packed_w, const float* bias, const StemsegVolume* out,
+                                   int32_t kt, int32_t kh, int32_t kw, int32_t tile_cfg, float* splitk_scratch, int64_t splitk_scratch_floats,
+                                   const StemsegConvEpilogue* epilogue, uint32_t* planes, int32_t* wrote_planes, void* stream);
+int64_t stemseg_hip_flat_dense_run_max(int32_t H, int32_t W, int64_t pitch, int64_t frame_stride, int32_t nt);
+int32_t stemseg_hip_flat_dense_capacity(int64_t pitch);
 
 int64_t stemseg_hip_packed_grouped_weight_bytes(int32_t Cout, int32_t Cin_g, int32_t groups, int32_t precision);
 int stemseg_hip_pack_grouped_conv_weight(const float* w, void* packed, int32_t Cout, int32_t Cin_g, int32_t groups, int32_t precision, void* stream);
diff --git a/stem-seg_amd/csrc/conv_igemm.h b/stem-seg_amd/csrc/conv_igemm.h
--- a/stem-seg_amd/csrc/conv_igemm.h
+++ b/stem-seg_amd/csrc/conv_igemm.h
@@ -39,6 +39,7 @@
     int zero_t_halo;
     int64_t in_bs, out_bs, gn_bs;
     unsigned int* out_p16;
+    int fd_dense, fd_W, fd_HW, fd_org, fd_N;
 };
 
 template <int KT_, int KH_, int KW_, int CK_, int MI_, int NI_, int WM_, int WN_, int COLS_, bool PIPE_ = false, int BF_ = 0, bool DB_ = false,
@@ -65,9 +66,12 @@
     static constexpr int XL = (TW + KW - 1 + 3) / 4;
     static constexpr int XP = DEEP ? 24 : (BLK ? ((4 * XL + 23) / 32) * 32 + 8 : 4 * XL);
     static constexpr int NT = NSEG * 32;
-    static constexpr int FL = NT + 2 * PMAX + 8;
+    static constexpr bool FDM = PMAX_ > 0 && BF_ == 3 && KT_ == 1;
+    static constexpr int FL_RUN = WN_ * NI_ * 32 + 2 * PMAX_ + 8;
+    static constexpr int FL = (FDM && PMAX_ <= 56) ? 1168 : FL_RUN;
+    static constexpr int FL_REG = (FDM && ((FL_RUN + 255) / 256) * 256 < FL) ? ((FL_RUN + 255) / 256) * 256 : FL;
     static constexpr int IN_CH_STRIDE = FLAT ? KT * FL : KT * RH * XP;
-    static constexpr int IN_PAIR_STRIDE = PMAX_ > 0 ? KT * (WN_ * NI_ * 32 + 2 * PMAX_ + 8) : TPL * RH * XP;
+    static constexpr int IN_PAIR_STRIDE = PMAX_ > 0 ? KT * FL : TPL * RH * XP;
     static constexpr int IN_PLANE_STRIDE = (CK / 2) * IN_PAIR_STRIDE;
     static constexpr int IN_FLOATS = X6 ? NPX * IN_PLANE_STRIDE : CK * IN_CH_STRIDE;
     static constexpr SplitLayout SL = SplitLayout(TAPS, BF_, CK_);
@@ -147,6 +151,16 @@
     const int pitch = (int)p.in_ys;
     const int F0 = pitch + tx * C::NT;
     const int co0 = co_tile * C::MT;
+    auto fd_word = [&](const int n) __attribute__((always_inline)) {
+        const int nc = min(n, p.fd_N - 1), fr = nc / p.fd_HW, r = nc - fr * p.fd_HW, yy = r / p.fd_W;
+        return fr * (int)p.in_ts + yy * pitch + (r - yy * p.fd_W) + p.fd_org;
+    };
+    int fd_R0 = 0, fd_rq = 1;
+    if constexpr (C::FDM) {
+        const int n0 = __builtin_amdgcn_readfirstlane(tx * C::NT);
+        fd_R0 = (fd_word(n0) - pitch - 1) & ~3;
+        fd_rq = min((fd_word(n0 + C::NT - 1) + pitch + 1 - fd_R0) / 4 + 1, C::FL / 4);
+    }
 
     f32x16 acc[C::MI][C::NI];
 #pragma unroll
@@ -172,6 +186,8 @@
         b_ptr6[ni] = C::FLAT ? reinterpret_cast<const unsigned int*>(in_lds) + half * (C::CPH / 2) * C::IN_PAIR_STRIDE + s * 32 + l31 + 3
                              : reinterpret_cast<const unsigned int*>(in_lds) + half * (C::CPH / 2) * C::IN_PAIR_STRIDE + seg_row(min(s, C::NLIVE - 1), l31) * C::XP + seg_col(min(s, C::NLIVE - 1), l31);
         if constexpr (C::DEEP) b_ptr6[ni] += wn * (C::RH * C::XP);
+        if constexpr (C::FDM)
+            b_ptr6[ni] = reinterpret_cast<const unsigned int*>(in_lds) + half * (C::CPH / 2) * C::IN_PAIR_STRIDE + (fd_word(tx * C::NT + s * 32 + l31) - pitch - 1 - fd_R0);
     }
     const float* in_tile = p.in + (int64_t)blockIdx.y * p.in_bs + (int64_t)t * p.in_ts + x0;
     const int64_t tile_base = (int64_t)t * p.in_ts + x0;
@@ -292,7 +308,10 @@
         else split_bf16x3(x, sh, sm, sl);
         h = sh; m = sm; l = sl;
     };
-    constexpr int FQ6 = C::FL / 4;
+    constexpr int FQ6 = C::FL_REG / 4;
+    static_assert(C::FL % 4 == 0 && C::FL_REG % 4 == 0 && C::FL_REG <= C::FL, "flat tiles: the staged run is whole 16-byte pieces");
+    const int fd_nq = C::FDM ? (C::CK / 2) * fd_rq : 0;
+    auto fd_lds = [&](const int q) __attribute__((always_inline)) { const int pr = q / fd_rq; return pr * C::IN_PAIR_STRIDE + (q - pr * fd_rq) * 4; };
     constexpr int XL6 = C::XL;
     constexpr int NQ6 = C::FLAT ? (C::CK / 2) * C::KT * FQ6 : (C::CK / 2) * (C::DEEP ? C::TD : C::KT) * C::RH * XL6;
     auto in6_lds = [](const int q) __attribute__((always_inline)) {
@@ -302,7 +321,11 @@
     constexpr int IN_PT6 = C::X6 ? (NQ6 + C::NTHREADS - 1) / C::NTHREADS : 1;
     constexpr int NWQ_A = C::NPL * C::GA * 2 * C::MT, NWQ6 = C::NPL * C::G * 2 * C::MT;
     auto in6_rel = [&](int q, int& c) -> int64_t {
-        if constexpr (C::FLAT) {
+        if constexpr (C::FDM) {
+            const int pr = q / fd_rq;
+            c = 2 * pr;
+            return (int64_t)c * p.in_cs + fd_R0 + 4 * (q - pr * fd_rq);
+        } else if constexpr (C::FLAT) {
             const int j4 = q % FQ6, rr = q / FQ6, dt = rr % C::KT;
             c = 2 * (rr / C::KT);
             const int f = F0 - pitch - 4 + 4 * j4;
@@ -335,11 +358,17 @@
     constexpr int NQ6V = TV ? (C::CK / 2) * 2 * R6 : NQ6;
     constexpr int IN_PT6V = TV ? (NQ6V + C::NTHREADS - 1) / C::NTHREADS : IN_PT6;
     auto in6_live = [](const int qv, const int first) __attribute__((always_inline)) { return qv + (qv / (2 * R6)) * R6 + (first ? R6 : 0); };
+    int in6_loff[C::FDM ? IN_PT6 : 1];
     if constexpr (C::X6) {
 #pragma unroll
         for (int k = 0; k < IN_PT6; ++k) {
             int q = tid + k * C::NTHREADS;
             bool inside = q < NQ6;
+            if constexpr (C::FDM) {
+                inside = inside && q < fd_nq;
+                q = inside ? q : 0;
+                in6_loff[k] = fd_lds(q);
+            }
             if constexpr (TV && !C::DEEP) {
                 if (tvar) { inside = q < NQ6V; q = inside ? in6_live(q, tvar == 1) : 0; }
             }
@@ -359,13 +388,13 @@
         v0 = *reinterpret_cast<const f32x4*>(base + (c0 < in6_clim[k] ? in6_voff[k] : 0u));
         v1 = *reinterpret_cast<const f32x4*>(base + (c0 + 1 < in6_clim[k] ? in6_voff[k] + cs4 : 0u));
     };
-    auto store_in6 = [&](int q, const float4& v0, const float4& v1) {
+    auto store_in6 = [&](int w, const float4& v0, const float4& v1) {
         unsigned int h0, m0, l0, h1, m1, l1;
         uint4 ph, pm, pl;
         if constexpr (C::F16) {
             split_pair_f16(v0.x, v1.x, ph.x, pm.x); split_pair_f16(v0.y, v1.y, ph.y, pm.y);
             split_pair_f16(v0.z, v1.z, ph.z, pm.z); split_pair_f16(v0.w, v1.w, ph.w, pm.w);
-            unsigned int* d16 = reinterpret_cast<unsigned int*>(in_lds) + in6_lds(q);
+            unsigned int* d16 = reinterpret_cast<unsigned int*>(in_lds) + w;
             *reinterpret_cast<uint4*>(d16) = ph;
             *reinterpret_cast<uint4*>(d16 + C::IN_PLANE_STRIDE) = pm;
             return;
@@ -374,24 +403,30 @@
         split3(v0.y, h0, m0, l0); split3(v1.y, h1, m1, l1); ph.y = h0 | (h1 << 16); pm.y = m0 | (m1 << 16); pl.y = l0 | (l1 << 16);
         split3(v0.z, h0, m0, l0); split3(v1.z, h1, m1, l1); ph.z = h0 | (h1 << 16); pm.z = m0 | (m1 << 16); pl.z = l0 | (l1 << 16);
         split3(v0.w, h0, m0, l0); split3(v1.w, h1, m1, l1); ph.w = h0 | (h1 << 16); pm.w = m0 | (m1 << 16); pl.w = l0 | (l1 << 16);
-        unsigned int* d = reinterpret_cast<unsigned int*>(in_lds) + in6_lds(q);
+        unsigned int* d = reinterpret_cast<unsigned int*>(in_lds) + w;
         *reinterpret_cast<uint4*>(d) = ph;
         *reinterpret_cast<uint4*>(d + C::IN_PLANE_STRIDE) = pm;
         if constexpr (C::NPX == 3) *reinterpret_cast<uint4*>(d + 2 * C::IN_PLANE_STRIDE) = pl;
     };
-    auto store_in6_masked = [&](int c0, int k, int q, const f32x4& r0, const f32x4& r1) __attribute__((always_inline)) {
+    auto store_in6_masked = [&](int c0, int k, int w, const f32x4& r0, const f32x4& r1) __attribute__((always_inline)) {
         const bool ok0 = c0 < in6_clim[k], ok1 = c0 + 1 < in6_clim[k];
         float4 v0, v1;
         v0.x = ok0 ? r0.x : 0.f; v0.y = ok0 ? r0.y : 0.f; v0.z = ok0 ? r0.z : 0.f; v0.w = ok0 ? r0.w : 0.f;
         v1.x = ok1 ? r1.x : 0.f; v1.y = ok1 ? r1.y : 0.f; v1.z = ok1 ? r1.z : 0.f; v1.w = ok1 ? r1.w : 0.f;
-        store_in6(q, v0, v1);
-    };
-    auto stage_in6_direct = [&](int c0) {
-        if (p.vec4) {
+        store_in6(w, v0, v1);
+    };
+    auto stage_in6_direct = [&](int c0, const int q_first = 0) {
+        if constexpr (C::FDM) {
+            for (int q = q_first + tid; q < fd_nq; q += C::NTHREADS) {
+                float4 v0, v1;
+                fetch_in6(c0, q, v0, v1);
+                store_in6(fd_lds(q), v0, v1);
+            }
+        } else if (p.vec4) {
             for (int q = tid; q < NQ6; q += C::NTHREADS) {
                 float4 v0, v1;
                 fetch_in6(c0, q, v0, v1);
-                store_in6(q, v0, v1);
+                store_in6(in6_lds(q), v0, v1);
             }
         } else if constexpr (!C::FLAT && !C::DEEP) {
             constexpr int NE6 = (C::CK / 2) * C::KT * C::RH * C::XP;
@@ -580,8 +615,10 @@
 #pragma unroll
                 for (int k = 0; k < PTV; ++k) {
                     const int q = tid + k * C::NTHREADS;
-                    if ((k + 1) * C::NTHREADS <= NQV || q < NQV) store_in6_masked(c0, k, V ? in6_live(q, V == 1) : q, rin[2 * k], rin[2 * k + 1]);
-                }
+                    if constexpr (C::FDM) { if (q < fd_nq) store_in6_masked(c0, k, in6_loff[k], rin[2 * k], rin[2 * k + 1]); }
+                    else if ((k + 1) * C::NTHREADS <= NQV || q < NQV) store_in6_masked(c0, k, in6_lds(V ? in6_live(q, V == 1) : q), rin[2 * k], rin[2 * k + 1]);
+                }
+                if constexpr (C::FDM && C::FL_REG < C::FL) stage_in6_direct(c0, IN_PT6 * C::NTHREADS);
             } else stage_in6_direct(c0);
         };
         auto side_items = [&](const int st, auto nspread_c, auto n_in_c, auto n_w_c, auto&& f_in, auto&& f_w) __attribute__((always_inline)) {
@@ -919,14 +956,22 @@
         int x = x0 + seg_col(s, l31);
         int te = t_out;
         if constexpr (C::FLAT) {
-            int f = F0 + s * 32 + l31;
-            if (p.flat_t) {
-                te = f / (int)p.in_ts;
-                f -= te * (int)p.in_ts;
-            }
-            const int y1 = f / pitch, x1 = f - y1 * pitch;
-            y = (y1 >= 1 && te < p.T_all) ? y1 - 1 : p.H;
-            x = (x1 >= 1) ? x1 - 1 : p.W;
+            if constexpr (C::FDM) {
+                const int n = tx * C::NT + s * 32 + l31;
+                te = n / p.fd_HW;
+                const int r = n - te * p.fd_HW, yy = r / p.fd_W, x1 = r - yy * p.fd_W + (p.fd_org - pitch);
+                y = n < p.fd_N ? yy : p.H;
+                x = (x1 >= 1) ? x1 - 1 : p.W;
+            } else {
+                int f = F0 + s * 32 + l31;
+                if (p.flat_t) {
+                    te = f / (int)p.in_ts;
+                    f -= te * (int)p.in_ts;
+                }
+                const int y1 = f / pitch, x1 = f - y1 * pitch;
+                y = (y1 >= 1 && te < p.T_all) ? y1 - 1 : p.H;
+                x = (x1 >= 1) ? x1 - 1 : p.W;
+            }
         }
         if (y < p.H && x < p.W) {
             int64_t off, roff = 0;
@@ -1019,12 +1064,25 @@
     LaunchCtx without_plan() const { return LaunchCtx{s, scratch, scratch_floats, nullptr, p16_keep_plan, sink, plan_clips, deep_tile}; }
 };
 
+static int64_t flat_dense_run_max(int H, int W, int64_t pitch, int64_t in_ts, int NT) {
+    const int64_t HW = (int64_t)H * W;
+    auto word = [&](int64_t n) { const int64_t f = n / HW, r = n % HW; return f * in_ts + (r / W + 1) * pitch + r % W + 1; };
+    int64_t g = HW, b = NT;
+    while (b) { const int64_t t = g % b; g = b; b = t; }
+    int64_t worst = 0;
+    for (int64_t k = 0; k < HW / g; ++k) {
+        const int64_t r0 = (word(k * NT) - pitch - 1) / 4 * 4;
+        worst = std::max(worst, ((word(k * NT + NT - 1) + pitch + 1 - r0) / 4 + 1) * 4);
+    }
+    return worst;
+}
+
 template <class C>
-static int64_t tile_workgroups(const ConvKParams& d, int flat_t = 0) {
+static int64_t tile_workgroups(const ConvKParams& d, int flat_t = 0, int dense = 0) {
     int64_t tx = C::FLAT ? ceil_div((int64_t)d.H * d.in_ys, C::NT) : ceil_div(d.W, C::TW);
     const int64_t ty = C::FLAT ? 1 : ceil_div(d.H, C::ROWS);
     int64_t T = ceil_div(d.T, C::TD);
-    if (C::FLAT && flat_t) { tx = ceil_div((int64_t)d.T * d.in_ts, C::NT); T = 1; }
+    if (C::FLAT && flat_t) { tx = ceil_div(dense ? (int64_t)d.T * d.H * d.W : (int64_t)d.T * d.in_ts, C::NT); T = 1; }
     return tx * ty * T * ceil_div(d.Cout, C::MT);
 }
 
@@ -1061,6 +1119,16 @@
         p.T = 1;
     }
     p.flat_t = flat_t;
+    if constexpr (C::FDM) {
+        SS_CHECK_ARG(flat_t && (int64_t)p.T_all * p.in_ts < (1ll << 31) && p.in_ys <= C::PMAX, "conv3d: flat tile on %d frames of pitch %lld", p.T_all, (long long)p.in_ys);
+        p.fd_dense = p.fd_dense ? 1 : 0;
+        SS_CHECK_ARG(!p.fd_dense || flat_dense_run_max(p.H, p.W, p.in_ys, p.in_ts, C::NT) <= C::FL, "conv3d: the dense flat run of a %d x %d map does not fit the tile", p.H, p.W);
+        p.fd_W = p.fd_dense ? p.W : (int)p.in_ys;
+        p.fd_HW = p.fd_dense ? p.H * p.W : (int)p.in_ts;
+        p.fd_org = (int)p.in_ys + p.fd_dense;
+        p.fd_N = p.T_all * p.fd_HW;
+        p.tiles_x = (int)ceil_div((int64_t)p.fd_N, C::NT);
+    } else p.fd_dense = 0;
     const int out_vec = p.vec_epi;
     if (C::FLAT) p.vec_epi = 0;
     const int nchunks = (int)ceil_div(p.Cin, C::CK);
@@ -1122,6 +1190,7 @@
             r.gn = ksplit > 1 ? (rp.gn_part ? 2 : 0) : (p.gn_part ? 1 : 0);
             r.zero_t_halo = p.zero_t_halo; r.nb = p.nb;
             r.deep = C::DEEP ? C::TD : 0;
+            r.flat_dense = p.fd_dense;
         }
         ++k.n;
         return STEMSEG_OK;
diff --git a/stem-seg_amd/csrc/conv_igemm.hip b/stem-seg_amd/csrc/conv_igemm.hip
--- a/stem-seg_amd/csrc/conv_igemm.hip
+++ b/stem-seg_amd/csrc/conv_igemm.hip
@@ -155,6 +155,7 @@
     p.tiles_x = p.tiles_y = 0;
     p.t_fastest = 1;
     p.flat_t = 0; p.T_all = p.T;
+    p.fd_dense = p.fd_W = p.fd_HW = p.fd_org = p.fd_N = 0;
     const bool aligned = (reinterpret_cast<uintptr_t>(in.ptr) % 16 == 0) && (in.c_stride % 4 == 0) &&
                          (in.T == 1 || in.t_stride % 4 == 0) && (in.H == 1 || in.y_stride % 4 == 0);
     p.vec4 = aligned ? 1 : 0;
@@ -300,6 +301,20 @@
                          epilogue ? &e : nullptr);
 }
 
+extern "C" int stemseg_hip_conv3d_pair_planes(const StemsegVolume* in, const float* packed_w, const float* bias, const StemsegVolume* out,
+                                              int32_t kt, int32_t kh, int32_t kw, int32_t tile_cfg, float* splitk_scratch,
+                                              int64_t splitk_scratch_floats, const StemsegConvEpilogue* epilogue, uint32_t* planes,
+                                              int32_t* wrote_planes, void* stream) {
+    using namespace stemseg;
+    SS_CHECK_ARG(in && out && planes && wrote_planes, "conv3d_pair_planes: null volume / planes");
+    ConvEpilogue e = epilogue_from_abi(epilogue);
+    int done = 0;
+    e.p16_out = planes; e.p16_done = &done;
+    const int rc = launch_conv3d(*in, packed_w, bias, *out, kt, kh, kw, tile_cfg, as_stream(stream), splitk_scratch, splitk_scratch_floats, &e);
+    *wrote_planes = done;
+    return rc;
+}
+
 static int conv3d_zero_t_halo(const StemsegVolume* in, const float* packed_w, const float* bias, const StemsegVolume* out, int32_t kt, int32_t kh,
                               int32_t kw, int32_t tile_cfg, float* splitk_scratch, int64_t splitk_scratch_floats, const StemsegConvEpilogue* epilogue,
                               int32_t groups, float eps, float* stats, double* gn_scratch, int32_t plan_clips, void* stream) {
@@ -348,7 +363,7 @@
                        int32_t gn_groups, int32_t plan_clips, StemsegConvPlanRecord* records, int32_t capacity, int32_t* count) {
     using namespace stemseg;
     SS_CHECK_ARG(in && out && count && capacity >= 0 && (records || capacity == 0), "conv3d_plan: null volume / record array");
-    SS_CHECK_ARG((form & ~(STEMSEG_PLAN_GN | STEMSEG_PLAN_ZERO_T_HALO)) == 0, "conv3d_plan: form %d", form);
+    SS_CHECK_ARG((form & ~(STEMSEG_PLAN_GN | STEMSEG_PLAN_ZERO_T_HALO | STEMSEG_PLAN_PAIR_PLANES)) == 0, "conv3d_plan: form %d", form);
     alignas(16) static float no_weights[4];
     alignas(16) static double no_table[2];
     PlanSink sink{records, capacity, 0};
@@ -362,6 +377,9 @@
     }
     e.plan_sink = &sink;
     e.plan_clips = plan_clips;
+    alignas(16) static unsigned int no_planes[4];
+    int p16_done = 0;
+    if (form & STEMSEG_PLAN_PAIR_PLANES) { e.p16_out = no_planes; e.p16_done = &p16_done; }
     float* const scratch = const_cast<float*>(splitk_scratch);
     const int rc = gn ? launch_conv3d_gn(*in, no_weights, bias, *out, kt, kh, kw, tile_cfg, nullptr, scratch, splitk_scratch_floats, &e, gn_groups, 1e-5f,
                                          no_weights, no_table)
diff --git a/stem-seg_amd/csrc/conv_split_f16x3.hip b/stem-seg_amd/csrc/conv_split_f16x3.hip
--- a/stem-seg_amd/csrc/conv_split_f16x3.hip
+++ b/stem-seg_amd/csrc/conv_split_f16x3.hip
@@ -7,3 +7,9 @@
 int launch_stem_f16x3(const ConvKParams& p, const LaunchCtx& L) { return launch_cfg<SplitTiles<3>::Y4Stem>(p, L.without_scratch()); }
 
 }
+
+extern "C" int64_t stemseg_hip_flat_dense_run_max(int32_t H, int32_t W, int64_t pitch, int64_t frame_stride, int32_t nt) {
+    if (H < 1 || W < 1 || nt < 1 || pitch < W + 2 || frame_stride < (int64_t)(H + 2) * pitch) return -1;
+    return stemseg::flat_dense_run_max(H, W, pitch, frame_stride, nt);
+}
+extern "C" int32_t stemseg_hip_flat_dense_capacity(int64_t pitch) { return stemseg::flat_dense_capacity(pitch); }
diff --git a/stem-seg_amd/csrc/conv_split_family.h b/stem-seg_amd/csrc/conv_split_family.h
--- a/stem-seg_amd/csrc/conv_split_family.h
+++ b/stem-seg_amd/csrc/conv_split_family.h
@@ -35,6 +35,11 @@
     return plan_ksplit<Deep>(q, L, 0, (int)ceil_div(p.Cin, Deep::CK)) == 1;
 }
 
+static int flat_dense_capacity(int64_t pitch) {
+    typedef SplitTiles<3> F3;
+    return pitch <= 56 ? F3::Y2Flat<56>::FL : (pitch <= 112 ? F3::Y2Flat<112>::FL : (pitch <= 224 ? F3::Y2Flat<224>::FL : 0));
+}
+
 template <int BFV>
 int launch_split_family(ConvKParams& p, const ConvKParams& d, const LaunchCtx& L, int tile_cfg, bool k3, bool k2) {
     float* const scratch = L.scratch;
@@ -48,10 +53,12 @@
         const bool flat_ok = p.vec4 && p.dec_W == 0 && p.in_ys % 4 == 0 && p.W + 2 <= p.in_ys && p.in_ys <= 224 && p.Cout % 128 == 0;
         if (flat_ok && k2 && !p.gn_part && p.in_ts == (int64_t)p.in_H * p.in_ys && p.in_H == p.H + 2 &&
             (tile_cfg == 5 || (auto_cfg && tile_workgroups<Y2Big>(d) >= (scratch ? 96 : 384)))) {
+            const bool dense = flat_dense_run_max(p.H, p.W, p.in_ys, p.in_ts, 512) <= flat_dense_capacity(p.in_ys);
             const double e2d = tile_efficiency<Y2Big>(p.H, p.W);
-            const double efl = (double)d.T * p.H * p.W / (512.0 * ceil_div((int64_t)d.T * p.in_ts, 512));
+            const double efl = (double)d.T * p.H * p.W / (512.0 * ceil_div(dense ? (int64_t)d.T * p.H * p.W : (int64_t)d.T * p.in_ts, 512));
             if (tile_cfg == 5 || (efl > 1.04 * e2d && p.in_ys <= 56)) {
                 p.flat_t = 1;
+                p.fd_dense = dense ? 1 : 0;
                 if (p.in_ys <= 56) return launch_cfg<typename F::template Y2Flat<56>>(p, L);
                 if (p.in_ys <= 112) return launch_cfg<typename F::template Y2Flat<112>>(p, L);
                 return launch_cfg<typename F::template Y2Flat<224>>(p, L);
diff --git a/stem-seg_amd/stemseg_amd/hip.py b/stem-seg_amd/stemseg_amd/hip.py
--- a/stem-seg_amd/stemseg_amd/hip.py
+++ b/stem-seg_amd/stemseg_amd/hip.py
@@ -45,7 +45,7 @@
 class ConvPlanRecord(C.Structure):
     _fields_ = [(n, C.c_int32) for n in ("kt", "kh", "kw", "ck", "mt", "rows", "tw", "nt", "flat", "pmax", "gl", "blk", "threads", "precision",
                                          "ksplit", "chunks_per_split", "nchunks")] + [("grid", C.c_int32 * 3)] + \
-               [(n, C.c_int32) for n in ("row0", "row1", "vec4", "vec_epi", "reduce", "gn", "zero_t_halo", "nb", "deep")]
+               [(n, C.c_int32) for n in ("row0", "row1", "vec4", "vec_epi", "reduce", "gn", "zero_t_halo", "nb", "deep", "flat_dense")]
 
 
 class EncoderDesc(C.Structure):
@@ -134,7 +134,11 @@
                                           C.POINTER(ConvPlanRecord), _I32, C.POINTER(_I32)]),
     "stemseg_hip_conv3d_plan_clips": (C.c_int, [C.POINTER(Volume), _P, C.POINTER(Volume), _I32, _I32, _I32, _I32, _P, _I64, C.POINTER(ConvEpilogue), _I32, _I32,
                                                 _I32, C.POINTER(ConvPlanRecord), _I32, C.POINTER(_I32)]),
-    "stemseg_hip_conv3d_zero_t_halo": (C.c_int, [C.POINTER(Volume), _P, _P, C.POINTER(Volume), _I32, _I32, _I32, _I32, _P, _I64, C.POINTER(ConvEpilogue),
+    "stemseg_hip_conv3d_pair_planes": (C.c_int, [C.POINTER(Volume), _P, _P, C.POINTER(Volume), _I32, _I32, _I32, _I32, _P, _I64, C.POINTER(ConvEpilogue), _P,
+                                                 C.POINTER(_I32), _P]),
+    "stemseg_hip_flat_dense_run_max":(C.c_int64, [_I32, _I32, _I64, _I64, _I32]),
+    "stemseg_hip_flat_dense_capacity": (C.c_int32, [_I64]),
+    "stemseg_hip_conv3d_zero_t_halo":(C.c_int, [C.POINTER(Volume), _P, _P, C.POINTER(Volume), _I32, _I32, _I32, _I32, _P, _I64, C.POINTER(ConvEpilogue),
                                                 _I32, _F, _P, _P, _P]),
     "stemseg_hip_conv3d_zero_t_halo_clips": (C.c_int, [C.POINTER(Volume), _P, _P, C.POINTER(Volume), _I32, _I32, _I32, _I32, _P, _I64, C.POINTER(ConvEpilogue),
                                                       _I32, _F, _P, _P, _I32, _P]),
@@ -491,16 +495,16 @@
     return e
 
 
-PLAN_GN, PLAN_ZERO_T_HALO = 1, 2
+PLAN_GN, PLAN_ZERO_T_HALO, PLAN_PAIR_PLANES = 1, 2, 4
 TILE_CFG_DEEP = 8
 PLAN_REDUCE_FORMS = {0: None, 1: "vec16", 2: "scalar"}
 PLAN_GN_FORMS = {0: None, 1: "tile epilogue", 2: "split-K reduce", 3: "separate pass"}
 
 
-def conv3d_plan(vin, vout, k, tile_cfg=0, scratch=None, epilogue=None, bias=1 << 20, gn_groups=0, zero_t_halo=False, plan_clips=0):
+def conv3d_plan(vin, vout, k, tile_cfg=0, scratch=None, epilogue=None, bias=1 << 20, gn_groups=0, zero_t_halo=False, plan_clips=0, pair_planes=False):
     kt, kh, kw = (k, k, k) if isinstance(k, int) else k
     e = _conv_epilogue(epilogue)
-    form = (PLAN_GN if gn_groups > 0 else 0) | (PLAN_ZERO_T_HALO if zero_t_halo else 0)
+    form = (PLAN_GN if gn_groups > 0 else 0) | (PLAN_ZERO_T_HALO if zero_t_halo else 0) | (PLAN_PAIR_PLANES if pair_planes else 0)
     addr, floats = scratch if scratch is not None else (None, 0)
     cap = 4
     rec, count = (ConvPlanRecord * cap)(), _I32(0)
@@ -516,6 +520,25 @@
         d["reduce"], d["gn"] = PLAN_REDUCE_FORMS[r.reduce], PLAN_GN_FORMS[r.gn]
         out.append(d)
     return out
+
+
+def conv3d_pair_planes(vin, packed_w, bias, vout, k, planes, tile_cfg=0, splitk_scratch=None, epilogue=None):
+    n = 0 if splitk_scratch is None else splitk_scratch.numel()
+    kt, kh, kw = (k, k, k) if isinstance(k, int) else k
+    e = _conv_epilogue(dict(epilogue or {}, precision="f16x3"))
+    assert planes.dtype == torch.int32 and planes.is_contiguous() and planes.numel() >= vout.C * vout.T * vout.H * vout.W
+    done = _I32(0)
+    check(lib().stemseg_hip_conv3d_pair_planes(C.byref(vin), ptr(packed_w), ptr(bias), C.byref(vout), kt, kh, kw, tile_cfg, ptr(splitk_scratch), n,
+                                               C.byref(e), ptr(planes), C.byref(done), stream()))
+    return bool(done.value)
+
+
+def flat_dense_run_max(H, W, pitch, frame_stride=None, nt=512):
+    return int(lib().stemseg_hip_flat_dense_run_max(H, W, pitch, (H + 2) * pitch if frame_stride is None else frame_stride, nt))
+
+
+def flat_dense_capacity(pitch):
+    return int(lib().stemseg_hip_flat_dense_capacity(pitch))
 
 
 def conv3d(vin, packed_w, bias, vout, k, tile_cfg=0, splitk_scratch=None, epilogue=None):
```

New measurement: 128.9, median of 6. Within noise of the previous version (+1.0%).
